# wyhlovecpp/GPT-Image-Edit

Measured on AMD Instinct MI355X. Metric: edited images/sec, 28-step FLUX-Kontext (VAE encode + 28 x MMDiT + VAE decode), higher is better.
Workload: dtype bf16; 1 GPU; cfg2_single_512x512_28step; batch_per_gpu=1, global_batch=1, height=512, width=512, S_txt=512, S_tgt=1024, S_cond=1024, seq_len=2560, num_inference_steps=28, blocks=19 double + 38 single, parallelism=dp1

## Files before the change

### gpt_image_edit_amd/csrc/attention_common.h

```cpp
#pragma once
#include <stdlib.h>

#include <type_traits>

#include "fk_common.h"

struct AttnParams {
  const bf16_t* q;
  const bf16_t* k;
  const bf16_t* v;
  bf16_t* o;
  int B, H, S;
  int64_t v_ld, v_bs;
  int64_t o_ld, o_bs;
  float scale_log2;
  float* lse;
  int n_items, min_part;
  int sk_rounds;
  float* sk_partials;
  unsigned* sk_ctl;
};

struct AttnMxOut {
  uint8_t *qa, *sa, *qb, *sb;
  int64_t ldq, lds;
  int split;
};

namespace {

constexpr int HD = 128;
constexpr int KVBLK = 64;
constexpr int K_TILE_BYTES = KVBLK * HD * 2;
constexpr int STAGE_BYTES = 2 * K_TILE_BYTES;

constexpr int PART_FLOATS = 256 * 128 + 2 * 512;

typedef __attribute__((address_space(3))) void lds_void;
typedef __attribute__((address_space(1))) const void gbl_void;
typedef short s16x4_t __attribute__((ext_vector_type(4)));

FK_DEV void buffer_lds16(__amdgpu_buffer_rsrc_t rsrc, char* lds_dst, int voffset, int soffset) {
#if defined(__HIP_DEVICE_COMPILE__)
  __builtin_amdgcn_raw_ptr_buffer_load_lds(rsrc, (lds_void*)lds_dst, 16, voffset, soffset, 0, 0);
#else
  (void)rsrc; (void)lds_dst; (void)voffset; (void)soffset;
#endif
}
FK_DEV void buffer_lds16(const BufDesc& d, char* lds_dst, int voffset, int soffset) {
  buffer_lds_opaque<16>(d, lds_addr_of(lds_dst), voffset, soffset);
}
FK_DEV s16x4_t lds_tr16(const char* p) {
  return __builtin_amdgcn_ds_read_tr16_b64_v4i16((__attribute__((address_space(3))) s16x4_t*)p);
}
template <int N>
FK_DEV void wait_vmcnt() {
  if constexpr (N == 0) asm volatile("s_waitcnt vmcnt(0)" ::: "memory");
  else if constexpr (N == 4) asm volatile("s_waitcnt vmcnt(4)" ::: "memory");
  else if constexpr (N == 8) asm volatile("s_waitcnt vmcnt(8)" ::: "memory");
  else if constexpr (N == 16) asm volatile("s_waitcnt vmcnt(16)" ::: "memory");
  else static_assert(N == 0, "add the vmcnt literal");
}

FK_DEV float merge2(float a, float wa, float b, float wb) {
#pragma clang fp contract(off)
  const float pa = a * wa;
  const float pb = b * wb;
  return pa + pb;
}

#ifndef FK_ATTN_PRIO
#define FK_ATTN_PRIO 1
#endif

}

int fk_attention_fwd4_launch(const AttnParams& p, int grid, bool streamk, hipStream_t stream);
int fk_attention_fwd4_mx_launch(const AttnParams& p, const AttnMxOut& mx, int grid, bool streamk, hipStream_t stream);
```

### gpt_image_edit_amd/csrc/attention_fwd.hip

```cpp
#include "attention_common.h"

namespace {

struct AttnParamsMasked : AttnParams {
  const uint64_t* kmask;
};

template <int NW, bool F32OUT, bool ILV, bool STREAMK, bool KMASK = false>
__global__ __launch_bounds__(NW * 64, NW >= 8 ? 2 : 1) void attention_fwd_kernel(
    const std::conditional_t<KMASK, AttnParamsMasked, AttnParams> p) {
  static_assert(!(KMASK && STREAMK), "masked launches take the plain grid");
  constexpr int STAGES = 3;
  constexpr int QBLK = NW * 32;
  static_assert(QBLK == 256, "the item list and the stream-K partial layout assume 256 query rows per workgroup");
  constexpr int LOADS = 32 / NW;
  constexpr int KL = LOADS / 2;
  constexpr int PF = STAGES - 1;
  extern __shared__ __attribute__((aligned(16))) char smem[];
  const int tid = threadIdx.x;
  const int lane = tid & 63;
  const int wave = __builtin_amdgcn_readfirstlane(tid >> 6);
  const int ql = lane & 31;
  const int hh = lane >> 5;

// ... 494 lines not shown
    const bool wide = ((p.o_ld | p.o_bs) & 7) == 0 && ((uintptr_t)p.o & 15) == 0;
#pragma unroll
    for (int df = 0; df < 4; ++df)
#pragma unroll
      for (int g = 0; g < 4; g += 2) {
        u32x2_t a, c;
        a[0] = pack_bf2(o[df][4 * g + 0] * inv, o[df][4 * g + 1] * inv);
        a[1] = pack_bf2(o[df][4 * g + 2] * inv, o[df][4 * g + 3] * inv);
        c[0] = pack_bf2(o[df][4 * g + 4] * inv, o[df][4 * g + 5] * inv);
        c[1] = pack_bf2(o[df][4 * g + 6] * inv, o[df][4 * g + 7] * inv);
        if (wide) {
#if defined(__HIP_DEVICE_COMPILE__)
          const auto r0 = __builtin_amdgcn_permlane32_swap(a[0], c[0], false, false);
          const auto r1 = __builtin_amdgcn_permlane32_swap(a[1], c[1], false, false);
          const u32x4_t w = {r0[0], r1[0], r0[1], r1[1]};
          if (q_row < p.S) *(u32x4_t*)(orow + 32 * df + 8 * g + 8 * hh) = w;
#endif
        } else if (q_row < p.S) {
          *(u32x2_t*)(orow + 32 * df + 8 * g + 4 * hh) = a;
          *(u32x2_t*)(orow + 32 * df + 8 * (g + 1) + 4 * hh) = c;
        }
      }
  }
  if constexpr (!STREAMK) break;
  else __syncthreads();
  }
}


__global__ __launch_bounds__(64) void pack_key_mask_kernel(const uint8_t* mask, int64_t batch_stride, int S, uint64_t* out) {
  const int t = blockIdx.x, b = blockIdx.y;
  const int key = t * KVBLK + (int)threadIdx.x;
  const bool valid = key < S && mask[(int64_t)b * batch_stride + key] != 0;
  const uint64_t w = __builtin_amdgcn_ballot_w64(valid);
  if (threadIdx.x == 0) out[(int64_t)b * gridDim.x + t] = w;
}

template <int NW, bool F32OUT, bool ILV, bool STREAMK, bool KMASK = false>
int launch(const std::conditional_t<KMASK, AttnParamsMasked, AttnParams>& p, int grid, hipStream_t stream) {
  constexpr int SMEM = 3 * STAGE_BYTES + 16;
  auto kern = attention_fwd_kernel<NW, F32OUT, ILV, STREAMK, KMASK>;
  FK_ENSURE_MAX_LDS(kern, SMEM, "fk_attention_fwd_bf16");
  hipLaunchKernelGGL(kern, dim3(grid), dim3(NW * 64), SMEM, stream, p);
  FK_CHECK_LAUNCH("fk_attention_fwd_bf16");
  return FK_OK;
}

static int attn_kernel_choice() {
  static int v = -1;
  if (v < 0) {
    const char* e = getenv("FK_ATTN_KERNEL");
    v = e && atoi(e) == 8 ? 8 : 4;
  }
  return v;
}

static int attn_cu_count() {
  static int cus = 0;
  if (!cus) {
    int dev = 0, v = 0;
    if (hipGetDevice(&dev) == hipSuccess &&
        hipDeviceGetAttribute(&v, hipDeviceAttributeMultiprocessorCount, dev) == hipSuccess && v > 0) cus = v;
    else return 256;
  }
  return cus;
}
constexpr int ATTN_MIN_PART = 8;
constexpr int ATTN_CTL_BYTES = 16384;

static bool use_interleaved(const AttnParams& p) {
  static int ov = -2;
  if (ov == -2) {
    const char* e = getenv("FK_ATTN_ILV");
    ov = e ? atoi(e) : -1;
  }
  if (ov >= 0) return ov != 0;
  return p.n_items >= 512;
}

int attention_entry(const void* q, const void* k, const void* v, void* o, int32_t B, int32_t H, int32_t S, int64_t v_ld,
                    int64_t v_batch_stride, int64_t o_ld, int64_t o_batch_stride, float scale, bool f32out,
                    hipStream_t stream, float* lse = nullptr, void* ws = nullptr, int64_t ws_bytes = 0, int grid = 0,
                    const AttnMxOut* mx = nullptr,
                    const uint64_t* kmask = nullptr) {
  FK_CHECK_ARG(grid >= -1 && grid != 1, "fk_attention_fwd_ws_bf16: grid %d is not 0 (stream-K grid where the plain one wastes a round), "
               "-1 (always one workgroup per 256-row block) or a workgroup count >= 2 (test hook)", grid);
  FK_CHECK_ARG(q && k && v && (o || mx), "fk_attention_fwd_bf16: null pointer");
  FK_CHECK_ARG(B > 0 && H > 0 && S > 0, "fk_attention_fwd_bf16: bad B/H/S %d %d %d", B, H, S);
  FK_CHECK_ARG(mx || (o_ld % 4 == 0 && o_batch_stride % 4 == 0 && ((uintptr_t)o % (f32out ? 16 : 8) == 0)),
               "fk_attention_fwd_bf16: output must be 8-byte aligned (o_ld %% 4 == 0)");
  FK_CHECK_ARG(v_ld % 8 == 0 && v_batch_stride % 8 == 0, "fk_attention_fwd_bf16: V strides must be multiples of 8");
  FK_CHECK_ARG(((uintptr_t)q % 16 == 0) && ((uintptr_t)k % 16 == 0) && ((uintptr_t)v % 16 == 0),
               "fk_attention_fwd_bf16: q/k/v must be 16-byte aligned");
  FK_CHECK_ARG(v_ld > 0 && (int64_t)S * HD * 2 < (1ll << 31) && ((int64_t)(S - 1) * v_ld + HD) * 2 < (1ll << 31) &&
                   (int64_t)(S + KVBLK) * v_ld * 2 < (1ll << 31),
               "fk_attention_fwd_bf16: S = %d with v_ld = %lld exceeds the 2 GiB a (batch, head)'s K / V may span", S,
               (long long)v_ld);
  const int64_t n_items = (int64_t)((S + 255) / 256) * H * B, nkt = (S + KVBLK - 1) / KVBLK;
  FK_CHECK_ARG(n_items * nkt < (1ll << 31), "fk_attention_fwd_bf16: B * H * S^2 too large for 32-bit tile counters");
  AttnParams p;
  p.q = (const bf16_t*)q; p.k = (const bf16_t*)k; p.v = (const bf16_t*)v; p.o = (bf16_t*)o;
  p.B = B; p.H = H; p.S = S; p.v_ld = v_ld; p.v_bs = v_batch_stride; p.o_ld = o_ld; p.o_bs = o_batch_stride;
  p.scale_log2 = scale * 1.4426950408889634f;
  p.lse = lse;
  p.n_items = (int)n_items;
  p.min_part = ATTN_MIN_PART;
  p.sk_rounds = 0;
  p.sk_partials = nullptr;
  p.sk_ctl = nullptr;
  if (kmask) {
    AttnParamsMasked pm;
    static_cast<AttnParams&>(pm) = p;
    pm.kmask = kmask;
    if (f32out) return launch<8, true, false, false, true>(pm, (int)n_items, stream);
    return use_interleaved(p) ? launch<8, false, true, false, true>(pm, (int)n_items, stream)
                              : launch<8, false, false, false, true>(pm, (int)n_items, stream);
  }
  if (f32out) return launch<8, true, false, false>(p, (int)n_items, stream);
  const int mode = grid == 0 ? 1 : (grid < 0 ? 0 : grid);
  const int G = mode >= 2 ? (mode < attn_cu_count() ? mode : attn_cu_count()) : attn_cu_count();
  const int64_t rounds = (n_items + G - 1) / G;
  const bool wasteful = mode >= 2 || (n_items > G && (rounds * G - n_items) * 25 >= rounds * G);
  int sk_rounds = (int)(n_items / G) - 1;
  while (sk_rounds >= 0 && (n_items - (int64_t)sk_rounds * G) * nkt < (int64_t)G * (nkt + 2 * ATTN_MIN_PART)) --sk_rounds;
  const bool cut_once = sk_rounds >= 0;
  const int64_t need = ATTN_CTL_BYTES + (int64_t)G * PART_FLOATS * 4;
  if (mode && wasteful && cut_once && ws && ws_bytes >= need && G <= ATTN_CTL_BYTES / 8) {
    p.sk_rounds = sk_rounds;
    FK_CHECK_ARG((uintptr_t)ws % 16 == 0, "fk_attention_fwd_ws_bf16: workspace must be 16-byte aligned");
    p.sk_ctl = (unsigned*)ws;
    p.sk_partials = (float*)((char*)ws + ATTN_CTL_BYTES);
    if (mx) return fk_attention_fwd4_mx_launch(p, *mx, G, true, stream);
    if (attn_kernel_choice() == 4) return fk_attention_fwd4_launch(p, G, true, stream);
    return use_interleaved(p) ? launch<8, false, true, true>(p, G, stream) : launch<8, false, false, true>(p, G, stream);
  }
  if (mx) return fk_attention_fwd4_mx_launch(p, *mx, (int)n_items, false, stream);
  if (attn_kernel_choice() == 4) return fk_attention_fwd4_launch(p, (int)n_items, false, stream);
  return use_interleaved(p) ? launch<8, false, true, false>(p, (int)n_items, stream)
                            : launch<8, false, false, false>(p, (int)n_items, stream);
}

}

extern "C" int64_t fk_attention_ws_bytes(void) { return ATTN_CTL_BYTES + (int64_t)attn_cu_count() * PART_FLOATS * 4; }

extern "C" int fk_attention_fwd_bf16(const void* q, const void* k, const void* v, void* o, int32_t B,
                                     int32_t H, int32_t S, int64_t v_ld, int64_t v_batch_stride, int64_t o_ld,
                                     int64_t o_batch_stride, float scale, fk_stream_t stream_) {
  return attention_entry(q, k, v, o, B, H, S, v_ld, v_batch_stride, o_ld, o_batch_stride, scale, false,
                         (hipStream_t)stream_);
}

extern "C" int fk_attention_fwd_lse_bf16(const void* q, const void* k, const void* v, void* o, float* lse, int32_t B,
                                         int32_t H, int32_t S, int64_t v_ld, int64_t v_batch_stride, int64_t o_ld,
                                         int64_t o_batch_stride, float scale, fk_stream_t stream_) {
  FK_CHECK_ARG(lse != nullptr, "fk_attention_fwd_lse_bf16: null lse");
  return attention_entry(q, k, v, o, B, H, S, v_ld, v_batch_stride, o_ld, o_batch_stride, scale, false,
                         (hipStream_t)stream_, lse);
}

extern "C" int fk_attention_fwd_ws_bf16(const void* q, const void* k, const void* v, void* o, float* lse, int32_t B, int32_t H,
                                        int32_t S, int64_t v_ld, int64_t v_batch_stride, int64_t o_ld, int64_t o_batch_stride,
                                        float scale, void* ws, int64_t ws_bytes, int32_t grid, fk_stream_t stream_) {
  return attention_entry(q, k, v, o, B, H, S, v_ld, v_batch_stride, o_ld, o_batch_stride, scale, false,
                         (hipStream_t)stream_, lse, ws, ws_bytes, grid);
}

extern "C" int fk_attention_fwd_ws_mxfp8(const void* q, const void* k, const void* v, float* lse, int32_t B, int32_t H, int32_t S,
                                         int64_t v_ld, int64_t v_batch_stride, float scale, const fk_attn_mx_out* out, void* ws,
                                         int64_t ws_bytes, int32_t grid, fk_stream_t stream_) {
  FK_CHECK_ARG(out != nullptr, "fk_attention_fwd_ws_mxfp8: null destination");
  FK_CHECK_ARG(H > 0 && S > 0 && out->split >= 0 && out->split <= S, "fk_attention_fwd_ws_mxfp8: bad H / S / split %d %d %lld", H, S,
               (long long)out->split);
  const int split = out->split == 0 ? S : (int)out->split;
  FK_CHECK_ARG(out->q && out->scales && (split == S || (out->q_b && out->scales_b)),
               "fk_attention_fwd_ws_mxfp8: null output pointer (rows [%d, %d) need the second stream)", split, S);
  const uintptr_t qbits = (uintptr_t)out->q | (split < S ? (uintptr_t)out->q_b : 0);
  const uintptr_t sbits = (uintptr_t)out->scales | (split < S ? (uintptr_t)out->scales_b : 0);
  FK_CHECK_ARG(out->ldq >= (int64_t)H * 128 && out->ldq % 16 == 0 && qbits % 16 == 0,
               "fk_attention_fwd_ws_mxfp8: output byte rows must be 16-byte aligned with ldq >= H * 128 (ldq %lld)", (long long)out->ldq);
  FK_CHECK_ARG(out->ldq_scale >= (int64_t)H * 4 && out->ldq_scale % 4 == 0 && sbits % 4 == 0,
               "fk_attention_fwd_ws_mxfp8: scale rows must be 4-byte aligned with ldq_scale >= H * 4 (ldq_scale %lld)",
               (long long)out->ldq_scale);
  if (attn_kernel_choice() != 4) {
    fk_set_error("fk_attention_fwd_ws_mxfp8: only the 4-wave kernel has the MXFP8-output form (FK_ATTN_KERNEL=8 is set)");
    return FK_EUNSUPPORTED;
  }
  const AttnMxOut mx = {(uint8_t*)out->q, (uint8_t*)out->scales, (uint8_t*)out->q_b, (uint8_t*)out->scales_b, out->ldq, out->ldq_scale,
                        split};
  return attention_entry(q, k, v, nullptr, B, H, S, v_ld, v_batch_stride, 0, 0, scale, false, (hipStream_t)stream_, lse, ws, ws_bytes,
                         grid, &mx);
}

extern "C" int fk_attention_fwd_f32_debug(const void* q, const void* k, const void* v, float* o, int32_t B,
                                          int32_t H, int32_t S, int64_t v_ld, int64_t v_batch_stride, int64_t o_ld,
                                          int64_t o_batch_stride, float scale, fk_stream_t stream_) {
  return attention_entry(q, k, v, o, B, H, S, v_ld, v_batch_stride, o_ld, o_batch_stride, scale, true,
                         (hipStream_t)stream_);
}

extern "C" int fk_pack_key_mask(const uint8_t* mask, int64_t batch_stride, int32_t B, int32_t S, uint64_t* out, fk_stream_t stream_) {
  FK_CHECK_ARG(mask && out && (uintptr_t)out % 8 == 0, "fk_pack_key_mask: null pointer or an output that is not 8-byte aligned");
  FK_CHECK_ARG(B > 0 && B <= 65535 && S > 0 && batch_stride >= 0, "fk_pack_key_mask: bad B / S / batch_stride %d %d %lld", B, S,
               (long long)batch_stride);
  hipLaunchKernelGGL(pack_key_mask_kernel, dim3((S + KVBLK - 1) / KVBLK, B), dim3(64), 0, (hipStream_t)stream_, mask, batch_stride, (int)S, out);
  FK_CHECK_LAUNCH("fk_pack_key_mask");
  return FK_OK;
}

extern "C" int fk_attention_fwd_masked_bf16(const void* q, const void* k, const void* v, void* o, float* lse, const uint64_t* kmask,
                                            int32_t B, int32_t H, int32_t S, int64_t v_ld, int64_t v_batch_stride, int64_t o_ld,
                                            int64_t o_batch_stride, float scale, fk_stream_t stream_) {
  FK_CHECK_ARG(kmask != nullptr && (uintptr_t)kmask % 8 == 0, "fk_attention_fwd_masked_bf16: the key mask must be an 8-byte aligned pointer");
  return attention_entry(q, k, v, o, B, H, S, v_ld, v_batch_stride, o_ld, o_batch_stride, scale, false, (hipStream_t)stream_, lse,
                         nullptr, 0, -1, nullptr, kmask);
}

extern "C" int fk_attention_fwd_masked_f32_debug(const void* q, const void* k, const void* v, float* o, const uint64_t* kmask, int32_t B,
                                                 int32_t H, int32_t S, int64_t v_ld, int64_t v_batch_stride, int64_t o_ld,
                                                 int64_t o_batch_stride, float scale, fk_stream_t stream_) {
  FK_CHECK_ARG(kmask != nullptr && (uintptr_t)kmask % 8 == 0, "fk_attention_fwd_masked_f32_debug: the key mask must be an 8-byte aligned pointer");
  return attention_entry(q, k, v, o, B, H, S, v_ld, v_batch_stride, o_ld, o_batch_stride, scale, true, (hipStream_t)stream_, nullptr,
                         nullptr, 0, -1, nullptr, kmask);
}
```

### gpt_image_edit_amd/csrc/attention_fwd4_kernel.inc

```
template <bool STREAMK>
__global__ __launch_bounds__(256, 1) void FK_A4_KERNEL(FK_A4_PARAMS) {
  constexpr int NW = 4, STAGES = A4_STAGES, QBLK = 256, LOADS = 32 / NW, KL = LOADS / 2, PF = STAGES - 1;
  extern __shared__ __attribute__((aligned(16))) char smem[];
  const int tid = threadIdx.x;
  const int lane = tid & 63;
  const int wave = __builtin_amdgcn_readfirstlane(tid >> 6);
  const int ql = lane & 31, hh = lane >> 5;
  const int nqb = (p.S + QBLK - 1) / QBLK;
  const int nkt = (p.S + KVBLK - 1) / KVBLK;
  int pos;
  {
    const int nwg = gridDim.x;
    const int q8 = nwg >> 3, r8 = nwg & 7;
    const int xcd = blockIdx.x & 7, idx = blockIdx.x >> 3;
    pos = (xcd < r8 ? xcd * (q8 + 1) : r8 * (q8 + 1) + (xcd - r8) * q8) + idx;
  }
  int u = 0, u_end = 0, round = 0;
  if constexpr (STREAMK) {
    const unsigned G = gridDim.x;
    const unsigned U = (unsigned)(p.n_items - p.sk_rounds * (int)G) * (unsigned)nkt;
    const unsigned qU = U / G, rU = U - qU * G;
    auto cut = [&](unsigned j) __attribute__((always_inline)) {
      unsigned c = qU * j + (rU * j) / G;
      const unsigned r = c % (unsigned)nkt;
      if (r != 0 && r < (unsigned)p.min_part) c -= r;
      else if (r != 0 && (unsigned)nkt - r < (unsigned)p.min_part) c += (unsigned)nkt - r;
      return (int)c;
    };
    u = cut(pos);
    u_end = cut(pos + 1);
  }
  const int prow = lane >> 4, pslot = lane & 15;
  const int tj = (lane & 15) >> 2, tq = lane & 3, tdh = (lane >> 4) & 1;
  const int v_rd = K_TILE_BYTES + (4 * hh + tj) * 256 + tdh * 32 + tq * 8;
  const int k_rd = ql * 256;
  const int k_sw = ql & 15;

  for (;;) {
  int item = pos, kt0 = 0, kt1 = nkt;
  if constexpr (STREAMK) {
    if (round < p.sk_rounds) {
      item = round * (int)gridDim.x + pos;
      ++round;
    } else {
      if (u >= u_end) break;
      const int ti = (unsigned)(u_end - 1) / (unsigned)nkt;
      item = p.sk_rounds * (int)gridDim.x + ti;
      kt1 = u_end - ti * nkt;
      kt0 = max(u - ti * nkt, 0);
      u_end -= kt1 - kt0;
    }
  }
  const int qb = item % nqb;
  const int bh = item / nqb;
  const int b = bh / p.H, h = bh - b * p.H;
  const int q_row0 = qb * QBLK + wave * 64;
  const bf16_t* Kg = p.k + (int64_t)bh * p.S * HD;
  const bf16_t* Vg = p.v + (int64_t)b * p.v_bs + h * HD;

  bf16x8_t qfA[8], qfB[8];
  {
    const bf16_t* qa = p.q + ((int64_t)bh * p.S + min(q_row0 + ql, p.S - 1)) * HD + 8 * hh;
    const bf16_t* qbp = p.q + ((int64_t)bh * p.S + min(q_row0 + 32 + ql, p.S - 1)) * HD + 8 * hh;
#pragma unroll
    for (int kk = 0; kk < 8; ++kk) {
      qfA[kk] = *(const bf16x8_t*)(qa + 16 * kk);
      qfB[kk] = *(const bf16x8_t*)(qbp + 16 * kk);
    }
  }
  const DmaDesc rs_k = make_dma_desc(Kg, (int64_t)p.S * HD * 2);
  const DmaDesc rs_v = make_dma_desc(Vg, ((int64_t)(p.S - 1) * p.v_ld + HD) * 2);
  const int k_voff0 = ((wave * 4 + prow) * HD + ((pslot ^ (wave * 4 + prow)) << 3)) * 2;
  const int v_voff0 = (int)(((wave * 4 + prow) * p.v_ld + ((((pslot >> 2) ^ prow) << 5) + ((pslot & 3) << 3))) * 2);
  const int k_tile_bytes = KVBLK * HD * 2, v_tile_bytes = (int)(KVBLK * p.v_ld * 2);
  const int v_piece_step = (int)(16 * p.v_ld * 2);
  auto issue_tile = [&](int kt, int stage) __attribute__((always_inline)) {
    char* sb = smem + stage * STAGE_BYTES;
#pragma unroll
    for (int i = 0; i < KL; ++i) {
      buffer_lds16(rs_k, sb + (i * NW + wave) * 1024, k_voff0, kt * k_tile_bytes + i * 4096);
      buffer_lds16(rs_v, sb + K_TILE_BYTES + (i * NW + wave) * 1024, v_voff0, kt * v_tile_bytes + i * v_piece_step);
    }
  };

  f32x16_t oA[4], oB[4];
  constexpr float REF_BIAS = 24.0f;
  float mA = 0.f, mB = 0.f, lA = 0.f, lB = 0.f, tA = 0.f, tB = 0.f;
  int st_cur = 0, st_pf = PF;
  auto fill = [&]() __attribute__((always_inline)) {
#pragma unroll
    for (int s = 0; s < PF; ++s)
      if (A4_DMA >= 2 || kt0 + s < kt1) issue_tile(min(kt0 + s, kt1 - 1), s);
    st_cur = 0;
    st_pf = PF;
  };
  auto acquire_tile = [&](int kt) __attribute__((always_inline)) {
    if (kt + PF - 1 < kt1) wait_vmcnt<(PF - 1) * LOADS>();
    else wait_vmcnt<0>();
    __builtin_amdgcn_s_barrier();
    if (kt + PF < kt1) issue_tile(kt + PF, st_pf);
    return smem + st_cur * STAGE_BYTES;
  };
  auto release_tile = [&]() __attribute__((always_inline)) {
    st_cur = (st_cur == STAGES - 1) ? 0 : st_cur + 1;
    st_pf = (st_pf == STAGES - 1) ? 0 : st_pf + 1;
  };
  auto k_frag = [&](const char* sb, int kb, int kk) __attribute__((always_inline)) {
    return *(const bf16x8_t*)(sb + k_rd + kb * 8192 + (((2 * kk + hh) ^ k_sw) << 4));
  };
  auto v_frag = [&](const char* sb, int st, int df) __attribute__((always_inline)) {
    const char* vp = sb + v_rd + st * 4096 + ((df ^ tj) << 6);
    const s16x4_t lo = lds_tr16(vp);
    const s16x4_t hi = lds_tr16(vp + 2048);
    bf16x8_t vf;
    vf[0] = lo[0]; vf[1] = lo[1]; vf[2] = lo[2]; vf[3] = lo[3];
    vf[4] = hi[0]; vf[5] = hi[1]; vf[6] = hi[2]; vf[7] = hi[3];
    return vf;
  };
  auto mask_block = [&](f32x16_t& s, int kt, int kb) __attribute__((always_inline)) {
    const int kbase = kt * KVBLK + 32 * kb + 4 * hh;
#pragma unroll
    for (int r = 0; r < 16; ++r)
      if (kbase + (r & 3) + 8 * (r >> 2) >= p.S) s[r] = -1.0e30f;
  };
  auto block_max = [&](const f32x16_t& s) __attribute__((always_inline)) {
    float mx = s[0];
#pragma unroll
    for (int r = 1; r < 16; ++r) mx = fmaxf(mx, s[r]);
    return fmaxf(mx, __shfl_xor(mx, 32)) * p.scale_log2;
  };
  bf16x8_t kf[8], vfr[8];
  f32x16_t sA, sB;
  u32x4_t pA[2], pB[2];

#define FK_SLOT_FENCE() __builtin_amdgcn_sched_barrier(0)
  auto s_mfma = [&](f32x16_t& acc, const bf16x8_t& a, const bf16x8_t& b, bool first) __attribute__((always_inline)) {
    if (first) asm volatile("v_mfma_f32_32x32x16_bf16 %0, %1, %2, 0" : "=&v"(acc) : "v"(a), "v"(b));
// ... 306 lines not shown
```

### gpt_image_edit_amd/csrc/blocks.hip

```cpp
#include "fk_common.h"

namespace {

constexpr int HD = 128;

struct Dims {
  int B, S_txt, S_img, S, H, D;
};

struct View {
  const void* p;
  fk_rows r;
};
View view(const void* base, const Dims& d, int64_t ld, int64_t r0, int64_t R, int64_t c0) {
  return View{(const char*)base + (r0 * ld + c0) * 2, fk_rows{ld, R, (int64_t)d.S * ld}};
}

void set_ws(fk_gemm_args& g, const fk_block_ws& ws) {
  if (g.K >= 6144 && g.N % 256 == 0 && (int64_t)g.M <= 256ll * ws.splitk_slots && ws.splitk_ws) {
    g.splitk_ws = ws.splitk_ws;
    g.splitk_slots = ws.splitk_slots;
  }
}

// ... 205 lines not shown
  {
    fk_gemm_args g = gemm(none, nullptr, w.bqkv, view(ws.qkv, d, 3 * D, 0, d.S, 0), Ms, 3 * D, D, FK_EPI_QKV);
    qkv_epi(g, ws, d, w.norm_q, w.norm_k, 0);
    ctl(g, ws); FK_TRY(mx_gemm(mxws, &g, 1, &n8, &wx.qkv, nullptr, 0, st));
  }
  const int rc_mx = (mxws.fused & 2) ? attention_mx(ws, d, cat8, nullptr, 0, st) : FK_EUNSUPPORTED;
  if (rc_mx != FK_EUNSUPPORTED) FK_TRY(rc_mx);
  else {
    FK_TRY(fk_attention_fwd_ws_bf16(ws.q, ws.k, (const char*)ws.qkv + (int64_t)2 * D * 2, ws.cat, nullptr, B, d.H, d.S, 3 * D,
                                    (int64_t)d.S * 3 * D, 5 * D, (int64_t)d.S * 5 * D, 0.08838834764831845f, ws.attn_ws,
                                    ws.attn_ws_bytes, ws.attn_grid, st));
    const View att = view(ws.cat, d, 5 * D, 0, d.S, 0);
    FK_TRY(quantize_view(mxws, att, Ms, D, cat8, st));
  }
  {
    fk_gemm_args g = gemm(none, nullptr, w.b_mlp, none, Ms, 4 * D, D, FK_EPI_GELU_TANH);
    ctl(g, ws); FK_TRY(mx_gemm(mxws, &g, 1, &n8, &wx.mlp, &cat8, D, st));
  }
  {
    fk_gemm_args g = gemm(none, nullptr, w.b_out, s_all, Ms, D, 5 * D, FK_EPI_GATE_RES);
    gate_res(g, s_all, chunk(2), mod_bs, d.S);
    set_ws(g, ws);
    ctl(g, ws); FK_TRY(mx_gemm(mxws, &g, 1, &cat8, &wx.out, nullptr, 0, st));
  }
  return FK_OK;
}

int double_block(const fk_block_ws& ws, const Dims& d, const fk_double_block_weights& w, const void* mod, int64_t mod_bs,
                 fk_stream_t st, const fk_mx_ws* mxws = nullptr,
                 const fk_double_block_weights_mx* wx = nullptr) {
  if (mxws && wx && mxws->fused) return double_block_fused(ws, d, w, mod, mod_bs, st, *mxws, *wx);
  FK_CHECK_ARG(ws.o && ws.ff && d.S_txt > 0, "fk_double_block_fwd: needs the o / ff buffers and a text stream");
  Mx mxc;
  auto mx = [&](const fk_mx_pair* pair) -> const Mx* { if (!pair) return nullptr; mxc = Mx{mxws, pair}; return &mxc; };
  const int D = d.D, B = d.B, Mi = B * d.S_img, Mt = B * d.S_txt;
  const char* mi = (const char*)mod + w.mod_off_img * 2;
  const char* mt = (const char*)mod + w.mod_off_txt * 2;
  auto chunk = [&](const char* m, int j) { return (const void*)(m + (int64_t)j * D * 2); };
  const View s_all = view(ws.s, d, D, 0, d.S, 0), n_all = view(ws.n, d, D, 0, d.S, 0);
  const View h = view(ws.s, d, D, d.S_txt, d.S_img, 0), cx = view(ws.s, d, D, 0, d.S_txt, 0);
  const View n_img = view(ws.n, d, D, d.S_txt, d.S_img, 0), n_txt = view(ws.n, d, D, 0, d.S_txt, 0);
  const int64_t M = (int64_t)B * d.S;
  FK_TRY(fk_ln_modulate2_bf16(s_all.p, s_all.r, (void*)n_all.p, n_all.r, chunk(mt, 0), chunk(mt, 1), chunk(mi, 0), chunk(mi, 1),
                              d.S_txt, mod_bs, d.S, M, D, ws.eps, st));
  {
    fk_gemm_args g[2];
    g[0] = gemm(n_img, w.wqkv_img, w.bqkv_img, view(ws.qkv, d, 3 * D, d.S_txt, d.S_img, 0), Mi, 3 * D, D, FK_EPI_QKV);
    qkv_epi(g[0], ws, d, w.norm_q, w.norm_k, d.S_txt);
    g[1] = gemm(n_txt, w.wqkv_txt, w.bqkv_txt, view(ws.qkv, d, 3 * D, 0, d.S_txt, 0), Mt, 3 * D, D, FK_EPI_QKV);
    qkv_epi(g[1], ws, d, w.norm_added_q, w.norm_added_k, 0);
    ctl(g[0], ws); FK_TRY(block_gemm(g, 2, mx(wx ? &wx->qkv_img : nullptr), st));
  }
  FK_TRY(fk_attention_fwd_ws_bf16(ws.q, ws.k, (const char*)ws.qkv + (int64_t)2 * D * 2, ws.o, nullptr, B, d.H, d.S, 3 * D,
                                  (int64_t)d.S * 3 * D, D, (int64_t)d.S * D, 0.08838834764831845f, ws.attn_ws, ws.attn_ws_bytes, ws.attn_grid, st));
  {
    fk_gemm_args g[2];
    g[0] = gemm(view(ws.o, d, D, d.S_txt, d.S_img, 0), w.w_out, w.b_out, h, Mi, D, D, FK_EPI_GATE_RES);
    gate_res(g[0], h, chunk(mi, 2), mod_bs, d.S_img);
    g[1] = gemm(view(ws.o, d, D, 0, d.S_txt, 0), w.w_add_out, w.b_add_out, cx, Mt, D, D, FK_EPI_GATE_RES);
    gate_res(g[1], cx, chunk(mt, 2), mod_bs, d.S_txt);
    set_ws(g[0], ws); set_ws(g[1], ws);
    ctl(g[0], ws); FK_TRY(block_gemm(g, 2, mx(wx ? &wx->out : nullptr), st));
  }
  FK_TRY(fk_ln_modulate2_bf16(s_all.p, s_all.r, (void*)n_all.p, n_all.r, chunk(mt, 3), chunk(mt, 4), chunk(mi, 3), chunk(mi, 4),
                              d.S_txt, mod_bs, d.S, M, D, ws.eps, st));
  {
    fk_gemm_args g[2];
    g[0] = gemm(n_img, w.w_ff1, w.b_ff1, view(ws.ff, d, 4 * D, d.S_txt, d.S_img, 0), Mi, 4 * D, D, FK_EPI_GELU_TANH);
    g[1] = gemm(n_txt, w.w_ff1_ctx, w.b_ff1_ctx, view(ws.ff, d, 4 * D, 0, d.S_txt, 0), Mt, 4 * D, D, FK_EPI_GELU_TANH);
    ctl(g[0], ws); FK_TRY(block_gemm(g, 2, mx(wx ? &wx->ff1 : nullptr), st));
  }
  {
    fk_gemm_args g[2];
    g[0] = gemm(view(ws.ff, d, 4 * D, d.S_txt, d.S_img, 0), w.w_ff2, w.b_ff2, h, Mi, D, 4 * D, FK_EPI_GATE_RES);
    gate_res(g[0], h, chunk(mi, 5), mod_bs, d.S_img);
    g[1] = gemm(view(ws.ff, d, 4 * D, 0, d.S_txt, 0), w.w_ff2_ctx, w.b_ff2_ctx, cx, Mt, D, 4 * D, FK_EPI_GATE_RES);
    gate_res(g[1], cx, chunk(mt, 5), mod_bs, d.S_txt);
    set_ws(g[0], ws); set_ws(g[1], ws);
    ctl(g[0], ws); FK_TRY(block_gemm(g, 2, mx(wx ? &wx->ff2 : nullptr), st));
  }
  return FK_OK;
}

int single_block(const fk_block_ws& ws, const Dims& d, const fk_single_block_weights& w, const void* mod, int64_t mod_bs,
                 fk_stream_t st, const fk_mx_ws* mxws = nullptr, const fk_single_block_weights_mx* wx = nullptr) {
  if (mxws && wx && mxws->fused) return single_block_fused(ws, d, w, mod, mod_bs, st, *mxws, *wx);
  Mx mxc;
  auto mx = [&](const fk_mx_pair* pair) -> const Mx* { if (!pair) return nullptr; mxc = Mx{mxws, pair}; return &mxc; };
  FK_CHECK_ARG(ws.cat != nullptr, "fk_single_block_fwd: needs the [attn | mlp] buffer");
  const int D = d.D, B = d.B;
  const int Ms = B * d.S;
  const char* m0 = (const char*)mod + w.mod_off * 2;
  auto chunk = [&](int j) { return (const void*)(m0 + (int64_t)j * D * 2); };
  const View s_all = view(ws.s, d, D, 0, d.S, 0), n_all = view(ws.n, d, D, 0, d.S, 0);
  FK_TRY(fk_ln_modulate_bf16(s_all.p, s_all.r, (void*)n_all.p, n_all.r, chunk(0), chunk(1), mod_bs, d.S, (int64_t)Ms, D, ws.eps, st));
  {
    fk_gemm_args g = gemm(n_all, w.wqkv, w.bqkv, view(ws.qkv, d, 3 * D, 0, d.S, 0), Ms, 3 * D, D, FK_EPI_QKV);
    qkv_epi(g, ws, d, w.norm_q, w.norm_k, 0);
    ctl(g, ws); FK_TRY(block_gemm(&g, 1, mx(wx ? &wx->qkv : nullptr), st));
  }
  FK_TRY(fk_attention_fwd_ws_bf16(ws.q, ws.k, (const char*)ws.qkv + (int64_t)2 * D * 2, ws.cat, nullptr, B, d.H, d.S, 3 * D,
                                  (int64_t)d.S * 3 * D, 5 * D, (int64_t)d.S * 5 * D, 0.08838834764831845f, ws.attn_ws,
                                  ws.attn_ws_bytes, ws.attn_grid, st));
  {
    fk_gemm_args g = gemm(n_all, w.w_mlp, w.b_mlp, view(ws.cat, d, 5 * D, 0, d.S, D), Ms, 4 * D, D, FK_EPI_GELU_TANH);
    ctl(g, ws); FK_TRY(block_gemm(&g, 1, mx(wx ? &wx->mlp : nullptr), st));
  }
  {
    fk_gemm_args g = gemm(view(ws.cat, d, 5 * D, 0, d.S, 0), w.w_out, w.b_out, s_all, Ms, D, 5 * D, FK_EPI_GATE_RES);
    gate_res(g, s_all, chunk(2), mod_bs, d.S);
    set_ws(g, ws);
    ctl(g, ws); FK_TRY(block_gemm(&g, 1, mx(wx ? &wx->out : nullptr), st));
  }
  return FK_OK;
}

}

extern "C" int fk_double_block_fwd(const fk_block_ws* ws, const fk_double_block_weights* w, const void* mod,
                                   int64_t mod_batch_stride, fk_stream_t stream) {
  Dims d;
  FK_TRY(check_ws(ws, d, "fk_double_block_fwd"));
  FK_CHECK_ARG(w && mod, "fk_double_block_fwd: null weights / modulation");
  return double_block(*ws, d, *w, mod, mod_batch_stride, stream);
}

extern "C" int fk_single_block_fwd(const fk_block_ws* ws, const fk_single_block_weights* w, const void* mod,
                                   int64_t mod_batch_stride, fk_stream_t stream) {
  Dims d;
  FK_TRY(check_ws(ws, d, "fk_single_block_fwd"));
  FK_CHECK_ARG(w && mod, "fk_single_block_fwd: null weights / modulation");
  return single_block(*ws, d, *w, mod, mod_batch_stride, stream);
}

extern "C" int fk_mmdit_blocks_fwd(const fk_block_ws* ws, const fk_double_block_weights* dbl, int32_t n_double,
                                   const fk_single_block_weights* sgl, int32_t n_single, const void* mod,
                                   int64_t mod_batch_stride, fk_stream_t stream) {
  Dims d;
  FK_TRY(check_ws(ws, d, "fk_mmdit_blocks_fwd"));
  FK_CHECK_ARG(mod && n_double >= 0 && n_single >= 0 && (n_double == 0 || dbl) && (n_single == 0 || sgl),
               "fk_mmdit_blocks_fwd: null weights / modulation");
  for (int i = 0; i < n_double; ++i) FK_TRY(double_block(*ws, d, dbl[i], mod, mod_batch_stride, stream));
  for (int i = 0; i < n_single; ++i) FK_TRY(single_block(*ws, d, sgl[i], mod, mod_batch_stride, stream));
  return FK_OK;
}

namespace {
int check_mx(const fk_mx_ws* mx, const char* who) {
  FK_CHECK_ARG(mx && mx->q && mx->s && (uintptr_t)mx->q % 16 == 0 && (uintptr_t)mx->s % 4 == 0,
               "%s: null or misaligned quantized-activation workspace", who);
  FK_CHECK_ARG((mx->fused & 3) != 2,
               "%s: fk_mx_ws.fused = %d: bit 1 (the attention emits MXFP8) is valid only together with bit 0 (the fused schedule)", who,
               (int)mx->fused);
  return FK_OK;
}
}

extern "C" int fk_double_block_fwd_mx(const fk_block_ws* ws, const fk_mx_ws* mx, const fk_double_block_weights* w,
                                      const fk_double_block_weights_mx* wx, const void* mod, int64_t mod_batch_stride,
                                      fk_stream_t stream) {
  Dims d;
  FK_TRY(check_ws(ws, d, "fk_double_block_fwd_mx"));
  FK_TRY(check_mx(mx, "fk_double_block_fwd_mx"));
  FK_CHECK_ARG(w && wx && mod, "fk_double_block_fwd_mx: null weights / modulation");
  return double_block(*ws, d, *w, mod, mod_batch_stride, stream, mx, wx);
}

extern "C" int fk_single_block_fwd_mx(const fk_block_ws* ws, const fk_mx_ws* mx, const fk_single_block_weights* w,
                                      const fk_single_block_weights_mx* wx, const void* mod, int64_t mod_batch_stride,
                                      fk_stream_t stream) {
  Dims d;
  FK_TRY(check_ws(ws, d, "fk_single_block_fwd_mx"));
  FK_TRY(check_mx(mx, "fk_single_block_fwd_mx"));
  FK_CHECK_ARG(w && wx && mod, "fk_single_block_fwd_mx: null weights / modulation");
  return single_block(*ws, d, *w, mod, mod_batch_stride, stream, mx, wx);
}

extern "C" int fk_mmdit_blocks_fwd_mx(const fk_block_ws* ws, const fk_mx_ws* mx, const fk_double_block_weights* dbl,
                                      const fk_double_block_weights_mx* dblx, int32_t n_double, const fk_single_block_weights* sgl,
                                      const fk_single_block_weights_mx* sglx, int32_t n_single, const void* mod,
                                      int64_t mod_batch_stride, fk_stream_t stream) {
  Dims d;
  FK_TRY(check_ws(ws, d, "fk_mmdit_blocks_fwd_mx"));
  FK_TRY(check_mx(mx, "fk_mmdit_blocks_fwd_mx"));
  FK_CHECK_ARG(mod && n_double >= 0 && n_single >= 0 && (n_double == 0 || (dbl && dblx)) && (n_single == 0 || (sgl && sglx)),
               "fk_mmdit_blocks_fwd_mx: null weights / modulation");
  if (mx->fused) {
    if (n_double > 0) FK_TRY(check_fused_ws(*mx, d, 4 * d.D, "fk_mmdit_blocks_fwd_mx"));
    if (n_single > 0) FK_TRY(check_fused_ws(*mx, d, 5 * d.D, "fk_mmdit_blocks_fwd_mx"));
  }
  for (int i = 0; i < n_double; ++i) FK_TRY(double_block(*ws, d, dbl[i], mod, mod_batch_stride, stream, mx, &dblx[i]));
  for (int i = 0; i < n_single; ++i) FK_TRY(single_block(*ws, d, sgl[i], mod, mod_batch_stride, stream, mx, &sglx[i]));
  return FK_OK;
}
```

### gpt_image_edit_amd/libfk.py

```python
import ctypes
import os

_HERE = os.path.dirname(os.path.abspath(__file__))
LIB_PATH = os.environ.get("FK_LIB_PATH") or os.path.join(_HERE, "libfk_gfx950.so")

c_i32, c_i64, c_f32, c_vp = ctypes.c_int32, ctypes.c_int64, ctypes.c_float, ctypes.c_void_p
c_f64 = ctypes.c_double

FK_PRODIGY_SLOTS = ("d", "d_max", "d_numerator", "d_denom", "d_hat", "dlr", "k", "skipped", "sum_dot", "sum_abs")

FK_SPLITK_SLOT_BYTES = 256 * 256 * 4 + 8
FK_EPI_NONE, FK_EPI_GELU_TANH, FK_EPI_SILU, FK_EPI_GATE_RES, FK_EPI_RES, FK_EPI_SCALE, FK_EPI_QKV = range(7)


class Rows(ctypes.Structure):
    _fields_ = [("ld", c_i64), ("rows_per_batch", c_i64), ("batch_stride", c_i64)]


class GemmArgs(ctypes.Structure):
    _fields_ = [
        ("A", c_vp), ("a", Rows),
        ("W", c_vp), ("ldw", c_i64),
        ("bias", c_vp),
        ("C", c_vp), ("c", Rows),
# ... 47 lines not shown
        ("dmodT", c_vp), ("gemm_variant", c_i32), ("gemm_plan", c_i32), ("gemm_group_m", c_i32), ("gemm_mfma", c_i32), ("attn_grid", c_i32),
        ("attn_passes", c_i32), ("gemm_variant_used", ctypes.POINTER(c_i32))]


class BlockSaved(ctypes.Structure):
    _fields_ = [(n, c_vp) for n in ("x0", "n1", "qkv", "q", "k", "y1", "h1", "o", "lse", "x1", "n2", "y2")]


SINGLE_GRAD_FIELDS = ("dwqkv", "dbqkv", "dw_mlp", "db_mlp", "dw_out", "db_out", "dnorm", "dw_mod", "db_mod")
DOUBLE_GRAD_FIELDS = ("dwqkv_img", "dbqkv_img", "dwqkv_txt", "dbqkv_txt", "dw_out", "db_out", "dw_add_out", "db_add_out", "dw_ff1", "db_ff1",
                      "dw_ff1_ctx", "db_ff1_ctx", "dw_ff2", "db_ff2", "dw_ff2_ctx", "db_ff2_ctx", "dnorm", "dw_mod_img", "db_mod_img",
                      "dw_mod_txt", "db_mod_txt")


class SingleBlockGrads(ctypes.Structure):
    _fields_ = [(n, c_vp) for n in SINGLE_GRAD_FIELDS]


class DoubleBlockGrads(ctypes.Structure):
    _fields_ = [(n, c_vp) for n in DOUBLE_GRAD_FIELDS]


DOUBLE_BLOCK_FIELDS = ("wqkv_img", "bqkv_img", "wqkv_txt", "bqkv_txt", "norm_q", "norm_k", "norm_added_q", "norm_added_k",
                       "w_out", "b_out", "w_add_out", "b_add_out", "w_ff1", "b_ff1", "w_ff1_ctx", "b_ff1_ctx",
                       "w_ff2", "b_ff2", "w_ff2_ctx", "b_ff2_ctx")
SINGLE_BLOCK_FIELDS = ("wqkv", "bqkv", "norm_q", "norm_k", "w_mlp", "b_mlp", "w_out", "b_out")


class DoubleBlockWeights(ctypes.Structure):
    _fields_ = [(n, c_vp) for n in DOUBLE_BLOCK_FIELDS] + [("mod_off_img", c_i64), ("mod_off_txt", c_i64)]


class SingleBlockWeights(ctypes.Structure):
    _fields_ = [(n, c_vp) for n in SINGLE_BLOCK_FIELDS] + [("mod_off", c_i64)]


class MxPair(ctypes.Structure):
    _fields_ = [("q", c_vp), ("s", c_vp)]


DOUBLE_BLOCK_MX_FIELDS = ("qkv_img", "qkv_txt", "out", "add_out", "ff1", "ff1_ctx", "ff2", "ff2_ctx")
SINGLE_BLOCK_MX_FIELDS = ("qkv", "mlp", "out")


class DoubleBlockWeightsMx(ctypes.Structure):
    _fields_ = [(n, MxPair) for n in DOUBLE_BLOCK_MX_FIELDS]


class SingleBlockWeightsMx(ctypes.Structure):
    _fields_ = [(n, MxPair) for n in SINGLE_BLOCK_MX_FIELDS]


class AttnMxOut(ctypes.Structure):
    _fields_ = [("q", c_vp), ("scales", c_vp), ("q_b", c_vp), ("scales_b", c_vp), ("split", c_i64), ("ldq", c_i64), ("ldq_scale", c_i64)]


class MxWs(ctypes.Structure):
    _fields_ = [("q", c_vp), ("s", c_vp), ("q_bytes", c_i64), ("s_bytes", c_i64), ("fused", c_i32),
                ("quantize_launches", ctypes.POINTER(c_i32)), ("splitk", c_i32)]


class LoraTerm(ctypes.Structure):
    _fields_ = [("up", c_vp), ("ld_up", c_i64), ("down", c_vp), ("ld_down", c_i64), ("rank", c_i32), ("scale", c_f32)]


FK_LORA_MAX_TERMS, FK_LORA_MAX_RANK = 4, 128

SIGNATURES = {
    "fk_gemm_bf16": (c_i32, [ctypes.POINTER(GemmArgs), c_vp]),
    "fk_gemm_bf16_grouped": (c_i32, [ctypes.POINTER(GemmArgs), c_i32, c_vp]),
    "fk_quantize_mxfp8": (c_i32, [c_vp, Rows, c_i64, c_i32, c_vp, c_i64, c_vp, c_i64, c_vp]),
    "fk_gemm_mxfp8": (c_i32, [ctypes.POINTER(GemmMxfp8Args), c_vp]),
    "fk_gemm_mxfp8_grouped": (c_i32, [ctypes.POINTER(GemmMxfp8Args), c_i32, c_vp]),
    "fk_gemm_mxfp8_q": (c_i32, [ctypes.POINTER(GemmMxfp8QArgs), c_vp]),
    "fk_gemm_mxfp8_q_grouped": (c_i32, [ctypes.POINTER(GemmMxfp8QArgs), c_i32, c_vp]),
    "fk_ln_modulate_mxfp8": (c_i32, [c_vp, Rows, c_vp, c_i64, c_vp, c_i64, c_vp, c_vp, c_i64, c_i64, c_i64, c_i32, c_f32, c_vp]),
    "fk_ln_modulate2_mxfp8": (c_i32, [c_vp, Rows, c_vp, c_vp, c_vp, c_vp, c_i64, c_i64, c_vp, c_vp, c_vp, c_vp, c_i64, c_i64, c_i64,
                                      c_i64, c_i32, c_f32, c_vp]),
    "fk_ln_modulate_bf16": (c_i32, [c_vp, Rows, c_vp, Rows, c_vp, c_vp, c_i64, c_i64, c_i64, c_i32, c_f32, c_vp]),
    "fk_ln_modulate2_bf16": (c_i32, [c_vp, Rows, c_vp, Rows, c_vp, c_vp, c_vp, c_vp, c_i64, c_i64, c_i64, c_i64, c_i32, c_f32, c_vp]),
    "fk_qkv_post_bf16": (c_i32, [c_vp] * 9 + [c_i32] * 4 + [c_f32, c_vp]),
    "fk_attention_fwd_bf16": (c_i32, [c_vp] * 4 + [c_i32] * 3 + [c_i64] * 4 + [c_f32, c_vp]),
    "fk_attention_fwd_ws_bf16": (c_i32, [c_vp] * 5 + [c_i32] * 3 + [c_i64] * 4 + [c_f32, c_vp, c_i64, c_i32, c_vp]),
    "fk_attention_fwd_ws_mxfp8": (c_i32, [c_vp] * 4 + [c_i32] * 3 + [c_i64] * 2 + [c_f32, ctypes.POINTER(AttnMxOut), c_vp, c_i64, c_i32, c_vp]),
    "fk_attention_ws_bytes": (c_i64, []),
    "fk_attention_fwd_f32_debug": (c_i32, [c_vp] * 4 + [c_i32] * 3 + [c_i64] * 4 + [c_f32, c_vp]),
    "fk_pack_key_mask": (c_i32, [c_vp, c_i64, c_i32, c_i32, c_vp, c_vp]),
    "fk_attention_fwd_masked_bf16": (c_i32, [c_vp] * 6 + [c_i32] * 3 + [c_i64] * 4 + [c_f32, c_vp]),
    "fk_attention_fwd_masked_f32_debug": (c_i32, [c_vp] * 5 + [c_i32] * 3 + [c_i64] * 4 + [c_f32, c_vp]),
    "fk_attention_bwd_masked_bf16": (c_i32, [ctypes.POINTER(AttnView)] * 4 + [c_vp, c_vp] + [ctypes.POINTER(AttnView)] * 3 + [c_vp] + [c_i32] * 3 + [c_f32, c_i32, c_vp]),
    "fk_attention_fwd_lse_bf16": (c_i32, [c_vp] * 5 + [c_i32] * 3 + [c_i64] * 4 + [c_f32, c_vp]),
    "fk_attention_bwd_bf16": (c_i32, [ctypes.POINTER(AttnView)] * 4 + [c_vp, c_vp] + [ctypes.POINTER(AttnView)] * 3 + [c_i32] * 3 + [c_f32, c_vp]),
    "fk_attention_bwd_ws_bf16": (c_i32, [ctypes.POINTER(AttnView)] * 4 + [c_vp, c_vp] + [ctypes.POINTER(AttnView)] * 3 + [c_i32] * 3 + [c_f32, c_vp, c_i64, c_i32, c_i32, c_vp]),
    "fk_bwd_ws_floats": (c_i64, []),
    "fk_bwd_ew_max_blocks": (c_i64, []),
    "fk_ln_modulate_bwd_bf16": (c_i32, [c_vp, Rows, c_vp, Rows, c_vp, c_i64, c_i64, c_vp, Rows, c_vp, Rows, c_vp, c_vp, c_i64, c_vp, c_i32, c_i32, c_f32, c_vp]),
    "fk_gate_res_bwd_bf16": (c_i32, [c_vp, Rows, c_vp, Rows, c_vp, c_i64, c_i64, c_vp, Rows, c_vp, c_i64, c_vp, c_i32, c_i32, c_vp]),
    "fk_gelu_bwd_bf16": (c_i32, [c_vp, c_vp, c_vp, c_i64, c_vp]),
    "fk_silu_bwd_bf16": (c_i32, [c_vp, c_vp, c_vp, c_i64, c_vp]),
    "fk_qkv_post_bwd_bf16": (c_i32, [c_vp] * 12 + [c_i32] * 4 + [c_f32, c_vp]),
    "fk_gate_res_fwd_bf16": (c_i32, [c_vp, Rows, c_vp, Rows, c_vp, c_i64, c_i64, c_vp, Rows, c_i64, c_i32, c_vp]),
    "fk_gelu_tanh_bf16": (c_i32, [c_vp, Rows, c_vp, Rows, c_i64, c_i32, c_vp]),
    "fk_f32_to_bf16_transposed": (c_i32, [c_vp, c_i64, c_vp, c_i32, c_i32, c_i32, c_vp]),
    "fk_colsum_bf16": (c_i32, [c_vp, Rows, c_i64, c_i32, c_vp, c_vp, c_vp]),
    "fk_rowdot_bf16": (c_i32, [c_vp, c_i64, c_i64, c_vp, c_i64, c_i64, c_vp, c_i32, c_i32, c_i32, c_vp]),
    "fk_silu_bf16": (c_i32, [c_vp, c_vp, c_i64, c_vp]),
    "fk_timestep_proj": (c_i32, [c_vp, c_i32, c_vp, c_vp, c_i32, c_vp]),
    "fk_add3_bf16": (c_i32, [c_vp] * 4 + [c_i64, c_vp]),
    "fk_true_cfg_bf16": (c_i32, [c_vp, c_vp, c_vp, c_f32, c_i64, c_vp]),
    "fk_reduce_ws_doubles": (c_i64, []),
    "fk_flow_noisy_tokens_bf16": (c_i32, [c_vp, c_vp, c_vp, c_vp, c_i64] + [c_i32] * 4 + [c_vp]),
    "fk_flow_loss_bf16": (c_i32, [c_vp, c_i64, c_vp, c_vp, c_vp, c_vp, c_i64, c_vp, c_vp] + [c_i32] * 4 + [c_vp]),
    "fk_flow_loss_weighted_bf16": (c_i32, [c_vp, c_i64, c_vp, c_vp, c_vp, c_vp, c_vp, c_vp, c_vp, c_i64, c_vp, c_vp] + [c_i32] * 4 + [c_vp]),
    "fk_sumsq": (c_i32, [c_vp, c_i32, c_i64, c_i32, c_vp, c_vp, c_vp]),
    "fk_adamw_step": (c_i32, [c_vp, c_vp, c_vp, c_i32, c_vp, c_vp, c_vp] + [c_f32] * 6 + [c_i32, c_i64, c_vp]),
    "fk_adamw_step_scaled": (c_i32, [c_vp, c_vp, c_vp, c_i32, c_vp, c_vp, c_vp] + [c_f32] * 7 + [c_i32, c_i64, c_vp]),
    "fk_prodigy_ws_doubles": (c_i64, []),
    "fk_prodigy_begin": (c_i32, [c_vp] + [c_f64] * 4 + [c_i32, c_vp]),
    "fk_prodigy_moments": (c_i32, [c_vp, c_vp, c_vp, c_i32, c_vp, c_vp, c_vp, c_vp, c_vp] + [c_f32] * 6 + [c_f64, c_i32, c_i32,
                                                                                                         c_i64, c_vp, c_vp]),
    "fk_prodigy_update_d": (c_i32, [c_vp, c_f64, c_f64, c_f64, c_vp]),
    "fk_prodigy_apply": (c_i32, [c_vp, c_vp, c_vp, c_vp, c_vp, c_f32, c_f32, c_i32, c_i64, c_vp]),
    "fk_euler_step_bf16": (c_i32, [c_vp, c_i64, c_vp, c_i64, c_i32, c_i32, c_i32, c_f32, c_vp]),
    "fk_euler_inpaint_step_bf16": (c_i32, [c_vp, c_i64, c_vp, c_i64, c_vp, c_i64, c_vp, c_i64, c_vp, c_i64, c_i32, c_i32, c_i32,
                                           c_f32, c_f32, c_vp]),
    "fk_scale_noise_bf16": (c_i32, [c_vp, c_i64, c_vp, c_i64, c_vp, c_i64, c_i32, c_i32, c_i32, c_f32, c_vp]),
    "fk_ab2_step_bf16": (c_i32, [c_vp, c_i64, c_vp, c_i64, c_vp, c_i64, c_vp, c_i64, c_vp, c_i64, c_vp, c_i64, c_i32, c_i32, c_i32,
                                 c_f32, c_f32, c_i32, c_f32, c_vp]),
    "fk_solver_step_f32": (c_i32, [c_vp, c_i64, c_vp, c_i64, c_vp, c_i64, c_vp, c_i64, c_vp, c_i64, c_vp, c_i64, c_vp, c_i64,
                                   c_i32, c_i32, c_i32, c_f32, c_f32, c_i32, c_i32, c_f32, c_vp]),
    "fk_absdiff_ws_floats": (c_i64, []),
    "fk_absdiff_sums_bf16": (c_i32, [c_vp, Rows, c_vp, Rows, c_i64, c_i32, c_i32, c_vp, c_vp, c_i64, c_vp]),
    "fk_residual_absdiff_sums_bf16": (c_i32, [c_vp, Rows, c_vp, Rows, c_vp, Rows, c_vp, Rows, c_i64, c_i32, c_i32, c_vp, c_vp, c_i64,
                                              c_vp]),
    "fk_residual_save_bf16": (c_i32, [c_vp, Rows, c_vp, Rows, c_vp, Rows, c_i64, c_i32, c_i32, c_vp]),
    "fk_residual_apply_bf16": (c_i32, [c_vp, Rows, c_vp, Rows, c_vp, Rows, c_i64, c_i32, c_i32, c_vp]),
    "fk_lora_merge_bf16": (c_i32, [c_vp, c_i64, c_vp, c_i64, c_i32, c_i32, ctypes.POINTER(LoraTerm), c_i32, c_vp]),
    "fk_lora_grad_ws_floats": (c_i64, [c_i32, c_i32, c_i32]),
    "fk_lora_grad_bf16": (c_i32, [c_vp, c_i64, c_vp, c_i64, c_vp, c_i64, c_i32, c_i32, c_i32, c_f32, c_vp, c_vp, c_vp, c_i64, c_vp]),
    "fk_lora_grad_acc_bf16": (c_i32, [c_vp, c_i64, c_vp, c_i64, c_vp, c_i64, c_i32, c_i32, c_i32, c_f32, c_vp, c_vp, c_i32, c_vp, c_i64,
                                      c_vp]),
    "fk_lora_side_grad_ws_floats": (c_i64, [c_i64] * 5),
    "fk_lora_side_grad_bf16": (c_i32, [c_vp, c_i64, c_i64, c_vp, c_i64, c_i64, c_i64, c_i64, c_i64, c_i64, c_vp, c_i64, c_vp, c_i64,
                                       c_i64, c_f32, c_vp, c_vp, c_i32, c_vp, c_i64, c_vp]),
    "fk_transpose_bf16": (c_i32, [c_vp, c_i64, c_i64, c_vp, c_i64, c_i64, c_i32, c_i32, c_i32, c_vp]),
    "fk_attention_hd512_bf16": (c_i32, [c_vp, c_vp, c_vp, c_i64, c_i64, c_vp, c_i64, c_i64, c_i32, c_i32, c_f32, c_vp]),
    "fk_softmax_rows": (c_i32, [c_vp, c_i64, c_vp, c_i64, c_i64, c_i32, c_vp]),
    "fk_softmax_rows_parts": (c_i32, [c_vp, c_i64, c_vp, c_i64, c_i64, c_i64, c_i32, c_vp]),
    "fk_split_f32_rows": (c_i32, [c_vp, c_i64, c_vp, c_i64, c_i64, c_i64, c_i32, c_i32, c_i32, c_vp]),
    "fk_groupnorm_f32_nhwc": (c_i32, [c_vp, c_vp, c_vp, c_vp, c_vp, c_vp, c_i32, c_i64, c_i32, c_i32, c_f32, c_i32, c_i32, c_vp]),
    "fk_conv2d_nhwc_f32out": (c_i32, [c_vp, c_vp]),
    "fk_conv3x3_halo_f32out": (c_i32, [c_vp, c_vp]),
    "fk_nchw_f32_to_nhwc_parts": (c_i32, [c_vp, c_vp, c_i32, c_i32, c_i32, c_i32, c_i32, c_i32, c_vp]),
    "fk_nhwc_f32_to_nchw": (c_i32, [c_vp, c_vp, c_i32, c_i32, c_i32, c_i32, c_i32, c_f32, c_f32, c_vp]),
    "fk_conv2d_nhwc_bf16": (c_i32, [ctypes.POINTER(ConvArgs), c_vp]),
    "fk_conv3x3_halo_bf16": (c_i32, [ctypes.POINTER(ConvArgs), c_vp, c_vp, c_vp, c_i32, c_i32, c_vp]),
    "fk_conv3x3_halo_f32_debug": (c_i32, [ctypes.POINTER(ConvArgs), c_vp, c_vp, c_vp, c_i32, c_i32, c_vp]),
    "fk_groupnorm_ws_floats": (c_i64, [c_i32, c_i64, c_i32]),
    "fk_groupnorm_stats_nhwc_bf16": (c_i32, [c_vp, c_vp, c_vp, c_i32, c_i64, c_i32, c_i32, c_f32, c_vp]),
    "fk_groupnorm_apply_nhwc_bf16": (c_i32, [c_vp] * 5 + [c_i32, c_i64, c_i32, c_i32, c_i32, c_vp]),
    "fk_nchw_to_nhwc_bf16": (c_i32, [c_vp, c_i32, c_vp] + [c_i32] * 5 + [c_f32, c_f32, c_vp]),
    "fk_nhwc_to_nchw": (c_i32, [c_vp, c_vp] + [c_i32] * 6 + [c_f32, c_f32, c_vp]),
    "fk_pixels_u8_to_nhwc_bf16": (c_i32, [c_vp, c_vp] + [c_i32] * 7 + [c_vp]),
    "fk_image_to_u8_nhwc": (c_i32, [c_vp, c_i32, c_vp] + [c_i32] * 4 + [c_vp]),
    "fk_mask_bbox_ws_ints": (c_i64, []),
    "fk_mask_bbox_u8": (c_i32, [c_vp] + [c_i32] * 4 + [c_vp, c_vp, c_i64, c_vp]),
    "fk_mask_blur_u8": (c_i32, [c_vp] * 4 + [c_i32] * 4 + [c_vp]),
    "fk_pixels_u8_box_to_nhwc_bf16": (c_i32, [c_vp, c_vp] + [c_i32] * 11 + [c_vp]),
    "fk_image_overlay_u8": (c_i32, [c_vp] + [c_i32] * 3 + [c_vp, c_i32, c_vp, c_i32, c_vp] + [c_i32] * 7 + [c_vp]),
    "fk_double_block_fwd": (c_i32, [ctypes.POINTER(BlockWs), ctypes.POINTER(DoubleBlockWeights), c_vp, c_i64, c_vp]),
    "fk_single_block_fwd": (c_i32, [ctypes.POINTER(BlockWs), ctypes.POINTER(SingleBlockWeights), c_vp, c_i64, c_vp]),
    "fk_single_block_bwd": (c_i32, [ctypes.POINTER(BwdWs), ctypes.POINTER(BlockSaved), ctypes.POINTER(SingleBlockWeights),
                                    ctypes.POINTER(SingleBlockGrads), c_vp]),
    "fk_double_block_bwd": (c_i32, [ctypes.POINTER(BwdWs), ctypes.POINTER(BlockSaved), ctypes.POINTER(DoubleBlockWeights),
                                    ctypes.POINTER(DoubleBlockGrads), c_vp]),
    "fk_double_block_fwd_mx": (c_i32, [ctypes.POINTER(BlockWs), ctypes.POINTER(MxWs), ctypes.POINTER(DoubleBlockWeights),
                                       ctypes.POINTER(DoubleBlockWeightsMx), c_vp, c_i64, c_vp]),
    "fk_single_block_fwd_mx": (c_i32, [ctypes.POINTER(BlockWs), ctypes.POINTER(MxWs), ctypes.POINTER(SingleBlockWeights),
                                       ctypes.POINTER(SingleBlockWeightsMx), c_vp, c_i64, c_vp]),
    "fk_mmdit_blocks_fwd_mx": (c_i32, [ctypes.POINTER(BlockWs), ctypes.POINTER(MxWs), ctypes.POINTER(DoubleBlockWeights),
                                       ctypes.POINTER(DoubleBlockWeightsMx), c_i32, ctypes.POINTER(SingleBlockWeights),
                                       ctypes.POINTER(SingleBlockWeightsMx), c_i32, c_vp, c_i64, c_vp]),
    "fk_mmdit_blocks_fwd": (c_i32, [ctypes.POINTER(BlockWs), ctypes.POINTER(DoubleBlockWeights), c_i32,
                                    ctypes.POINTER(SingleBlockWeights), c_i32, c_vp, c_i64, c_vp]),
    "fk_last_error": (ctypes.c_char_p, []),
    "fk_version": (ctypes.c_char_p, []),
}

_lib = None


def load():
    global _lib
    if _lib is not None:
        return _lib
    if not os.path.exists(LIB_PATH):
        raise RuntimeError(
            f"{LIB_PATH} not found: the HIP extension is not built. Run `python -c 'import "
            f"__graft_entry__ as g; g.build()'` (or `make -C gpt_image_edit_amd/csrc`). There is no CPU "
            f"fallback for the FLUX-Kontext hot path.")
    lib = ctypes.CDLL(LIB_PATH)
    for name, (res, args) in SIGNATURES.items():
        fn = getattr(lib, name)
        fn.restype = res
        fn.argtypes = args
    _lib = lib
    return lib


def check(code, what):
    if code != 0:
        msg = load().fk_last_error().decode(errors="replace")
        raise RuntimeError(f"{what} failed (code {code}): {msg}")
```

### gpt_image_edit_amd/ops.py

```python
import ctypes
import threading
from types import SimpleNamespace
import os

import torch

from . import helpers, libfk, param_tree
from .libfk import (FK_EPI_GATE_RES, FK_EPI_GELU_TANH, FK_EPI_NONE, FK_EPI_QKV, FK_EPI_RES, FK_EPI_SCALE,
                    FK_EPI_SILU, GemmArgs, GemmMxfp8Args, GemmMxfp8QArgs, Rows)

BF16 = torch.bfloat16


def _stream():
    return ctypes.c_void_p(torch.cuda.current_stream().cuda_stream)


def _ptr(t):
    return ctypes.c_void_p(t.data_ptr()) if t is not None else ctypes.c_void_p(0)


def _need_cuda(*ts):
    for t in ts:
        if t is not None and not t.is_cuda:
# ... 31 lines not shown
        _SPLITK_WS[key] = ws
    return ws, SPLITK_SLOTS


_VARIANT_USED = threading.local()


def _variant_slot():
    slot = getattr(_VARIANT_USED, "slot", None)
    if slot is None:
        slot = _VARIANT_USED.slot = ctypes.c_int32(0)
    return slot


def gemm_last_variant():
    return int(_variant_slot().value)


def _check_splitk_ws(splitk_ws):
    ws, slots = splitk_ws
    _need_cuda(ws)
    if (ws.dtype != torch.uint8 or not ws.is_contiguous() or int(slots) < 1 or ws.numel() < int(slots) * libfk.FK_SPLITK_SLOT_BYTES
            or ws.data_ptr() % 16 != 0):
        raise ValueError("splitk_ws: (contiguous 16-byte aligned uint8 tensor of >= slots * FK_SPLITK_SLOT_BYTES bytes, slots >= 1)")
    return ws, int(slots)


def _gemm_args(a, w, bias, out, epilogue, res, gate, out_fp32, alpha, qkv=None, layout=0, splitk_ws=None):
    _need_cuda(a, w, bias, out, res, gate)
    if a.dtype != BF16 or w.dtype != BF16:
        raise TypeError("fk_gemm_bf16 takes bf16 operands")
    if layout == 0:
        M, ra = rows_of(a)
        N, K = w.shape
        if a.shape[-1] != K:
            raise ValueError(f"K mismatch: a {tuple(a.shape)} vs w {tuple(w.shape)}")
        out_shape = (*a.shape[:-1], N)
    elif layout == 1:
        M, ra = rows_of(a)
        K, N = w.shape
        if a.shape[-1] != K or w.stride(1) != 1:
            raise ValueError(f"layout 1: a {tuple(a.shape)} @ w {tuple(w.shape)} (w rows contiguous)")
        out_shape = (*a.shape[:-1], N)
    elif layout == 2:
        a = a[0] if a.dim() == 3 and a.shape[0] == 1 else a
        w = w[0] if w.dim() == 3 and w.shape[0] == 1 else w
        K, ra = rows_of(a)
        M, N = a.shape[-1], w.shape[-1]
        Kw, rw = rows_of(w)
        if Kw != K or w.stride(-1) != 1 or (rw.rows_per_batch > 0 and rw.batch_stride != rw.rows_per_batch * rw.ld):
            raise ValueError(f"layout 2: a {tuple(a.shape)} ^T @ w {tuple(w.shape)} (uniformly strided w rows)")
        out_shape = (M, N)
    else:
        raise ValueError(f"layout {layout}")
    if out is None:
        out = torch.empty(out_shape, device=a.device, dtype=torch.float32 if out_fp32 else BF16)
    Mo, rc = rows_of(out)
    if Mo != M or out.shape[-1] != N:
        raise ValueError(f"output shape {tuple(out.shape)} does not match M={M}, N={N}")
    args = GemmArgs()
    args.layout = layout
    args.A, args.a = a.data_ptr(), ra
    args.W, args.ldw = w.data_ptr(), (w.stride(0) if layout != 2 else rw.ld)
    args.bias = bias.data_ptr() if bias is not None else None
    args.C, args.c = out.data_ptr(), rc
    if res is not None:
        Mr, rr = rows_of(res)
        if Mr != M:
            raise ValueError("residual rows mismatch")
        args.res, args.r = res.data_ptr(), rr
    if gate is not None:
        if a.dim() != 3 or gate.dim() != 2 or gate.shape[0] != a.shape[0] or gate.stride(1) != 1:
            raise ValueError("gate must be a [B, N] view matching a 3-D activation")
        args.gate = gate.data_ptr()
        args.gate_batch_stride = gate.stride(0)
        args.gate_rows_per_batch = a.shape[1]
    args.M, args.N, args.K = M, N, K
    _apply_gemm_launch(args)
    args.variant_used = ctypes.pointer(_variant_slot())
    args.epilogue, args.out_fp32, args.alpha = epilogue, int(out_fp32), float(alpha)
    if int(out_fp32) == 1:
        args.f32_flags = ((1 if bias is not None and bias.dtype == torch.float32 else 0) |
                          (2 if res is not None and res.dtype == torch.float32 and epilogue == FK_EPI_NONE else 0))
    if splitk_ws is not None:
        ws, slots = _check_splitk_ws(splitk_ws)
        args.splitk_ws, args.splitk_slots = ws.data_ptr(), slots
    elif K >= 6144 and N % 256 == 0 and M <= 256 * SPLITK_SLOTS and int(out_fp32) != 1 and layout == 0:
        ws, slots = splitk_workspace(a.device)
        args.splitk_ws, args.splitk_slots = ws.data_ptr(), slots
    if epilogue == FK_EPI_QKV:
        _set_qkv(args, qkv)
    return args, out


def _set_qkv(args, qkv):
    cs = qkv["cs"] if "cs" in qkv else pack_rope(qkv["cos"], qkv["sin"])
    _need_cuda(qkv["q_out"], qkv["k_out"], qkv["wq"], qkv["wk"], cs)
    if cs.dtype != torch.float32 or not cs.is_contiguous() or tuple(cs.shape) != (qkv["q_out"].shape[2], 64, 2):
        raise ValueError("cs must be a contiguous fp32 [S_total, 64, 2] table (see pack_rope)")
    args.q_out, args.k_out = qkv["q_out"].data_ptr(), qkv["k_out"].data_ptr()
    args.wq, args.wk = qkv["wq"].data_ptr(), qkv["wk"].data_ptr()
    args.rope_cs = cs.data_ptr()
    args.qkv_s_offset, args.qkv_s_total, args.qkv_heads = qkv["s_offset"], qkv["q_out"].shape[2], qkv["q_out"].shape[1]


def gemm(a, w, bias=None, out=None, epilogue=FK_EPI_NONE, res=None, gate=None, out_fp32=False, alpha=1.0, qkv=None, layout=0,
         splitk_ws=None):
    args, out = _gemm_args(a, w, bias, out, epilogue, res, gate, out_fp32, alpha, qkv, layout, splitk_ws)
    libfk.check(libfk.load().fk_gemm_bf16(ctypes.byref(args), _stream()), "fk_gemm_bf16")
    return out


FK_GEMM_PLAN_EXPLICIT = 8
FK_GEMM_PLAN_SPLITK = {"default": 0, "whole": 16, "symmetric": 32, "unannounced": 64}


def _env_int(name, default):
    v = os.environ.get(name)
    return default if v is None or v == "" else int(v)


LAUNCH = SimpleNamespace(
    gemm_variant=_env_int("FK_GEMM_BN", 0),
    gemm_plan=(FK_GEMM_PLAN_EXPLICIT | (_env_int("FK_GEMM_PLAN", 3) & 7)) if os.environ.get("FK_GEMM_PLAN") else 0,
    gemm_splitk=0,
    gemm_group_m=_env_int("FK_GEMM_GROUP_M", 0),
    gemm_mfma=_env_int("FK_GEMM_MFMA", 0),
    attn_grid={0: -1, 1: 0}.get(_env_int("FK_ATTN_SPLIT", 1), _env_int("FK_ATTN_SPLIT", 1)),
    attn_bwd_passes=0 if _env_int("FK_ATTN_BWD", 1) else 3)
_LAUNCH_CFG_EPOCH = [0]


def launch_config_epoch():
    return _LAUNCH_CFG_EPOCH[0]


def _set_launch(**kw):
    for k, v in kw.items():
        setattr(LAUNCH, k, v)
    _LAUNCH_CFG_EPOCH[0] += 1


def gemm_set_variant(variant):
    if int(variant) not in (0, 128, 256, 384, 512, 640, 1024):
        raise ValueError(f"gemm_set_variant: {variant} is not one of 0, 128, 256, 384, 512, 640, 1024")
    _set_launch(gemm_variant=int(variant))


def gemm_set_plan(allow):
    if not 0 <= int(allow) <= 7:
        raise ValueError(f"gemm_set_plan: {allow} is not in 0..7")
    _set_launch(gemm_plan=FK_GEMM_PLAN_EXPLICIT | int(allow))


def gemm_set_splitk_exchange(mode):
    _set_launch(gemm_splitk=FK_GEMM_PLAN_SPLITK[mode])


def launch_plan():
    if not LAUNCH.gemm_splitk:
        return LAUNCH.gemm_plan
    return (LAUNCH.gemm_plan or (FK_GEMM_PLAN_EXPLICIT | 3)) | LAUNCH.gemm_splitk


def gemm_set_group_m(depth):
    if not 0 <= int(depth) <= 4096:
        raise ValueError(f"gemm_set_group_m: {depth} is not 0 (default) or 1..4096 row tiles")
# ... 196 lines not shown
    return outs


def ln_modulate(x, shift, scale, out=None, eps=1e-6):
    _need_cuda(x, shift, scale, out)
    if x.dim() != 3:
        raise ValueError("x must be [B, R, D]")
    B, R, D = x.shape
    if out is None:
        out = torch.empty((B, R, D), device=x.device, dtype=BF16)
    M, rx = rows_of(x)
    _, ro = rows_of(out)
    if shift.stride(0) != scale.stride(0) or shift.stride(1) != 1 or scale.stride(1) != 1:
        raise ValueError("shift/scale must be [B, D] views with a common batch stride")
    lib = libfk.load()
    libfk.check(lib.fk_ln_modulate_bf16(_ptr(x), rx, _ptr(out), ro, _ptr(shift), _ptr(scale),
                                        shift.stride(0), R, M, D, eps, _stream()), "fk_ln_modulate_bf16")
    return out


def ln_modulate2(x, shift_a, scale_a, shift_b, scale_b, split, out=None, eps=1e-6):
    _need_cuda(x, shift_a, scale_a, shift_b, scale_b, out)
    B, R, D = x.shape
    if out is None:
        out = torch.empty((B, R, D), device=x.device, dtype=BF16)
    M, rx = rows_of(x)
    _, ro = rows_of(out)
    st = shift_a.stride(0)
    if any(t.stride(0) != st or t.stride(1) != 1 for t in (scale_a, shift_b, scale_b)):
        raise ValueError("modulation views must share one batch stride")
    libfk.check(libfk.load().fk_ln_modulate2_bf16(_ptr(x), rx, _ptr(out), ro, _ptr(shift_a), _ptr(scale_a),
                                                  _ptr(shift_b), _ptr(scale_b), split, st, R, M, D, eps, _stream()),
                "fk_ln_modulate2_bf16")
    return out


def qkv_post(qkv, q_out, k_out, wq_img, wk_img, wq_txt, wk_txt, cos, sin, s_txt, eps=1e-6):
    _need_cuda(qkv, q_out, k_out, cos, sin)
    B, S, D3 = qkv.shape
    H = D3 // 384
    if not qkv.is_contiguous():
        raise ValueError("qkv must be contiguous")
    lib = libfk.load()
    libfk.check(lib.fk_qkv_post_bf16(_ptr(qkv), _ptr(q_out), _ptr(k_out), _ptr(wq_img), _ptr(wk_img), _ptr(wq_txt),
                                     _ptr(wk_txt), _ptr(cos), _ptr(sin), B, S, s_txt, H, eps, _stream()),
                "fk_qkv_post_bf16")


_ATTN_WS = {}


def attention_workspace(device):
    key = (device.index if device.index is not None else torch.cuda.current_device(), torch.cuda.current_stream(device).cuda_stream)
    ws = _ATTN_WS.get(key)
    if ws is None:
        ws = torch.zeros(libfk.load().fk_attention_ws_bytes(), device=device, dtype=torch.uint8)
        _ATTN_WS[key] = ws
    return ws


def attention_set_split(mode):
    mode = int(mode)
    if mode < 0:
        raise ValueError(f"attention_set_split: {mode} is not 0, 1 or a workgroup count >= 2")
    _set_launch(attn_grid={0: -1, 1: 0}.get(mode, mode))


def pack_key_mask(mask):
    _need_cuda(mask)
    if mask.dim() != 2:
        raise ValueError("pack_key_mask takes a [B, S] mask")
    m = (mask != 0).to(torch.uint8).contiguous()
    B, S = m.shape
    out = torch.empty((B, (S + 63) // 64), device=m.device, dtype=torch.int64)
    libfk.check(libfk.load().fk_pack_key_mask(_ptr(m), m.stride(0), B, S, _ptr(out), _stream()), "fk_pack_key_mask")
    return out


def _check_key_mask(key_mask, B, S):
    if key_mask.dtype != torch.int64 or key_mask.shape != (B, (S + 63) // 64) or not key_mask.is_contiguous():
        raise ValueError(f"key_mask must be the contiguous int64 [{B}, {(S + 63) // 64}] tensor pack_key_mask gives")


def attention(q, k, v, out, scale=None, lse=None, key_mask=None):
    _need_cuda(q, k, v, out, lse, key_mask)
    B, H, S, hd = q.shape
    if hd != 128:
        raise ValueError("head_dim must be 128")
    if v.dim() != 3 or v.shape[-1] != H * 128 or v.stride(2) != 1:
        raise ValueError("v must be a [B, S, H*128] view with a contiguous last dimension")
    if lse is not None and (lse.dtype != torch.float32 or lse.shape != (B, H, S) or not lse.is_contiguous()):
        raise ValueError("lse must be a contiguous fp32 [B,H,S] tensor")
    if scale is None:
        scale = hd ** -0.5
    if key_mask is not None:
        _check_key_mask(key_mask, B, S)
        libfk.check(libfk.load().fk_attention_fwd_masked_bf16(_ptr(q), _ptr(k), _ptr(v), _ptr(out), _ptr(lse), _ptr(key_mask), B, H, S,
                                                             v.stride(1), v.stride(0), out.stride(1), out.stride(0), scale,
                                                             _stream()), "fk_attention_fwd_masked_bf16")
        return out
    ws = attention_workspace(q.device)
    libfk.check(libfk.load().fk_attention_fwd_ws_bf16(_ptr(q), _ptr(k), _ptr(v), _ptr(out), _ptr(lse), B, H, S, v.stride(1),
                                                     v.stride(0), out.stride(1), out.stride(0), scale, _ptr(ws), ws.numel(),
                                                     LAUNCH.attn_grid, _stream()), "fk_attention_fwd_bf16")
    return out


def attention_mxfp8(q, k, v, out, out_b=None, split=0, scale=None, lse=None):
    _need_cuda(q, k, v, lse, *out, *(out_b or ()))
    B, H, S, hd = q.shape
    if hd != 128:
        raise ValueError("head_dim must be 128")
    if v.dim() != 3 or v.shape[-1] != H * 128 or v.stride(2) != 1:
        raise ValueError("v must be a [B, S, H*128] view with a contiguous last dimension")
    if lse is not None and (lse.dtype != torch.float32 or lse.shape != (B, H, S) or not lse.is_contiguous()):
        raise ValueError("lse must be a contiguous fp32 [B,H,S] tensor")
    pairs = [out] + ([out_b] if out_b is not None else [])
    for qt, st in pairs:
        if qt.dtype != torch.uint8 or st.dtype != torch.uint8 or qt.dim() != 2 or st.dim() != 2 or qt.stride(1) != 1 or st.stride(1) != 1:
            raise ValueError("attention_mxfp8: an output is a (uint8 [rows, cols], uint8 [rows, cols / 32]) pair, rows contiguous")
    if len({pr[0].stride(0) for pr in pairs}) != 1 or len({pr[1].stride(0) for pr in pairs}) != 1:
        raise ValueError("attention_mxfp8: both streams' outputs must share their row strides")
    dst = libfk.AttnMxOut(_ptr(out[0]), _ptr(out[1]), _ptr(out_b[0]) if out_b is not None else None,
                          _ptr(out_b[1]) if out_b is not None else None, int(split), out[0].stride(0), out[1].stride(0))
    ws = attention_workspace(q.device)
    libfk.check(libfk.load().fk_attention_fwd_ws_mxfp8(_ptr(q), _ptr(k), _ptr(v), _ptr(lse), B, H, S, v.stride(1), v.stride(0),
                                                      hd ** -0.5 if scale is None else scale, ctypes.byref(dst), _ptr(ws),
                                                      ws.numel(), LAUNCH.attn_grid, _stream()), "fk_attention_fwd_ws_mxfp8")
    return out if out_b is None else (out, out_b)


def attention_f32_debug(q, k, v, scale=None, key_mask=None):
    _need_cuda(q, k, v, key_mask)
    B, H, S, hd = q.shape
    if hd != 128 or v.dim() != 3 or v.shape[-1] != H * 128 or v.stride(2) != 1:
        raise ValueError("q, k: [B,H,S,128]; v: [B,S,H*128] view with a contiguous last dimension")
    out = torch.empty((B, S, H * 128), device=q.device, dtype=torch.float32)
    if key_mask is not None:
        _check_key_mask(key_mask, B, S)
        libfk.check(libfk.load().fk_attention_fwd_masked_f32_debug(_ptr(q), _ptr(k), _ptr(v), _ptr(out), _ptr(key_mask), B, H, S,
                                                                  v.stride(1), v.stride(0), out.stride(1), out.stride(0),
                                                                  hd ** -0.5 if scale is None else scale, _stream()),
                    "fk_attention_fwd_masked_f32_debug")
        return out
    libfk.check(libfk.load().fk_attention_fwd_f32_debug(_ptr(q), _ptr(k), _ptr(v), _ptr(out), B, H, S, v.stride(1),
                                                       v.stride(0), out.stride(1), out.stride(0),
                                                       hd ** -0.5 if scale is None else scale, _stream()),
                "fk_attention_fwd_f32_debug")
    return out


def silu(x, out=None):
    _need_cuda(x)
    if out is None:
        out = torch.empty_like(x)
    libfk.check(libfk.load().fk_silu_bf16(_ptr(x), _ptr(out), x.numel(), _stream()), "fk_silu_bf16")
    return out


def add3(a, b, c, out=None):
    _need_cuda(a, b, c)
    if out is None:
        out = torch.empty_like(a)
    libfk.check(libfk.load().fk_add3_bf16(_ptr(a), _ptr(b), _ptr(c), _ptr(out), a.numel(), _stream()),
                "fk_add3_bf16")
    return out


def true_cfg(pos, neg, scale, out=None):
    _need_cuda(pos, neg, out)
    if pos.shape != neg.shape or pos.dtype != BF16 or neg.dtype != BF16 or not (pos.is_contiguous() and neg.is_contiguous()):
        raise ValueError("true_cfg takes two contiguous bf16 tensors of one shape")
    if out is None:
        out = torch.empty_like(pos)
    libfk.check(libfk.load().fk_true_cfg_bf16(_ptr(pos), _ptr(neg), _ptr(out), float(scale), pos.numel(), _stream()),
                "fk_true_cfg_bf16")
    return out


def timestep_proj(v, freqs, out=None):
    _need_cuda(v, freqs)
    B = v.shape[0]
    if v.dtype not in (BF16, torch.float32):
        raise TypeError("timestep must be bf16 or fp32")
# ... 926 lines not shown
```

### gpt_image_edit_amd/pipeline.py

```python
import os
from types import SimpleNamespace

import numpy as np
import torch

from . import helpers, image_processor, ops
from .scheduler import FlowMatchEulerDiscreteScheduler

BF16 = torch.bfloat16


class FluxPipelineOutput(SimpleNamespace):
    pass


class FluxKontextPipeline:
    def __init__(self, transformer, vae, scheduler=None, text_encoder=None, tokenizer=None,
                 text_encoder_2=None, tokenizer_2=None, use_graph=None):
        self.use_graph = (os.environ.get("FK_GRAPH", "0") == "1") if use_graph is None else bool(use_graph)
        self._loop_graph = None
        self.transformer = transformer
        self.vae = vae
        self.scheduler = scheduler or FlowMatchEulerDiscreteScheduler()
        self.text_encoder, self.tokenizer = text_encoder, tokenizer
# ... 398 lines not shown

        num_channels_latents = self.transformer.config.in_channels // 4
        latents, image_latents, latent_ids, image_ids = self.prepare_latents(
            image, batch_size, num_channels_latents, height, width, BF16, device, generator, latents)
        S_tgt = latents.shape[1]
        if image_ids is not None:
            latent_ids = torch.cat([latent_ids, image_ids], dim=0)
            tokens = torch.cat([latents, image_latents], dim=1).contiguous()
        else:
            tokens = latents.contiguous().clone()
        x0 = noise = None
        if mask is not None or strength < 1.0:
            if init_image is None and cond_hw == (height, width):
                x0 = image_latents
            else:
                x0 = self._encode_init_image(image_in if init_image is None else init_image, batch_size,
                                             num_channels_latents, height, width, device, edit)
            noise = latents.contiguous()

        sig = np.linspace(1.0, 1 / num_inference_steps, num_inference_steps) if sigmas is None else sigmas
        cfg = self.scheduler.config
        mu = helpers.calculate_shift(S_tgt, cfg.get("base_image_seq_len", 256), cfg.get("max_image_seq_len", 4096),
                                     cfg.get("base_shift", 0.5), cfg.get("max_shift", 1.15))
        self.scheduler.set_timesteps(sigmas=sig, mu=mu, device="cpu")
        t_start = helpers.strength_t_start(len(self.scheduler.timesteps), strength)
        timesteps = self.scheduler.timesteps[t_start:]
        self._num_timesteps = len(timesteps)
        t_model = (timesteps.to(BF16) / 1000)[:, None].expand(-1, model_batch).contiguous().to(device)
        guidance = None
        if self.transformer.config.guidance_embeds:
            guidance = torch.full([model_batch], guidance_scale, device=device, dtype=torch.float32)
        self.scheduler.set_begin_index(t_start)
        if t_start > 0:
            ops.scale_noise(x0, noise, float(self.scheduler._sigmas_host[t_start]), out=tokens[:, :S_tgt])
        steps = range(t_start, t_start + len(timesteps))
        model_tokens = torch.empty((model_batch, *tokens.shape[1:]), device=device, dtype=BF16) if do_true_cfg else tokens
        solver_order = getattr(self.scheduler, "solver_order", 1)
        if solver_order not in (1, 2):
            raise NotImplementedError(f"the denoise loop has a first- and a second-order step, not solver_order={solver_order}")
        ab2 = [self.scheduler.coefficients(i, i > t_start) for i in steps] if solver_order == 2 else None
        hist = torch.empty((batch_size, S_tgt, tokens.shape[2]), device=device, dtype=BF16) if ab2 is not None else None
        state = torch.empty((batch_size, S_tgt, tokens.shape[2]), device=device, dtype=torch.float32) \
            if latent_state == "fp32" else None

        L = SimpleNamespace(tokens=tokens, model_tokens=model_tokens, t_model=t_model, guidance=guidance, pooled=model_pooled,
                            embeds=model_embeds, text_ids=text_ids, latent_ids=latent_ids, S_tgt=S_tgt, batch_size=batch_size,
                            do_true_cfg=do_true_cfg, true_cfg_scale=true_cfg_scale, jak=joint_attention_kwargs or {},
                            geom=(height, width, None if image is None else tuple(image.shape[-2:])),
                            dsigma=[self.scheduler.dsigma(i) for i in steps], inpaint=inpaint,
                            sigma_next=[self.scheduler.sigma_next(i) for i in steps] if inpaint else [],
                            x0=x0 if mask is not None else None, noise=noise if mask is not None else None, mask=mask,
                            step_cache=step_cache, cache_state=None, ab2=ab2, hist=hist, latent_state=latent_state, state=state)
        graphable = self.use_graph and callback_on_step_end is None and not joint_attention_kwargs and not self._interrupt
        if graphable and step_cache is not None and step_cache.adaptive:
            if not self._said_adaptive_is_eager:
                print("step cache: the adaptive mode reads its measure back once per step, so this call runs the eager loop; "
                      "replay its decisions through the graph with StepCache(schedule=step_cache.computed_steps)")
                self._said_adaptive_is_eager = True
            graphable = False
        if graphable:
            tokens = self._denoise_graph(L)
        else:
            self._denoise(L, callback_on_step_end, timesteps)

        latents = tokens[:, :S_tgt]
        if output_type == "latent":
            image_out = latents.contiguous()
        else:
            z = self._unpack_latents(latents, height, width, self.vae_scale_factor).contiguous()
            vcfg = self.vae.config
            img = self.vae.decode(z, return_dict=False, pre_div=vcfg.scaling_factor, pre_add=vcfg.shift_factor)[0]
            if edit is not None and edit.overlay:
                image_out = ops.image_overlay(img.contiguous(), edit.pic, edit.alpha, edit.box).cpu().numpy()
                if output_type == "pil":
                    from PIL import Image
                    image_out = [Image.fromarray(a) for a in image_out]
            else:
                image_out = self.postprocess(img, output_type)
        if not return_dict:
            return (image_out,)
        return FluxPipelineOutput(images=image_out, latents=latents, crop_box=edit.box if edit is not None and edit.crop else None)

    def _denoise(self, L, callback_on_step_end=None, timesteps=None):
        if hasattr(self.transformer, "prepare_conditioning"):
            self.transformer.prepare_conditioning(L.t_model, L.guidance, L.pooled)
        tokens, B = L.tokens, L.batch_size
        sc, st = L.step_cache, None
        if sc is not None:
            st = self._step_cache_state(L)
            sc.begin(len(L.dsigma))
        seed = True
        for i in range(len(L.dsigma)):
            if self._interrupt:
                continue
            if L.do_true_cfg:
                L.model_tokens[:B].copy_(tokens)
                L.model_tokens[B:].copy_(tokens)
            fwd = dict(hidden_states=L.model_tokens, timestep=L.t_model[i], guidance=L.guidance,
                       pooled_projections=L.pooled, encoder_hidden_states=L.embeds,
                       txt_ids=L.text_ids, img_ids=L.latent_ids, joint_attention_kwargs=L.jak)
            if sc is None:
                noise_pred = self.transformer(**fwd, return_dict=False)[0]
            else:
                self.transformer.step_cache_begin(st, **fwd)
                compute = sc.step(i, st.sums.tolist() if sc.adaptive and i > 0 else None)
                noise_pred = self.transformer.step_cache_end(st, compute)
            if L.do_true_cfg:
                noise_pred = ops.true_cfg(noise_pred[:B], noise_pred[B:], L.true_cfg_scale)
            self._solver_step(L, i, noise_pred, seed)
            seed = False
            if callback_on_step_end is not None:
                out = callback_on_step_end(self, i, timesteps[i], {"latents": tokens[:, :L.S_tgt]})
                if out and "latents" in out:
                    tokens[:, :L.S_tgt].copy_(out["latents"])
                    seed = True
        if sc is not None:
            sc.block_passes = st.block_passes

    def _solver_step(self, L, i, noise_pred, seed):
        sigma_next = L.sigma_next[i] if L.inpaint else 0.0
        c_v, c_h, use_hist = L.ab2[i] if L.ab2 is not None else (L.dsigma[i], 0.0, 0)
        if L.state is not None:
            ops.solver_step_f32(L.state, L.tokens, noise_pred, L.S_tgt, c_v, c_h, use_hist, 0 if seed else 1, L.hist, sigma_next,
                                L.x0, L.noise, L.mask)
        elif L.ab2 is not None:
            ops.ab2_step(L.tokens, noise_pred, L.hist, L.S_tgt, c_v, c_h, use_hist, sigma_next, L.x0, L.noise, L.mask)
        elif L.inpaint:
            ops.euler_inpaint_step(L.tokens, noise_pred, L.S_tgt, c_v, sigma_next, L.x0, L.noise, L.mask)
        else:
            ops.euler_step(L.tokens, noise_pred, L.S_tgt, c_v)

    def _step_cache_state(self, L):
        tr = self.transformer
        if not hasattr(tr, "step_cache_begin"):
            raise ValueError("`step_cache` needs a transformer with the two-phase forward (HipFluxTransformer2DModel)")
        st = L.cache_state if L.cache_state is not None else self._cache_state
        sc = L.step_cache
        if st is None or st.measure != sc.adaptive or st.mode != sc.measure:
            st = tr.step_cache_state(measure=sc.adaptive, mode=sc.measure)
        if L.cache_state is None:
            self._cache_state = st
        st.steps, st.block_passes, st.have_residual, st.f = 0, 0, False, None
        return st

    _GRAPH_INPUTS = ("tokens", "t_model", "guidance", "pooled", "embeds", "text_ids", "latent_ids", "x0", "noise", "mask")

    def _graph_key(self, L):
        if hasattr(self.transformer, "packed"):
            self.transformer.packed()
        key = (tuple(L.tokens.shape), tuple(L.embeds.shape), tuple(L.latent_ids.shape), L.geom, L.do_true_cfg,
               float(L.true_cfg_scale), tuple(L.dsigma), L.guidance is None, L.S_tgt,
               getattr(self.transformer, "_pack_serial", 0), ops.launch_config_epoch(),
               L.inpaint, None if L.mask is None else tuple(L.mask.shape), tuple(L.sigma_next),
               None if L.step_cache is None else (L.step_cache.schedule, L.step_cache.measure),
               L.latent_state,
               1 if L.ab2 is None else 2, None if L.ab2 is None else tuple(L.ab2))
        return key

    def _denoise_graph(self, L):
        key = self._graph_key(L)
        cur = torch.cuda.current_stream()
        if self._loop_graph is None or self._loop_graph[0] != key:
            self._loop_graph = None
            G = SimpleNamespace(**vars(L))
            for n in self._GRAPH_INPUTS:
                t = getattr(L, n)
                setattr(G, n, None if t is None else t.clone())
            G.model_tokens = torch.empty_like(L.model_tokens) if L.do_true_cfg else G.tokens
            if L.hist is not None:
                G.hist = torch.empty_like(L.hist)
            if L.state is not None:
                G.state = torch.empty_like(L.state)
            if L.step_cache is not None:
                G.cache_state = self.transformer.step_cache_state(measure=False, mode=L.step_cache.measure)
            side = torch.cuda.Stream(device=L.tokens.device)
            side.wait_stream(cur)
            with torch.cuda.stream(side):
                self._denoise(G)
            cur.wait_stream(side)
            graph = torch.cuda.CUDAGraph()
            with torch.cuda.graph(graph):
                self._denoise(G)
            self._loop_graph = (key, G, graph)
        _, G, graph = self._loop_graph
# ... 15 lines not shown
```

### gpt_image_edit_amd/transformer.py

```python
import math
import os
from types import SimpleNamespace

import torch
from torch import nn

from . import flux_spec, ops
from .lora import LoraMixin
from .param_tree import ParamTreeMixin, build_param_tree

BF16 = torch.bfloat16
FUSE_QKV = os.environ.get("FK_FUSE_QKV", "1") != "0"
MLP_FIRST = os.environ.get("FK_MLP_FIRST", "0") == "1"
BLOCK_API = int(os.environ.get("FK_BLOCK_API", "2"))
MX_FUSED_QUANT = os.environ.get("FK_MX_FUSED_QUANT", "0") == "1"
MX_SPLITK = os.environ.get("FK_MX_SPLITK", "0") == "1"


def set_mx_splitk(on):
    global MX_SPLITK
    MX_SPLITK = bool(on)
    ops._set_launch()


MX_FUSED_ATTN = os.environ.get("FK_MX_FUSED_ATTN", "0") == "1"


def set_mx_fused_attn(on):
    global MX_FUSED_ATTN
    MX_FUSED_ATTN = bool(on)
    ops._set_launch()


def _mx_fused_bits():
    return (1 | (2 if MX_FUSED_ATTN else 0)) if MX_FUSED_QUANT else 0


OVERLAP_MLP = {"0": False, "1": True, "auto": "auto"}.get(os.environ.get("FK_OVERLAP_MLP", "0"), False)


def rope_tables(ids, axes_dim=(16, 56, 56), theta=10000.0):
    pos = ids.detach().to(torch.float32)
    cos_parts, sin_parts = [], []
    for i, d in enumerate(axes_dim):
        inv = 1.0 / (theta ** (torch.arange(0, d, 2, dtype=torch.float64, device=pos.device) / d))
        ang = pos[:, i].to(torch.float64)[:, None] * inv[None, :]
        cos_parts.append(torch.repeat_interleave(torch.cos(ang), 2, dim=1).float())
        sin_parts.append(torch.repeat_interleave(torch.sin(ang), 2, dim=1).float())
    return torch.cat(cos_parts, dim=1).contiguous(), torch.cat(sin_parts, dim=1).contiguous()


class HipFluxTransformer2DModel(LoraMixin, ParamTreeMixin, nn.Module):

    def __init__(self, config=None, device="cuda", dtype=BF16, init="empty", seed=0, weight_format="bf16"):
        super().__init__()
        if dtype != BF16:
            raise ValueError("the HIP path computes in bf16 (fp32 accumulate); dtype must be torch.bfloat16")
        cfg = dict(flux_spec.FLUX_KONTEXT_CONFIG)
        cfg.update(config or {})
        self.config = SimpleNamespace(**cfg)
        self.num_heads = cfg["num_attention_heads"]
        if cfg["attention_head_dim"] != 128:
            raise ValueError("attention_head_dim must be 128 (kernel tiling)")
        self.inner_dim = self.num_heads * 128
        shapes = flux_spec.flux_param_shapes(cfg)
        if init == "synthetic":
            state = flux_spec.synthetic_state(shapes, seed=seed, device=device, dtype=dtype,
                                              gen_device="cuda" if str(device).startswith("cuda") else None)
        else:
            state = {k: torch.empty(s, device=device, dtype=dtype) for k, s in shapes.items()}
        self._names = list(shapes.keys())
        self.__dict__["_pmap"] = build_param_tree(self, state, requires_grad=False)
        self._packed = None
        self._train_packs = False
        self._ws = {}
        self._rope_cache = {}
        self._freqs = None
        self._cond = None
        self._lora_init()
        self.weight_format = "bf16"
        self.set_weight_format(weight_format)

    WEIGHT_FORMATS = ("bf16", "mxfp8")

    def set_weight_format(self, weight_format):
        if weight_format not in self.WEIGHT_FORMATS:
            raise ValueError(f"weight_format must be one of {self.WEIGHT_FORMATS}, got {weight_format!r}")
        if weight_format != self.weight_format:
            self.weight_format = weight_format
            self._packed = None

    def load_state_dict(self, state_dict, strict=True, **kwargs):
        self._packed = None
        return super().load_state_dict(state_dict, strict=strict, **kwargs)

    @property
    def dtype(self):
        return BF16

    @property
    def device(self):
        return self.p("x_embedder.weight").device

    def _apply(self, fn, *a, **k):
        self._packed = None
        self._ws = {}
        self._rope_cache = {}
        self._freqs = None
        self._cond = None
        for name, t in self._lora_base.items():
            self._lora_base[name] = fn(t)
        for entries in self._lora_adapters.values():
            for e in entries.values():
                e.up, e.down = fn(e.up), fn(e.down)
        return super()._apply(fn, *a, **k)

    def packed(self):
        pk = self._packed
        if (pk is None or pk.format != self._pack_format() or pk.versions != self.param_versions(pk.sources)
                or pk.alias_ptrs != self._ptrs(pk.aliased)):
            pk = self.pack_weights()
        return pk

    def _ptrs(self, names):
        pm = self._pmap
        return tuple(pm[n].data_ptr() for n in names)

    def _fuse(self, pk, names):
        ts = [self.p(n).data for n in names]
        side_by_side = all(t.is_contiguous() and t.untyped_storage().data_ptr() == ts[0].untyped_storage().data_ptr() for t in ts) and all(
            b.data_ptr() == a.data_ptr() + a.numel() * a.element_size() for a, b in zip(ts, ts[1:]))
        if side_by_side and self._train_packs:
            shape = (sum(t.shape[0] for t in ts),) + tuple(ts[0].shape[1:])
            pk.aliased += names
            return ts[0].new_empty(0).set_(ts[0].untyped_storage(), ts[0].storage_offset(), shape)
        pk.sources += names
        t = torch.cat(ts).contiguous()
        pk.copies.append((t, names))
        return t

    def repack(self, changed):
        pk = self._packed
        if pk is None:
            return
        if pk.mod_w is not None and any(n in changed for n in pk.mod_sources):
            self._packed = None
            return
        for t, names in pk.copies:
            if any(n in changed for n in names):
                torch.cat([self.p(n).data for n in names], out=t)
        pk.versions = self.param_versions(pk.sources)

    def _pack_format(self):
        return "bf16" if self._train_packs else self.weight_format

    MX_DOUBLE = (("out", "attn.to_out.0.weight"), ("add_out", "attn.to_add_out.weight"), ("ff1", "ff.net.0.proj.weight"),
                 ("ff1_ctx", "ff_context.net.0.proj.weight"), ("ff2", "ff.net.2.weight"), ("ff2_ctx", "ff_context.net.2.weight"))
    MX_SINGLE = (("mlp", "proj_mlp.weight"), ("out", "proj_out.weight"))

    def _pack_mx(self, pk):
        pk.mx_double, pk.mx_single = [], []
        for i, blk in enumerate(pk.double):
            p = f"transformer_blocks.{i}."
            m = SimpleNamespace(qkv_img=ops.quantize_mxfp8(blk.wqkv_img), qkv_txt=ops.quantize_mxfp8(blk.wqkv_txt))
            for f, n in self.MX_DOUBLE:
                setattr(m, f, ops.quantize_mxfp8(self.p(p + n).data))
# ... 47 lines not shown
            assert o == off
        else:
            pk.mod_w = torch.cat([self.p(n + ".weight") for n in mod_names]).contiguous()
            pk.mod_b = torch.cat([self.p(n + ".bias") for n in mod_names]).contiguous()
            pk.sources += pk.mod_sources
        if pk.format == "mxfp8":
            self._pack_mx(pk)
        pk.versions, pk.alias_ptrs = self.param_versions(pk.sources), self._ptrs(pk.aliased)
        self.__dict__["_pack_serial"] = pk.serial = self.__dict__.get("_pack_serial", 0) + 1
        self._packed = pk
        return pk

    def _workspace(self, B, S_txt, S_img):
        key = (B, S_txt, S_img)
        ws = self._ws.get(key)
        if ws is not None:
            return ws
        dev, D, H = self.device, self.inner_dim, self.num_heads
        S = S_txt + S_img
        S_pad = (S + 63) // 64 * 64
        e = lambda *shape: torch.empty(shape, device=dev, dtype=BF16)
        ws = SimpleNamespace(
            S=S, S_pad=S_pad,
            s=e(B, S, D), n=e(B, S, D), qkv=e(B, S, 3 * D), q=e(B, H, S, 128), k=e(B, H, S, 128),
            o=e(B, S, D), ff=e(B, S, 4 * D), cat=e(B, S, 5 * D),
            mod=e(B, self._packed.mod_total), temb=e(B, D), act=e(B, D), tproj=e(B, 256), e1=e(B, D),
            t_emb=e(B, D), g_emb=e(B, D), p_emb=e(B, D), mxq=None, mxs=None,
        )
        self._ws = {key: ws}
        return ws

    def _overlap_pays(self, B, S, cus=256):
        nwg = B * self.num_heads * ((S + 255) // 256)
        rounds = (nwg + cus - 1) // cus
        return nwg > cus and (rounds * cus - nwg) / (rounds * cus) >= 0.08

    def _side_stream(self):
        st = self.__dict__.get("_side")
        if st is None:
            st = torch.cuda.Stream(device=self.device)
            self.__dict__["_side"] = st
            self.__dict__["_side_events"] = (torch.cuda.Event(), torch.cuda.Event())
        return st

    def _rope(self, txt_ids, img_ids, packed=False):
        key = (id(txt_ids), id(img_ids), txt_ids._version, img_ids._version)
        hit = self._rope_cache.get(key)
        if hit is None:
            t2 = txt_ids[0] if txt_ids.dim() == 3 else txt_ids
            i2 = img_ids[0] if img_ids.dim() == 3 else img_ids
            ids = torch.cat([t2.float().to(self.device), i2.float().to(self.device)], dim=0)
            cos, sin = rope_tables(ids, self.config.axes_dims_rope)
            hit = (cos, sin, txt_ids, img_ids, ops.pack_rope(cos, sin, check=False))
            self._rope_cache = {key: hit}
        return hit[4] if packed else (hit[0], hit[1])

    def _conditioning(self, timestep, guidance, pooled, tproj, e1, t_emb, g_emb, p_emb, temb, act, mod):
        c, P, pk = self.config, self.p, self._packed
        if self._freqs is None:
            self._freqs = torch.exp(-math.log(10000.0) * torch.arange(128, dtype=torch.float32) / 128).to(self.device)
        te = "time_text_embed."
        ops.timestep_proj(timestep if timestep.dtype in (BF16, torch.float32) else timestep.float(), self._freqs, out=tproj)
        ops.gemm(tproj, P(te + "timestep_embedder.linear_1.weight"), P(te + "timestep_embedder.linear_1.bias"), out=e1, epilogue=ops.FK_EPI_SILU)
        ops.gemm(e1, P(te + "timestep_embedder.linear_2.weight"), P(te + "timestep_embedder.linear_2.bias"), out=t_emb)
        if c.guidance_embeds:
            if guidance is None:
                raise ValueError("guidance is required when config.guidance_embeds is True")
            ops.timestep_proj(guidance if guidance.dtype in (BF16, torch.float32) else guidance.float(), self._freqs, out=tproj)
            ops.gemm(tproj, P(te + "guidance_embedder.linear_1.weight"), P(te + "guidance_embedder.linear_1.bias"), out=e1, epilogue=ops.FK_EPI_SILU)
            ops.gemm(e1, P(te + "guidance_embedder.linear_2.weight"), P(te + "guidance_embedder.linear_2.bias"), out=g_emb)
        else:
            g_emb.zero_()
        ops.gemm(pooled, P(te + "text_embedder.linear_1.weight"), P(te + "text_embedder.linear_1.bias"), out=e1, epilogue=ops.FK_EPI_SILU)
        ops.gemm(e1, P(te + "text_embedder.linear_2.weight"), P(te + "text_embedder.linear_2.bias"), out=p_emb)
        ops.add3(t_emb, g_emb, p_emb, out=temb)
        ops.silu(temb, out=act)
        if pk.mod_w is not None:
            ops.gemm(act, pk.mod_w, pk.mod_b, out=mod)
        else:
            for n, o, rows in pk.mod_parts:
                ops.gemm(act, P(n + ".weight"), P(n + ".bias"), out=mod[:, o:o + rows])

    @torch.no_grad()
    def prepare_conditioning(self, timesteps, guidance, pooled_projections):
        pk = self.packed()
        N, B = timesteps.shape
        D, dev = self.inner_dim, self.device
        ts = timesteps.contiguous()
        M = N * B
        e = lambda *shape: torch.empty(shape, device=dev, dtype=BF16)
        g_all = guidance.repeat(N).contiguous() if guidance is not None else None
        pooled = pooled_projections.to(BF16)
        p_all = pooled.repeat(N, 1).contiguous()
        mod = e(M, pk.mod_total)
        self._conditioning(ts.view(M), g_all, p_all, e(M, 256), e(M, D), e(M, D), e(M, D), e(M, D), e(M, D), e(M, D), mod)
        sources = [n for n in self._names if n.startswith("time_text_embed.")] + list(pk.mod_sources)
        self._cond = SimpleNamespace(ts=ts, N=N, B=B, step_bytes=B * ts.element_size(), guidance=guidance,
                                     pooled=pooled_projections, mod=mod.view(N, B, pk.mod_total), sources=sources,
                                     versions=self.param_versions(sources))

    def _cached_modulation(self, timestep, guidance, pooled_in):
        cd = self._cond
        if cd is None or timestep is None or timestep.dtype != cd.ts.dtype or timestep.numel() != cd.B:
            return None
        off = timestep.data_ptr() - cd.ts.data_ptr()
        if off < 0 or off % cd.step_bytes or off // cd.step_bytes >= cd.N or guidance is not cd.guidance:
            return None
        if pooled_in is not cd.pooled and pooled_in.data_ptr() != cd.pooled.data_ptr():
            return None
        if cd.versions != self.param_versions(cd.sources):
            self._cond = None
            return None
        return cd.mod[off // cd.step_bytes]

    def forward(self, hidden_states, encoder_hidden_states=None, pooled_projections=None, timestep=None,
                img_ids=None, txt_ids=None, guidance=None, joint_attention_kwargs=None, return_dict=True,
                **unused):
        if not hidden_states.is_cuda:
            raise RuntimeError("HipFluxTransformer2DModel needs GPU tensors: there is no CPU fallback")
        key_mask = None
        if joint_attention_kwargs and joint_attention_kwargs.get("attention_mask") is not None:
            key_mask = self._joint_key_mask(joint_attention_kwargs["attention_mask"], hidden_states, encoder_hidden_states)
        if torch.is_grad_enabled():
            names = self.grad_parameter_names()
            if names or (encoder_hidden_states is not None and encoder_hidden_states.requires_grad):
                sample = self._forward_train(names, hidden_states, encoder_hidden_states, pooled_projections, timestep,
                                             img_ids, txt_ids, guidance, key_mask)
                return SimpleNamespace(sample=sample) if return_dict else (sample,)
        return self._forward_infer(hidden_states, encoder_hidden_states, pooled_projections, timestep, img_ids, txt_ids,
                                   guidance, return_dict, key_mask)

    def _joint_key_mask(self, mask, hidden_states, encoder_hidden_states):
        B, S_img = hidden_states.shape[0], hidden_states.shape[1]
        S_txt = 0 if encoder_hidden_states is None else encoder_hidden_states.shape[1]
        if not torch.is_tensor(mask) or mask.dim() not in (2, 3) or mask.shape[0] != B or mask.shape[-1] != S_img:
            raise ValueError(f"attention_mask must be a [B, S_img] = [{B}, {S_img}] or [B, C, S_img] tensor, got "
                             f"{tuple(mask.shape) if torch.is_tensor(mask) else type(mask).__name__}")
        if S_txt < 1:
            raise ValueError("attention_mask needs a text stream (S_txt >= 1): the text keys are what keeps every sample's key set non-empty")
        if self.weight_format == "mxfp8":
            raise ValueError('attention_mask is not available with weight_format="mxfp8": the masked attention runs on the bf16 route')
        m = mask.to(hidden_states.device) != 0
        if m.dim() == 3:
            m = m.any(dim=1)
        joint = torch.cat([torch.ones((B, S_txt), device=m.device, dtype=torch.bool), m], dim=1)
        return ops.pack_key_mask(joint)

    def grad_parameter_names(self):
        return [n for n, prm in self._pmap.items() if prm.requires_grad]

    def _forward_train(self, names, hidden_states, encoder_hidden_states, pooled_projections, timestep, img_ids, txt_ids,
                       guidance, key_mask=None):
        from .backward import FluxBackward, FluxTrainFunction
        key = tuple(names)
        bw = self.__dict__.get("_autograd_bw")
        if bw is None or bw.trainable_key != key:
            bw = FluxBackward(self, trainable=names,
                              store_activations=False if self.gradient_checkpointing else "auto")
            bw.trainable_key = key
            self.__dict__["_autograd_bw"] = bw
        bw.store_activations = False if self.gradient_checkpointing else "auto"
        params = [self._pmap[n] for n in names]
        return FluxTrainFunction.apply(bw, names, hidden_states, encoder_hidden_states, pooled_projections, timestep,
                                       img_ids, txt_ids, guidance, key_mask, *params)

    @torch.no_grad()
    def _forward_infer(self, hidden_states, encoder_hidden_states, pooled_projections, timestep, img_ids, txt_ids,
                       guidance, return_dict, key_mask=None):
        f = self._infer_frame(hidden_states, encoder_hidden_states, pooled_projections, img_ids, txt_ids)
        P = self.p
        ops.gemm(f.hs, P("x_embedder.weight"), P("x_embedder.bias"), out=f.h)
        ops.gemm(f.enc, P("context_embedder.weight"), P("context_embedder.bias"), out=f.cx)
        mod = self._infer_modulation(f, timestep, guidance, pooled_projections)
        self._infer_blocks(f, mod, key_mask)
        sample = self._infer_head(f, mod)
        if not return_dict:
            return (sample,)
        return SimpleNamespace(sample=sample)

    def _infer_frame(self, hidden_states, encoder_hidden_states, pooled_projections, img_ids, txt_ids):
        pk = self.packed()
        B, S_img, _ = hidden_states.shape
        S_txt = encoder_hidden_states.shape[1]
        ws = self._workspace(B, S_txt, S_img)
        cos, sin = self._rope(txt_ids, img_ids)
        cs = self._rope(txt_ids, img_ids, packed=True)
        if cos.shape[0] != ws.S:
            raise ValueError(f"txt_ids + img_ids give {cos.shape[0]} positions for a sequence of {ws.S}")
        s, n = ws.s, ws.n
        return SimpleNamespace(pk=pk, ws=ws, B=B, S_img=S_img, S_txt=S_txt, cos=cos, sin=sin, cs=cs,
                               hs=hidden_states.to(BF16).contiguous(), enc=encoder_hidden_states.to(BF16).contiguous(),
                               pooled=pooled_projections.to(BF16).contiguous(),
                               h=s[:, S_txt:], cx=s[:, :S_txt],
                               n_img=n[:, S_txt:])

    def _infer_modulation(self, f, timestep, guidance, pooled_projections):
        mod = self._cached_modulation(timestep, guidance, pooled_projections)
        if mod is None:
            ws = f.ws
            self._conditioning(timestep, guidance, f.pooled, ws.tproj, ws.e1, ws.t_emb, ws.g_emb, ws.p_emb, ws.temb,
                               ws.act, ws.mod)
            mod = ws.mod
        return mod

    @staticmethod
    def _block_ranges(pk, blocks):
        nd, ns = len(pk.double), len(pk.single)
        lo, hi = (0, nd + ns) if blocks is None else blocks
        if not 0 <= lo <= hi <= nd + ns:
            raise ValueError(f"block range {blocks} outside the model's {nd} + {ns} blocks")
        return range(min(lo, nd), min(hi, nd)), range(max(lo - nd, 0), max(hi - nd, 0))

    def _infer_blocks(self, f, mod, key_mask=None, blocks=None):
        D = self.inner_dim
        pk, ws, B, S_txt, S_img, cos, sin, cs = f.pk, f.ws, f.B, f.S_txt, f.S_img, f.cos, f.sin, f.cs
        s = ws.s
        block_api = BLOCK_API if (FUSE_QKV and not MLP_FIRST and not (OVERLAP_MLP and (OVERLAP_MLP != "auto" or self._overlap_pays(B, ws.S)))
                                  and S_txt > 0) else 0
        if key_mask is not None:
            self._blocks_by_kernel_calls(ws, pk, mod, cos, sin, cs, B, S_txt, key_mask, blocks=blocks)
        elif pk.format == "mxfp8":
            if ws.mxq is None:
                cols = 6 * D
                ws.mxq = torch.empty(B * ws.S * cols, device=s.device, dtype=torch.uint8)
                ws.mxs = torch.empty(B * ws.S * cols // 32, device=s.device, dtype=torch.uint8)
            if S_txt == 0:
                raise ValueError("the mxfp8 weight format needs a text stream (S_txt > 0)")
            if BLOCK_API:
                self._blocks_by_c_entry(ws, pk, mod, cs, B, S_txt, S_img, BLOCK_API, blocks=blocks)
            elif MX_FUSED_QUANT:
                self._blocks_by_kernel_calls_mx_fused(ws, pk, mod, cs, B, S_txt, blocks=blocks)
            else:
                self._blocks_by_kernel_calls_mx(ws, pk, mod, cs, S_txt, blocks=blocks)
        elif block_api:
            self._blocks_by_c_entry(ws, pk, mod, cs, B, S_txt, S_img, block_api, blocks=blocks)
        else:
            self._blocks_by_kernel_calls(ws, pk, mod, cos, sin, cs, B, S_txt, blocks=blocks)

    def _infer_head(self, f, mod):
        D, off = self.inner_dim, f.pk.mod_out
        ops.ln_modulate(f.h, mod[:, off + D: off + 2 * D], mod[:, off: off + D], out=f.n_img)
        return ops.gemm(f.n_img, self.p("proj_out.weight"), self.p("proj_out.bias"))

    def step_cache_state(self, measure, mode="input"):
        if mode not in ("input", "first_block"):
            raise ValueError(f"unknown step-cache mode {mode!r}")
        if mode == "first_block" and len(self.packed().double) + len(self.packed().single) < 2:
            raise ValueError("the first-block step cache needs a model of at least two blocks: behind block 0 there is nothing to skip")
        return SimpleNamespace(measure=bool(measure), mode=mode, key=None, f=None, mod=None, key_mask=None, block_passes=0, steps=0,
                               have_residual=False, h0=None, r=None, cur=None, prev=None, sums=None, absdiff_ws=None)

    @torch.no_grad()
    def step_cache_begin(self, state, hidden_states, encoder_hidden_states=None, pooled_projections=None, timestep=None,
                         img_ids=None, txt_ids=None, guidance=None, joint_attention_kwargs=None):
        if not hidden_states.is_cuda:
            raise RuntimeError("HipFluxTransformer2DModel needs GPU tensors: there is no CPU fallback")
        state.key_mask = None
        if joint_attention_kwargs and joint_attention_kwargs.get("attention_mask") is not None:
            state.key_mask = self._joint_key_mask(joint_attention_kwargs["attention_mask"], hidden_states, encoder_hidden_states)
        f = self._infer_frame(hidden_states, encoder_hidden_states, pooled_projections, img_ids, txt_ids)
        if state.mode == "first_block":
            return self._first_block_begin(state, f, timestep, guidance, pooled_projections)
        D, dev = self.inner_dim, f.ws.s.device
        key = (f.B, f.S_img, D, dev, state.measure)
        if state.key != key:
            e = lambda: torch.empty((f.B, f.S_img, D), device=dev, dtype=BF16)
            state.key, state.h0, state.r, state.have_residual, state.steps = key, e(), e(), False, 0
            if state.measure:
                state.cur, state.prev = e(), e()
                state.sums = torch.zeros(2, device=dev, dtype=torch.float32)
                state.absdiff_ws = ops.absdiff_ws(dev)
        ops.gemm(f.hs, self.p("x_embedder.weight"), self.p("x_embedder.bias"), out=state.h0)
        state.f, state.mod = f, self._infer_modulation(f, timestep, guidance, pooled_projections)
        if state.measure:
            pk, mod = f.pk, state.mod
            off = pk.double[0].mod_img if pk.double else pk.single[0].mod
            ops.ln_modulate(state.h0, mod[:, off: off + D], mod[:, off + D: off + 2 * D], out=state.cur)
            if state.steps > 0:
                ops.absdiff_sums(state.cur, state.prev, out=state.sums, ws=state.absdiff_ws)
            state.cur, state.prev = state.prev, state.cur
        state.steps += 1

    def _first_block_begin(self, state, f, timestep, guidance, pooled_projections):
        D, dev = self.inner_dim, f.ws.s.device
        key = (f.B, f.S_img, D, dev, state.measure, state.mode)
        if state.key != key:
            e = lambda: torch.empty((f.B, f.S_img, D), device=dev, dtype=BF16)
            state.key, state.h0, state.r, state.have_residual, state.steps = key, e(), e(), False, 0
            if state.measure:
                state.cur, state.prev = e(), e()
                state.sums = torch.zeros(2, device=dev, dtype=torch.float32)
                state.absdiff_ws = ops.absdiff_ws(dev)
        ops.gemm(f.hs, self.p("x_embedder.weight"), self.p("x_embedder.bias"), out=f.h)
        ops.gemm(f.enc, self.p("context_embedder.weight"), self.p("context_embedder.bias"), out=f.cx)
        state.f, state.mod = f, self._infer_modulation(f, timestep, guidance, pooled_projections)
        if state.measure:
            state.h0.copy_(f.h)
        self._infer_blocks(f, state.mod, state.key_mask, blocks=(0, 1))
        if state.measure:
            if state.steps > 0:
                ops.residual_absdiff_sums(f.h, state.h0, state.prev, r_out=state.cur, out=state.sums, ws=state.absdiff_ws)
            else:
                ops.residual_save(f.h, state.h0, state.cur)
        state.steps += 1

    def _first_block_end(self, state, f, mod, compute):
        if compute:
            state.h0.copy_(f.h)
            pk = f.pk
            self._infer_blocks(f, mod, state.key_mask, blocks=(1, len(pk.double) + len(pk.single)))
            ops.residual_save(f.h, state.h0, state.r)
            if state.measure:
                state.cur, state.prev = state.prev, state.cur
            state.have_residual = True
            state.block_passes += 1
        else:
            if not state.have_residual:
                raise RuntimeError("step cache: a skipped step before any computed one has no residual to add")
            ops.residual_apply(f.h, state.r, out=f.h)
        return self._infer_head(f, mod)

    @torch.no_grad()
    def step_cache_end(self, state, compute):
        f, mod = state.f, state.mod
        if f is None:
            raise RuntimeError("step_cache_end without step_cache_begin")
        state.f = None
        if state.mode == "first_block":
            return self._first_block_end(state, f, mod, compute)
        if compute:
            f.h.copy_(state.h0)
            ops.gemm(f.enc, self.p("context_embedder.weight"), self.p("context_embedder.bias"), out=f.cx)
            self._infer_blocks(f, mod, state.key_mask)
            ops.residual_save(f.h, state.h0, state.r)
            state.have_residual = True
            state.block_passes += 1
        else:
            if not state.have_residual:
                raise RuntimeError("step cache: a skipped step before any computed one has no residual to add")
            ops.residual_apply(state.h0, state.r, out=f.h)
        return self._infer_head(f, mod)

    def _blocks_by_kernel_calls(self, ws, pk, mod, cos, sin, cs, B, S_txt, key_mask=None, blocks=None):
        P, D = self.p, self.inner_dim
        s, n = ws.s, ws.n
        h, cx = s[:, S_txt:], s[:, :S_txt]
        n_img, n_txt = n[:, S_txt:], n[:, :S_txt]

        def chunk(off, j):
            return mod[:, off + j * D: off + (j + 1) * D]

        dr, sr = self._block_ranges(pk, blocks)
        for i in dr:
            blk = pk.double[i]
            p = f"transformer_blocks.{i}."
            mi, mt = blk.mod_img, blk.mod_txt
            ops.ln_modulate2(s, chunk(mt, 0), chunk(mt, 1), chunk(mi, 0), chunk(mi, 1), S_txt, out=n)
            if FUSE_QKV:
                ops.gemm_grouped([dict(a=n_img, w=blk.wqkv_img, bias=blk.bqkv_img, out=ws.qkv[:, S_txt:],
                                       qkv=dict(q_out=ws.q, k_out=ws.k, wq=P(p + "attn.norm_q.weight"),
                                                wk=P(p + "attn.norm_k.weight"), cs=cs, s_offset=S_txt)),
                                  dict(a=n_txt, w=blk.wqkv_txt, bias=blk.bqkv_txt, out=ws.qkv[:, :S_txt],
                                       qkv=dict(q_out=ws.q, k_out=ws.k, wq=P(p + "attn.norm_added_q.weight"),
                                                wk=P(p + "attn.norm_added_k.weight"), cs=cs, s_offset=0))],
                                 epilogue=ops.FK_EPI_QKV)
            else:
                ops.gemm_grouped([dict(a=n_img, w=blk.wqkv_img, bias=blk.bqkv_img, out=ws.qkv[:, S_txt:]),
                                  dict(a=n_txt, w=blk.wqkv_txt, bias=blk.bqkv_txt, out=ws.qkv[:, :S_txt])])
                ops.qkv_post(ws.qkv, ws.q, ws.k, P(p + "attn.norm_q.weight"), P(p + "attn.norm_k.weight"),
                             P(p + "attn.norm_added_q.weight"), P(p + "attn.norm_added_k.weight"), cos, sin, S_txt)
            ops.attention(ws.q, ws.k, ws.qkv[:, :, 2 * D:], ws.o, key_mask=key_mask)
            ops.gemm_grouped([dict(a=ws.o[:, S_txt:], w=P(p + "attn.to_out.0.weight"), bias=P(p + "attn.to_out.0.bias"),
                                   out=h, res=h, gate=chunk(mi, 2)),
                              dict(a=ws.o[:, :S_txt], w=P(p + "attn.to_add_out.weight"), bias=P(p + "attn.to_add_out.bias"),
                                   out=cx, res=cx, gate=chunk(mt, 2))], epilogue=ops.FK_EPI_GATE_RES)
            ops.ln_modulate2(s, chunk(mt, 3), chunk(mt, 4), chunk(mi, 3), chunk(mi, 4), S_txt, out=n)
            ops.gemm_grouped([dict(a=n_img, w=P(p + "ff.net.0.proj.weight"), bias=P(p + "ff.net.0.proj.bias"), out=ws.ff[:, S_txt:]),
                              dict(a=n_txt, w=P(p + "ff_context.net.0.proj.weight"), bias=P(p + "ff_context.net.0.proj.bias"),
                                   out=ws.ff[:, :S_txt])], epilogue=ops.FK_EPI_GELU_TANH)
            ops.gemm_grouped([dict(a=ws.ff[:, S_txt:], w=P(p + "ff.net.2.weight"), bias=P(p + "ff.net.2.bias"),
                                   out=h, res=h, gate=chunk(mi, 5)),
                              dict(a=ws.ff[:, :S_txt], w=P(p + "ff_context.net.2.weight"), bias=P(p + "ff_context.net.2.bias"),
                                   out=cx, res=cx, gate=chunk(mt, 5))], epilogue=ops.FK_EPI_GATE_RES)

        use_side = key_mask is None and (self._overlap_pays(B, ws.S) if OVERLAP_MLP == "auto" else OVERLAP_MLP)
        side = self._side_stream() if use_side else None
        if side is not None:
            main = torch.cuda.current_stream()
            ev_n, ev_mlp = self._side_events
        for i in sr:
            blk = pk.single[i]
            p = f"single_transformer_blocks.{i}."
            m0 = blk.mod
            ops.ln_modulate(s, chunk(m0, 0), chunk(m0, 1), out=n)
            if side is not None:
                ev_n.record(main)
                side.wait_event(ev_n)
                with torch.cuda.stream(side):
                    ops.gemm(n, P(p + "proj_mlp.weight"), P(p + "proj_mlp.bias"), out=ws.cat[:, :, D:],
                             epilogue=ops.FK_EPI_GELU_TANH)
                    ev_mlp.record(side)
            if side is None and MLP_FIRST:
                ops.gemm(n, P(p + "proj_mlp.weight"), P(p + "proj_mlp.bias"), out=ws.cat[:, :, D:],
                         epilogue=ops.FK_EPI_GELU_TANH)
            if FUSE_QKV:
                ops.gemm(n, blk.wqkv, blk.bqkv, out=ws.qkv, epilogue=ops.FK_EPI_QKV,
                         qkv=dict(q_out=ws.q, k_out=ws.k, wq=P(p + "attn.norm_q.weight"),
                                  wk=P(p + "attn.norm_k.weight"), cs=cs, s_offset=0))
            else:
                ops.gemm(n, blk.wqkv, blk.bqkv, out=ws.qkv)
                ops.qkv_post(ws.qkv, ws.q, ws.k, P(p + "attn.norm_q.weight"), P(p + "attn.norm_k.weight"), None, None,
                             cos, sin, 0)
            ops.attention(ws.q, ws.k, ws.qkv[:, :, 2 * D:], ws.cat[:, :, :D], key_mask=key_mask)
            if side is not None:
                main.wait_event(ev_mlp)
            elif not MLP_FIRST:
                ops.gemm(n, P(p + "proj_mlp.weight"), P(p + "proj_mlp.bias"), out=ws.cat[:, :, D:],
                         epilogue=ops.FK_EPI_GELU_TANH)
            ops.gemm(ws.cat, P(p + "proj_out.weight"), P(p + "proj_out.bias"), out=s,
                     epilogue=ops.FK_EPI_GATE_RES, res=s, gate=chunk(m0, 2))


    def _blocks_by_kernel_calls_mx(self, ws, pk, mod, cs, S_txt, blocks=None):
        P, D = self.p, self.inner_dim
        s, n = ws.s, ws.n
        h, cx = s[:, S_txt:], s[:, :S_txt]
        n_img, n_txt = n[:, S_txt:], n[:, :S_txt]

        def chunk(off, j):
            return mod[:, off + j * D: off + (j + 1) * D]

        def mm(problems, epilogue):
            for pr in problems:
                pr["a"] = ops.quantize_mxfp8(pr["a"])
            ops.gemm_mxfp8_grouped(problems, epilogue=epilogue, splitk=MX_SPLITK and problems[0]["w"][0].shape[1] >= 6144)

        dr, sr = self._block_ranges(pk, blocks)
        for i in dr:
            blk, w = pk.double[i], pk.mx_double[i]
            p = f"transformer_blocks.{i}."
            mi, mt = blk.mod_img, blk.mod_txt
            ops.ln_modulate2(s, chunk(mt, 0), chunk(mt, 1), chunk(mi, 0), chunk(mi, 1), S_txt, out=n)
            mm([dict(a=n_img, w=w.qkv_img, bias=blk.bqkv_img, out=ws.qkv[:, S_txt:],
                     qkv=dict(q_out=ws.q, k_out=ws.k, wq=P(p + "attn.norm_q.weight"), wk=P(p + "attn.norm_k.weight"), cs=cs,
                              s_offset=S_txt)),
                dict(a=n_txt, w=w.qkv_txt, bias=blk.bqkv_txt, out=ws.qkv[:, :S_txt],
                     qkv=dict(q_out=ws.q, k_out=ws.k, wq=P(p + "attn.norm_added_q.weight"), wk=P(p + "attn.norm_added_k.weight"),
                              cs=cs, s_offset=0))], ops.FK_EPI_QKV)
            ops.attention(ws.q, ws.k, ws.qkv[:, :, 2 * D:], ws.o)
            mm([dict(a=ws.o[:, S_txt:], w=w.out, bias=P(p + "attn.to_out.0.bias"), out=h, res=h, gate=chunk(mi, 2)),
                dict(a=ws.o[:, :S_txt], w=w.add_out, bias=P(p + "attn.to_add_out.bias"), out=cx, res=cx, gate=chunk(mt, 2))],
               ops.FK_EPI_GATE_RES)
            ops.ln_modulate2(s, chunk(mt, 3), chunk(mt, 4), chunk(mi, 3), chunk(mi, 4), S_txt, out=n)
            mm([dict(a=n_img, w=w.ff1, bias=P(p + "ff.net.0.proj.bias"), out=ws.ff[:, S_txt:]),
                dict(a=n_txt, w=w.ff1_ctx, bias=P(p + "ff_context.net.0.proj.bias"), out=ws.ff[:, :S_txt])], ops.FK_EPI_GELU_TANH)
            mm([dict(a=ws.ff[:, S_txt:], w=w.ff2, bias=P(p + "ff.net.2.bias"), out=h, res=h, gate=chunk(mi, 5)),
                dict(a=ws.ff[:, :S_txt], w=w.ff2_ctx, bias=P(p + "ff_context.net.2.bias"), out=cx, res=cx, gate=chunk(mt, 5))],
               ops.FK_EPI_GATE_RES)
        for i in sr:
            blk, w = pk.single[i], pk.mx_single[i]
            p = f"single_transformer_blocks.{i}."
            m0 = blk.mod
            ops.ln_modulate(s, chunk(m0, 0), chunk(m0, 1), out=n)
            mm([dict(a=n, w=w.qkv, bias=blk.bqkv, out=ws.qkv,
                     qkv=dict(q_out=ws.q, k_out=ws.k, wq=P(p + "attn.norm_q.weight"), wk=P(p + "attn.norm_k.weight"), cs=cs,
                              s_offset=0))], ops.FK_EPI_QKV)
            ops.attention(ws.q, ws.k, ws.qkv[:, :, 2 * D:], ws.cat[:, :, :D])
            mm([dict(a=n, w=w.mlp, bias=P(p + "proj_mlp.bias"), out=ws.cat[:, :, D:])], ops.FK_EPI_GELU_TANH)
            mm([dict(a=ws.cat, w=w.out, bias=P(p + "proj_out.bias"), out=s, res=s, gate=chunk(m0, 2))], ops.FK_EPI_GATE_RES)

    def _blocks_by_kernel_calls_mx_fused(self, ws, pk, mod, cs, B, S_txt, blocks=None):
        P, D = self.p, self.inner_dim
        s = ws.s
        S = ws.S
        h, cx = s[:, S_txt:], s[:, :S_txt]
        M, Mi, Mt = B * S, B * (S - S_txt), B * S_txt

        def chunk(off, j):
            return mod[:, off + j * D: off + (j + 1) * D]

        def region(byte_off, rows, ld):
            return (ws.mxq[byte_off: byte_off + rows * ld].view(rows, ld),
                    ws.mxs[byte_off // 32: (byte_off + rows * ld) // 32].view(rows, ld // 32))

        def streams(byte_off, ld):
            return region(byte_off, Mi, ld), region(byte_off + Mi * ld, Mt, ld)

        n8_img, n8_txt = streams(0, D)
        o8_img, o8_txt = streams(M * D, D)
        ff8_img, ff8_txt = streams(M * D, 4 * D)
        dr, sr = self._block_ranges(pk, blocks)
        for i in dr:
            blk, w = pk.double[i], pk.mx_double[i]
            p = f"transformer_blocks.{i}."
            mi, mt = blk.mod_img, blk.mod_txt
            ops.ln_modulate2_mxfp8(s, chunk(mt, 0), chunk(mt, 1), chunk(mi, 0), chunk(mi, 1), S_txt, out=n8_txt, out_b=n8_img)
            ops.gemm_mxfp8_grouped(
                [dict(a=n8_img, w=w.qkv_img, bias=blk.bqkv_img, out=ws.qkv[:, S_txt:],
                      qkv=dict(q_out=ws.q, k_out=ws.k, wq=P(p + "attn.norm_q.weight"), wk=P(p + "attn.norm_k.weight"), cs=cs,
                               s_offset=S_txt)),
                 dict(a=n8_txt, w=w.qkv_txt, bias=blk.bqkv_txt, out=ws.qkv[:, :S_txt],
                      qkv=dict(q_out=ws.q, k_out=ws.k, wq=P(p + "attn.norm_added_q.weight"), wk=P(p + "attn.norm_added_k.weight"),
                               cs=cs, s_offset=0))], epilogue=ops.FK_EPI_QKV)
# ... 3 lines not shown
                ops.attention(ws.q, ws.k, ws.qkv[:, :, 2 * D:], ws.o)
                ops.quantize_mxfp8(ws.o[:, S_txt:], *o8_img)
                ops.quantize_mxfp8(ws.o[:, :S_txt], *o8_txt)
            ops.gemm_mxfp8_grouped(
                [dict(a=o8_img, w=w.out, bias=P(p + "attn.to_out.0.bias"), out=h, res=h, gate=chunk(mi, 2)),
                 dict(a=o8_txt, w=w.add_out, bias=P(p + "attn.to_add_out.bias"), out=cx, res=cx, gate=chunk(mt, 2))],
                epilogue=ops.FK_EPI_GATE_RES)
            ops.ln_modulate2_mxfp8(s, chunk(mt, 3), chunk(mt, 4), chunk(mi, 3), chunk(mi, 4), S_txt, out=n8_txt, out_b=n8_img)
            ops.gemm_mxfp8_grouped(
                [dict(a=n8_img, w=w.ff1, bias=P(p + "ff.net.0.proj.bias"), out_mx=ff8_img),
                 dict(a=n8_txt, w=w.ff1_ctx, bias=P(p + "ff_context.net.0.proj.bias"), out_mx=ff8_txt)], epilogue=ops.FK_EPI_GELU_TANH)
            ops.gemm_mxfp8_grouped(
                [dict(a=ff8_img, w=w.ff2, bias=P(p + "ff.net.2.bias"), out=h, res=h, gate=chunk(mi, 5)),
                 dict(a=ff8_txt, w=w.ff2_ctx, bias=P(p + "ff_context.net.2.bias"), out=cx, res=cx, gate=chunk(mt, 5))],
                epilogue=ops.FK_EPI_GATE_RES, splitk=MX_SPLITK)
        n8 = region(0, M, D)
        cat8 = region(M * D, M, 5 * D)
        cat8_attn = (cat8[0][:, :D], cat8[1][:, :D // 32])
        for i in sr:
            blk, w = pk.single[i], pk.mx_single[i]
            p = f"single_transformer_blocks.{i}."
            m0 = blk.mod
            ops.ln_modulate_mxfp8(s, chunk(m0, 0), chunk(m0, 1), out=n8)
            ops.gemm_mxfp8(n8, w.qkv, bias=blk.bqkv, out=ws.qkv, epilogue=ops.FK_EPI_QKV,
                           qkv=dict(q_out=ws.q, k_out=ws.k, wq=P(p + "attn.norm_q.weight"), wk=P(p + "attn.norm_k.weight"), cs=cs,
                                    s_offset=0))
            if MX_FUSED_ATTN:
                ops.attention_mxfp8(ws.q, ws.k, ws.qkv[:, :, 2 * D:], cat8_attn)
            else:
                ops.attention(ws.q, ws.k, ws.qkv[:, :, 2 * D:], ws.cat[:, :, :D])
                ops.quantize_mxfp8(ws.cat[:, :, :D], *cat8_attn)
            ops.gemm_mxfp8(n8, w.mlp, bias=P(p + "proj_mlp.bias"), epilogue=ops.FK_EPI_GELU_TANH, out_mx=(cat8[0], cat8[1], D))
            ops.gemm_mxfp8(cat8, w.out, bias=P(p + "proj_out.bias"), out=s, res=s, gate=chunk(m0, 2), epilogue=ops.FK_EPI_GATE_RES,
                           splitk=MX_SPLITK)

    def _block_mx_structs(self, pk):
        from . import libfk
        st = self.__dict__.get("_block_structs_mx")
        if st is None or st.serial != pk.serial:
            nd, ns = len(pk.mx_double), len(pk.mx_single)
            dbl, sgl = (libfk.DoubleBlockWeightsMx * max(nd, 1))(), (libfk.SingleBlockWeightsMx * max(ns, 1))()
            for arr, blocks, fields in ((dbl, pk.mx_double, libfk.DOUBLE_BLOCK_MX_FIELDS), (sgl, pk.mx_single, libfk.SINGLE_BLOCK_MX_FIELDS)):
                for i, m in enumerate(blocks):
                    for f in fields:
                        q, sc = getattr(m, f)
                        setattr(arr[i], f, libfk.MxPair(q.data_ptr(), sc.data_ptr()))
            st = SimpleNamespace(serial=pk.serial, dbl=dbl, sgl=sgl)
            self.__dict__["_block_structs_mx"] = st
        return st

    def _block_weight_structs(self, pk):
        from . import libfk
        P = self.p
        names_d = ("attn.norm_q.weight", "attn.norm_k.weight", "attn.norm_added_q.weight", "attn.norm_added_k.weight",
                   "attn.to_out.0.weight", "attn.to_out.0.bias", "attn.to_add_out.weight", "attn.to_add_out.bias",
                   "ff.net.0.proj.weight", "ff.net.0.proj.bias", "ff_context.net.0.proj.weight", "ff_context.net.0.proj.bias",
                   "ff.net.2.weight", "ff.net.2.bias", "ff_context.net.2.weight", "ff_context.net.2.bias")
        names_s = ("attn.norm_q.weight", "attn.norm_k.weight", "proj_mlp.weight", "proj_mlp.bias", "proj_out.weight", "proj_out.bias")
        ptrs = []
        for i, blk in enumerate(pk.double):
            p = f"transformer_blocks.{i}."
            ptrs.append((blk.wqkv_img.data_ptr(), blk.bqkv_img.data_ptr(), blk.wqkv_txt.data_ptr(), blk.bqkv_txt.data_ptr())
                        + tuple(P(p + k).data_ptr() for k in names_d))
        for i, blk in enumerate(pk.single):
            p = f"single_transformer_blocks.{i}."
            ptrs.append((blk.wqkv.data_ptr(), blk.bqkv.data_ptr()) + tuple(P(p + k).data_ptr() for k in names_s))
        ptrs = tuple(ptrs)
        st = self.__dict__.get("_block_structs")
        if st is None or st.ptrs != ptrs:
            nd, ns = len(pk.double), len(pk.single)
            dbl, sgl = (libfk.DoubleBlockWeights * max(nd, 1))(), (libfk.SingleBlockWeights * max(ns, 1))()
            for i, blk in enumerate(pk.double):
                for f, v in zip(libfk.DOUBLE_BLOCK_FIELDS, ptrs[i]):
                    setattr(dbl[i], f, v)
                dbl[i].mod_off_img, dbl[i].mod_off_txt = blk.mod_img, blk.mod_txt
            for i, blk in enumerate(pk.single):
                for f, v in zip(libfk.SINGLE_BLOCK_FIELDS, ptrs[nd + i]):
                    setattr(sgl[i], f, v)
                sgl[i].mod_off = blk.mod
            st = SimpleNamespace(ptrs=ptrs, dbl=dbl, sgl=sgl, nd=nd, ns=ns)
            self.__dict__["_block_structs"] = st
        return st

    def _blocks_by_c_entry(self, ws, pk, mod, cs, B, S_txt, S_img, api, blocks=None):
        import ctypes
        from . import libfk
        lib = libfk.load()
        st = self._block_weight_structs(pk)
        sk, slots = ops.splitk_workspace(ws.s.device)
        aw = ops.attention_workspace(ws.s.device)
        key = tuple(getattr(ws, f).data_ptr() for f in ("s", "n", "qkv", "q", "k", "o", "ff", "cat")) + (
            cs.data_ptr(), sk.data_ptr(), aw.data_ptr(), B, S_txt, S_img, pk.format,
            ws.mxq.data_ptr() if pk.format == "mxfp8" else 0, _mx_fused_bits(), MX_SPLITK)
        bw = self.__dict__.get("_block_ws")
        if bw is None or bw[0] != key:
            c = libfk.BlockWs()
            for f in ("s", "n", "qkv", "q", "k", "o", "ff", "cat"):
                setattr(c, f, getattr(ws, f).data_ptr())
            c.rope_cs, c.splitk_ws, c.attn_ws, c.attn_ws_bytes, c.splitk_slots = cs.data_ptr(), sk.data_ptr(), aw.data_ptr(), aw.numel(), slots
            c.B, c.S_txt, c.S_img, c.H, c.eps = B, S_txt, S_img, self.num_heads, 1e-6
            mxw = None
            if pk.format == "mxfp8":
                mxw = libfk.MxWs(ws.mxq.data_ptr(), ws.mxs.data_ptr(), ws.mxq.numel(), ws.mxs.numel(), _mx_fused_bits(),
                                 ctypes.pointer(ops._QUANTIZE_SLOT),
                                 int(MX_SPLITK))
            bw = (key, c, (cs, sk, aw, ws.mxq, ws.mxs), mxw)
            self.__dict__["_block_ws"] = bw
        c = bw[1]
        L = ops.LAUNCH
        c.gemm_variant, c.gemm_plan, c.gemm_group_m, c.gemm_mfma, c.attn_grid = L.gemm_variant, ops.launch_plan(), L.gemm_group_m, L.gemm_mfma, L.attn_grid
        c.gemm_variant_used = ctypes.pointer(ops._variant_slot())
        stream = ctypes.c_void_p(torch.cuda.current_stream().cuda_stream)
        mp, mbs = ctypes.c_void_p(mod.data_ptr()), mod.stride(0)
        dr, sr = self._block_ranges(pk, blocks)

        def at(arr, r):
            return arr if r.start == 0 or not len(r) else ctypes.pointer(arr[r.start])

        if pk.format == "mxfp8":
            sx, mxw = self._block_mx_structs(pk), bw[3]
            if api >= 2:
                libfk.check(lib.fk_mmdit_blocks_fwd_mx(ctypes.byref(c), ctypes.byref(mxw), at(st.dbl, dr), at(sx.dbl, dr), len(dr),
                                                       at(st.sgl, sr), at(sx.sgl, sr), len(sr), mp, mbs, stream),
                            "fk_mmdit_blocks_fwd_mx")
                return
            for i in dr:
                libfk.check(lib.fk_double_block_fwd_mx(ctypes.byref(c), ctypes.byref(mxw), ctypes.byref(st.dbl[i]),
                                                       ctypes.byref(sx.dbl[i]), mp, mbs, stream), "fk_double_block_fwd_mx")
            for i in sr:
                libfk.check(lib.fk_single_block_fwd_mx(ctypes.byref(c), ctypes.byref(mxw), ctypes.byref(st.sgl[i]),
                                                       ctypes.byref(sx.sgl[i]), mp, mbs, stream), "fk_single_block_fwd_mx")
            return
        if api >= 2:
            libfk.check(lib.fk_mmdit_blocks_fwd(ctypes.byref(c), at(st.dbl, dr), len(dr), at(st.sgl, sr), len(sr), mp, mbs, stream),
                        "fk_mmdit_blocks_fwd")
            return
        for i in dr:
            libfk.check(lib.fk_double_block_fwd(ctypes.byref(c), ctypes.byref(st.dbl[i]), mp, mbs, stream), "fk_double_block_fwd")
        for i in sr:
            libfk.check(lib.fk_single_block_fwd(ctypes.byref(c), ctypes.byref(st.sgl[i]), mp, mbs, stream), "fk_single_block_fwd")

    gradient_checkpointing = False

    def enable_gradient_checkpointing(self):
        self.gradient_checkpointing = True

    def disable_gradient_checkpointing(self):
        self.gradient_checkpointing = False

    def save_pretrained(self, save_directory, max_shard_size=5 << 30, **unused):
        import json
        import os as _os
        from . import checkpoint
        _os.makedirs(save_directory, exist_ok=True)
        checkpoint.save_sharded(self.state_dict(), save_directory, max_shard_bytes=int(max_shard_size))
        cfg = {"_class_name": "FluxTransformer2DModel", "_diffusers_version": "0.32.2"}
        cfg.update({k: (list(v) if isinstance(v, tuple) else v) for k, v in vars(self.config).items()})
        with open(_os.path.join(save_directory, "config.json"), "w") as f:
            json.dump(cfg, f, indent=1)
        return save_directory

    @classmethod
    def from_pretrained(cls, directory, device="cuda", subfolder=None, torch_dtype=BF16, weight_format="bf16", **unused):
        import os as _os
        from . import checkpoint
        d = _os.path.join(directory, subfolder) if subfolder else directory
        cfg = checkpoint._config_of(d, flux_spec.FLUX_KONTEXT_CONFIG)
        model = cls(config=cfg, device=device, dtype=torch_dtype, init="empty")
        state = checkpoint.read_state_dict(d, dtype=BF16)
        checkpoint.check_against(flux_spec.flux_param_shapes(cfg), state, f"FLUX transformer at {d}")
        model.load_state_dict(state, strict=True)
        model.set_weight_format(weight_format)
        return model
```

### include/fk.h

```cpp
#ifndef FK_H_
#define FK_H_

#include <stdint.h>

#ifdef __cplusplus
extern "C" {
#endif

typedef void* fk_stream_t;

enum {
  FK_OK = 0,
  FK_EINVAL = -1,
  FK_EUNSUPPORTED = -2,
  FK_ELAUNCH = -3,
};

enum {
  FK_EPI_NONE = 0,
  FK_EPI_GELU_TANH = 1,
  FK_EPI_SILU = 2,
  FK_EPI_GATE_RES = 3,
  FK_EPI_RES = 4,
  FK_EPI_SCALE = 5,
// ... 13 lines not shown
  void* C; fk_rows c;
  const void* res; fk_rows r;
  const void* gate;
  int64_t gate_batch_stride;
  int64_t gate_rows_per_batch;
  int32_t M, N, K;
  int32_t epilogue;
  int32_t out_fp32;
  float alpha;
  void* q_out; void* k_out;
  const void* wq; const void* wk;
  const float* rope_cs;
  void* splitk_ws;
  int32_t qkv_s_offset, qkv_s_total, qkv_heads;
  int32_t splitk_slots;
  int32_t layout;
  int32_t f32_flags;
  int32_t variant, plan, group_m, mfma;
  int32_t* variant_used;
} fk_gemm_args;
#define FK_GEMM_PLAN_EXPLICIT 8
#define FK_GEMM_PLAN_BATCH_INVARIANT (FK_GEMM_PLAN_EXPLICIT | 1)
#define FK_GEMM_PLAN_SPLITK_WHOLE 16
#define FK_GEMM_PLAN_SPLITK_SYMMETRIC 32
#define FK_GEMM_PLAN_SPLITK_UNANNOUNCED 64
#define FK_SPLITK_SLOT_BYTES (256 * 256 * 4 + 8)

int fk_gemm_bf16(const fk_gemm_args* args, fk_stream_t stream);

#define FK_MAX_GROUP 4
int fk_gemm_bf16_grouped(const fk_gemm_args* args, int32_t n, fk_stream_t stream);

int fk_quantize_mxfp8(const void* x, fk_rows xr, int64_t M, int32_t K, void* q, int64_t ldq, void* scales,
                      int64_t ld_scale, fk_stream_t stream);

typedef struct fk_gemm_mxfp8_args {
  fk_gemm_args g;
  const void* A8; int64_t lda8;
  const void* A_scale; int64_t lda_scale;
  const void* W8; int64_t ldw8;
  const void* W_scale; int64_t ldw_scale;
} fk_gemm_mxfp8_args;

int fk_gemm_mxfp8(const fk_gemm_mxfp8_args* args, fk_stream_t stream);
int fk_gemm_mxfp8_grouped(const fk_gemm_mxfp8_args* args, int32_t n, fk_stream_t stream);

typedef struct fk_gemm_mxfp8_q_args {
  fk_gemm_mxfp8_args a;
  void* Q; int64_t ldq;
  void* Q_scale; int64_t ldq_scale;
  int64_t col_offset;
} fk_gemm_mxfp8_q_args;
int fk_gemm_mxfp8_q(const fk_gemm_mxfp8_q_args* args, fk_stream_t stream);
int fk_gemm_mxfp8_q_grouped(const fk_gemm_mxfp8_q_args* args, int32_t n, fk_stream_t stream);

int fk_ln_modulate_bf16(const void* x, fk_rows xr, void* out, fk_rows outr, const void* shift,
                        const void* scale, int64_t mod_batch_stride, int64_t mod_rows_per_batch,
                        int64_t M, int32_t D, float eps, fk_stream_t stream);

int fk_ln_modulate2_bf16(const void* x, fk_rows xr, void* out, fk_rows outr, const void* shift,
                         const void* scale, const void* shift_b, const void* scale_b, int64_t split,
                         int64_t mod_batch_stride, int64_t mod_rows_per_batch, int64_t M, int32_t D, float eps,
                         fk_stream_t stream);

int fk_ln_modulate_mxfp8(const void* x, fk_rows xr, void* q, int64_t ldq, void* scales, int64_t ld_scale, const void* shift,
                         const void* scale, int64_t mod_batch_stride, int64_t mod_rows_per_batch, int64_t M, int32_t D,
                         float eps, fk_stream_t stream);
int fk_ln_modulate2_mxfp8(const void* x, fk_rows xr, void* q, void* scales, void* q_b, void* scales_b, int64_t ldq,
                          int64_t ld_scale, const void* shift, const void* scale, const void* shift_b, const void* scale_b,
                          int64_t split, int64_t mod_batch_stride, int64_t mod_rows_per_batch, int64_t M, int32_t D, float eps,
                          fk_stream_t stream);

int fk_qkv_post_bf16(const void* qkv, void* q_out, void* k_out, const void* wq_img, const void* wk_img,
                     const void* wq_txt, const void* wk_txt, const float* cos, const float* sin, int32_t B,
                     int32_t S, int32_t S_txt, int32_t H, float eps, fk_stream_t stream);

int fk_attention_fwd_bf16(const void* q, const void* k, const void* v, void* o, int32_t B, int32_t H,
                          int32_t S, int64_t v_ld, int64_t v_batch_stride, int64_t o_ld,
                          int64_t o_batch_stride, float scale, fk_stream_t stream);
int fk_attention_fwd_ws_bf16(const void* q, const void* k, const void* v, void* o, float* lse, int32_t B, int32_t H,
                             int32_t S, int64_t v_ld, int64_t v_batch_stride, int64_t o_ld, int64_t o_batch_stride,
                             float scale, void* ws, int64_t ws_bytes, int32_t grid, fk_stream_t stream);
int64_t fk_attention_ws_bytes(void);

typedef struct fk_attn_mx_out {
  void* q; void* scales;
  void* q_b; void* scales_b;
  int64_t split;
  int64_t ldq, ldq_scale;
} fk_attn_mx_out;
int fk_attention_fwd_ws_mxfp8(const void* q, const void* k, const void* v, float* lse, int32_t B, int32_t H, int32_t S,
                              int64_t v_ld, int64_t v_batch_stride, float scale, const fk_attn_mx_out* out, void* ws,
                              int64_t ws_bytes, int32_t grid, fk_stream_t stream);

int fk_attention_fwd_f32_debug(const void* q, const void* k, const void* v, float* o, int32_t B, int32_t H,
                               int32_t S, int64_t v_ld, int64_t v_batch_stride, int64_t o_ld,
                               int64_t o_batch_stride, float scale, fk_stream_t stream);

int fk_pack_key_mask(const uint8_t* mask, int64_t batch_stride, int32_t B, int32_t S, uint64_t* out, fk_stream_t stream);
int fk_attention_fwd_masked_bf16(const void* q, const void* k, const void* v, void* o, float* lse, const uint64_t* kmask, int32_t B,
                                 int32_t H, int32_t S, int64_t v_ld, int64_t v_batch_stride, int64_t o_ld, int64_t o_batch_stride,
                                 float scale, fk_stream_t stream);
int fk_attention_fwd_masked_f32_debug(const void* q, const void* k, const void* v, float* o, const uint64_t* kmask, int32_t B,
                                      int32_t H, int32_t S, int64_t v_ld, int64_t v_batch_stride, int64_t o_ld,
                                      int64_t o_batch_stride, float scale, fk_stream_t stream);

typedef struct fk_block_ws {
  void *s, *n, *qkv, *q, *k, *o, *ff, *cat;
  const float* rope_cs;
  void* splitk_ws;
  void* attn_ws;
  int64_t attn_ws_bytes;
  int32_t splitk_slots;
  int32_t B, S_txt, S_img, H;
  float eps;
  int32_t gemm_variant, gemm_plan, gemm_group_m, gemm_mfma, attn_grid;
  int32_t* gemm_variant_used;
} fk_block_ws;
typedef struct fk_double_block_weights {
  const void *wqkv_img, *bqkv_img, *wqkv_txt, *bqkv_txt;
  const void *norm_q, *norm_k, *norm_added_q, *norm_added_k;
  const void *w_out, *b_out, *w_add_out, *b_add_out;
  const void *w_ff1, *b_ff1, *w_ff1_ctx, *b_ff1_ctx;
  const void *w_ff2, *b_ff2, *w_ff2_ctx, *b_ff2_ctx;
  int64_t mod_off_img, mod_off_txt;
} fk_double_block_weights;
typedef struct fk_single_block_weights {
  const void *wqkv, *bqkv, *norm_q, *norm_k;
  const void *w_mlp, *b_mlp, *w_out, *b_out;
  int64_t mod_off;
} fk_single_block_weights;
int fk_double_block_fwd(const fk_block_ws* ws, const fk_double_block_weights* w, const void* mod, int64_t mod_batch_stride,
                        fk_stream_t stream);
int fk_single_block_fwd(const fk_block_ws* ws, const fk_single_block_weights* w, const void* mod, int64_t mod_batch_stride,
                        fk_stream_t stream);
int fk_mmdit_blocks_fwd(const fk_block_ws* ws, const fk_double_block_weights* dbl, int32_t n_double,
                        const fk_single_block_weights* sgl, int32_t n_single, const void* mod, int64_t mod_batch_stride,
                        fk_stream_t stream);

typedef struct fk_mx_pair {
  const void* q;
  const void* s;
} fk_mx_pair;
typedef struct fk_double_block_weights_mx {
  fk_mx_pair qkv_img, qkv_txt, out, add_out, ff1, ff1_ctx, ff2, ff2_ctx;
} fk_double_block_weights_mx;
typedef struct fk_single_block_weights_mx {
  fk_mx_pair qkv, mlp, out;
} fk_single_block_weights_mx;
typedef struct fk_mx_ws {
  void* q;
  void* s;
  int64_t q_bytes, s_bytes;
  int32_t fused;
  int32_t* quantize_launches;
  int32_t splitk;
} fk_mx_ws;
int fk_double_block_fwd_mx(const fk_block_ws* ws, const fk_mx_ws* mx, const fk_double_block_weights* w,
                           const fk_double_block_weights_mx* wx, const void* mod, int64_t mod_batch_stride, fk_stream_t stream);
int fk_single_block_fwd_mx(const fk_block_ws* ws, const fk_mx_ws* mx, const fk_single_block_weights* w,
                           const fk_single_block_weights_mx* wx, const void* mod, int64_t mod_batch_stride, fk_stream_t stream);
int fk_mmdit_blocks_fwd_mx(const fk_block_ws* ws, const fk_mx_ws* mx, const fk_double_block_weights* dbl,
                           const fk_double_block_weights_mx* dblx, int32_t n_double, const fk_single_block_weights* sgl,
                           const fk_single_block_weights_mx* sglx, int32_t n_single, const void* mod, int64_t mod_batch_stride,
                           fk_stream_t stream);

int fk_attention_fwd_lse_bf16(const void* q, const void* k, const void* v, void* o, float* lse, int32_t B, int32_t H,
                              int32_t S, int64_t v_ld, int64_t v_batch_stride, int64_t o_ld, int64_t o_batch_stride,
                              float scale, fk_stream_t stream);
typedef struct fk_attn_view {
  const void* p;
  int64_t ld, head_stride, batch_stride;
} fk_attn_view;
int fk_attention_bwd_bf16(const fk_attn_view* q, const fk_attn_view* k, const fk_attn_view* v, const fk_attn_view* dout,
                          const float* lse, const float* dsum, const fk_attn_view* dq, const fk_attn_view* dk,
                          const fk_attn_view* dv, int32_t B, int32_t H, int32_t S, float scale, fk_stream_t stream);
int fk_attention_bwd_ws_bf16(const fk_attn_view* q, const fk_attn_view* k, const fk_attn_view* v, const fk_attn_view* dout,
                             const float* lse, const float* dsum, const fk_attn_view* dq, const fk_attn_view* dk,
                             const fk_attn_view* dv, int32_t B, int32_t H, int32_t S, float scale, void* ws, int64_t ws_bytes,
                             int32_t grid, int32_t passes, fk_stream_t stream);

int fk_attention_bwd_masked_bf16(const fk_attn_view* q, const fk_attn_view* k, const fk_attn_view* v, const fk_attn_view* dout,
                                 const float* lse, const float* dsum, const fk_attn_view* dq, const fk_attn_view* dk,
                                 const fk_attn_view* dv, const uint64_t* kmask, int32_t B, int32_t H, int32_t S, float scale,
                                 int32_t passes, fk_stream_t stream);

int64_t fk_bwd_ws_floats(void);
int64_t fk_bwd_ew_max_blocks(void);
int fk_ln_modulate_bwd_bf16(const void* x, fk_rows xr, const void* dn, fk_rows dnr, const void* scale,
                            int64_t mod_batch_stride, int64_t rows_per_batch, const void* dx_in, fk_rows dxi, void* dx_out,
                            fk_rows dxo, float* dshift, float* dscale, int64_t dmod_batch_stride, float* ws, int32_t B,
                            int32_t D, float eps, fk_stream_t stream);
int fk_gate_res_bwd_bf16(const void* dout, fk_rows dor, const void* y, fk_rows yr, const void* gate,
                         int64_t gate_batch_stride, int64_t rows_per_batch, void* dy, fk_rows dyr, float* dgate,
                         int64_t dgate_batch_stride, float* ws, int32_t B, int32_t N, fk_stream_t stream);
int fk_gelu_bwd_bf16(const void* h, const void* df, void* out, int64_t n, fk_stream_t stream);
int fk_silu_bwd_bf16(const void* h, const void* df, void* out, int64_t n, fk_stream_t stream);
int fk_qkv_post_bwd_bf16(const void* dq, const void* dk, const void* qkv, void* dqkv, const void* wq_img, const void* wk_img,
                         const void* wq_txt, const void* wk_txt, const float* cos, const float* sin, float* dw, float* ws,
                         int32_t B, int32_t S, int32_t S_txt, int32_t H, float eps, fk_stream_t stream);
int fk_gate_res_fwd_bf16(const void* res, fk_rows rr, const void* y, fk_rows yr, const void* gate, int64_t gate_batch_stride,
                         int64_t rows_per_batch, void* out, fk_rows orr, int64_t M, int32_t N, fk_stream_t stream);
int fk_gelu_tanh_bf16(const void* x, fk_rows xr, void* y, fk_rows yr, int64_t M, int32_t N, fk_stream_t stream);
int fk_f32_to_bf16_transposed(const float* src, int64_t src_ld, void* dst, int32_t dst_ld, int32_t R, int32_t C,
                              fk_stream_t stream);
int fk_colsum_bf16(const void* x, fk_rows xr, int64_t M, int32_t N, float* out, float* ws, fk_stream_t stream);
int fk_rowdot_bf16(const void* a, int64_t a_ld, int64_t a_batch_stride, const void* c, int64_t c_ld,
                   int64_t c_batch_stride, float* out, int32_t B, int32_t S, int32_t H, fk_stream_t stream);

typedef struct fk_bwd_ws {
  int32_t B, S_txt, S_img, H;
  float eps;
  int32_t splitk_slots;
  void* g;
  void *dy, *dff, *dn, *d_o, *dqkv;
  void *dq, *dk;
  float* dsum;
  float* dmod;
  void *ff, *cat;
  const float *cos, *sin;
  float* red_ws;
  void* attn_ws; int64_t attn_ws_bytes;
  void* splitk_ws;
  const void* mod; int64_t mod_batch_stride;
  const void *actT, *onesT;
  void* dmodT;
  int32_t gemm_variant, gemm_plan, gemm_group_m, gemm_mfma, attn_grid, attn_passes;
  int32_t* gemm_variant_used;
} fk_bwd_ws;
typedef struct fk_block_saved {
  const void *x0;
  const void *n1, *qkv, *q, *k;
  const void *y1, *h1, *o;
  const float* lse;
  const void *x1, *n2, *y2;
} fk_block_saved;
typedef struct fk_single_block_grads {
  void* dwqkv; float* dbqkv;
  void* dw_mlp; float* db_mlp;
  void* dw_out; float* db_out;
  float* dnorm;
  void *dw_mod, *db_mod;
} fk_single_block_grads;
typedef struct fk_double_block_grads {
  void* dwqkv_img; float* dbqkv_img; void* dwqkv_txt; float* dbqkv_txt;
  void* dw_out; float* db_out; void* dw_add_out; float* db_add_out;
  void* dw_ff1; float* db_ff1; void* dw_ff1_ctx; float* db_ff1_ctx;
  void* dw_ff2; float* db_ff2; void* dw_ff2_ctx; float* db_ff2_ctx;
// ... 190 lines not shown
```

Before: 1.122 images/s.

## Compute only target-token rows in the last single block and output head

Adds an output-row window so the final single transformer block runs attention queries, the MLP GEMM and the output projection only over the rows whose outputs are consumed (the target image tokens), and the final LayerNorm and proj_out head process only those tokens. The attention kernel gains a query-block offset and count so it launches only the windowed 256-row blocks. The pipeline also passes text embeddings into prepare_conditioning, which probably precomputes text-side work once for the whole denoising loop. Split-K is turned off for the smaller windowed out-projection when the grid would already fill the device. The cost removed is the wasted compute on text and conditioning-image rows of the last block, whose results are discarded, in exchange for extra code paths.

```diff
diff --git a/gpt_image_edit_amd/csrc/attention_common.h b/gpt_image_edit_amd/csrc/attention_common.h
--- a/gpt_image_edit_amd/csrc/attention_common.h
+++ b/gpt_image_edit_amd/csrc/attention_common.h
@@ -19,6 +19,7 @@
   int sk_rounds;
   float* sk_partials;
   unsigned* sk_ctl;
+  int qb_first, qb_count;
 };
 
 struct AttnMxOut {
diff --git a/gpt_image_edit_amd/csrc/attention_fwd.hip b/gpt_image_edit_amd/csrc/attention_fwd.hip
--- a/gpt_image_edit_amd/csrc/attention_fwd.hip
+++ b/gpt_image_edit_amd/csrc/attention_fwd.hip
@@ -600,7 +600,8 @@
                     int64_t v_batch_stride, int64_t o_ld, int64_t o_batch_stride, float scale, bool f32out,
                     hipStream_t stream, float* lse = nullptr, void* ws = nullptr, int64_t ws_bytes = 0, int grid = 0,
                     const AttnMxOut* mx = nullptr,
-                    const uint64_t* kmask = nullptr) {
+                    const uint64_t* kmask = nullptr,
+                    int win_row0 = 0, int win_rows = 0) {
   FK_CHECK_ARG(grid >= -1 && grid != 1, "fk_attention_fwd_ws_bf16: grid %d is not 0 (stream-K grid where the plain one wastes a round), "
                "-1 (always one workgroup per 256-row block) or a workgroup count >= 2 (test hook)", grid);
   FK_CHECK_ARG(q && k && v && (o || mx), "fk_attention_fwd_bf16: null pointer");
@@ -626,6 +627,8 @@
   p.sk_rounds = 0;
   p.sk_partials = nullptr;
   p.sk_ctl = nullptr;
+  p.qb_first = 0;
+  p.qb_count = (S + 255) / 256;
   if (kmask) {
     AttnParamsMasked pm;
     static_cast<AttnParams&>(pm) = p;
@@ -653,7 +656,14 @@
     return use_interleaved(p) ? launch<8, false, true, true>(p, G, stream) : launch<8, false, false, true>(p, G, stream);
   }
   if (mx) return fk_attention_fwd4_mx_launch(p, *mx, (int)n_items, false, stream);
-  if (attn_kernel_choice() == 4) return fk_attention_fwd4_launch(p, (int)n_items, false, stream);
+  if (attn_kernel_choice() == 4) {
+    if (win_rows > 0) {
+      p.qb_first = win_row0 / 256;
+      p.qb_count = (win_row0 + win_rows + 255) / 256 - p.qb_first;
+      p.n_items = B * H * p.qb_count;
+    }
+    return fk_attention_fwd4_launch(p, p.n_items, false, stream);
+  }
   return use_interleaved(p) ? launch<8, false, true, false>(p, (int)n_items, stream)
                             : launch<8, false, false, false>(p, (int)n_items, stream);
 }
@@ -682,6 +692,16 @@
                                         float scale, void* ws, int64_t ws_bytes, int32_t grid, fk_stream_t stream_) {
   return attention_entry(q, k, v, o, B, H, S, v_ld, v_batch_stride, o_ld, o_batch_stride, scale, false,
                          (hipStream_t)stream_, lse, ws, ws_bytes, grid);
+}
+
+extern "C" int fk_attention_fwd_ws_rows_bf16(const void* q, const void* k, const void* v, void* o, float* lse, int32_t B, int32_t H,
+                                             int32_t S, int64_t v_ld, int64_t v_batch_stride, int64_t o_ld, int64_t o_batch_stride,
+                                             float scale, int32_t row0, int32_t rows, void* ws, int64_t ws_bytes, int32_t grid,
+                                             fk_stream_t stream_) {
+  FK_CHECK_ARG(row0 >= 0 && rows > 0 && (int64_t)row0 + rows <= S, "fk_attention_fwd_ws_rows_bf16: rows [%d, %d + %d) outside [0, %d)", row0,
+               row0, rows, S);
+  return attention_entry(q, k, v, o, B, H, S, v_ld, v_batch_stride, o_ld, o_batch_stride, scale, false,
+                         (hipStream_t)stream_, lse, ws, ws_bytes, grid, nullptr, nullptr, row0, rows);
 }
 
 extern "C" int fk_attention_fwd_ws_mxfp8(const void* q, const void* k, const void* v, float* lse, int32_t B, int32_t H, int32_t S,
diff --git a/gpt_image_edit_amd/csrc/attention_fwd4_kernel.inc b/gpt_image_edit_amd/csrc/attention_fwd4_kernel.inc
--- a/gpt_image_edit_amd/csrc/attention_fwd4_kernel.inc
+++ b/gpt_image_edit_amd/csrc/attention_fwd4_kernel.inc
@@ -6,7 +6,6 @@
   const int lane = tid & 63;
   const int wave = __builtin_amdgcn_readfirstlane(tid >> 6);
   const int ql = lane & 31, hh = lane >> 5;
-  const int nqb = (p.S + QBLK - 1) / QBLK;
   const int nkt = (p.S + KVBLK - 1) / KVBLK;
   int pos;
   {
@@ -51,8 +50,8 @@
       u_end -= kt1 - kt0;
     }
   }
-  const int qb = item % nqb;
-  const int bh = item / nqb;
+  const int qb = p.qb_first + item % p.qb_count;
+  const int bh = item / p.qb_count;
   const int b = bh / p.H, h = bh - b * p.H;
   const int q_row0 = qb * QBLK + wave * 64;
   const bf16_t* Kg = p.k + (int64_t)bh * p.S * HD;
diff --git a/gpt_image_edit_amd/csrc/blocks.hip b/gpt_image_edit_amd/csrc/blocks.hip
--- a/gpt_image_edit_amd/csrc/blocks.hip
+++ b/gpt_image_edit_amd/csrc/blocks.hip
@@ -311,39 +311,89 @@
   return FK_OK;
 }
 
+bool full_block_may_split(const Dims& d) {
+  static int cus = 0;
+  if (!cus) {
+    int dev = 0, v = 0;
+    cus = hipGetDevice(&dev) == hipSuccess && hipDeviceGetAttribute(&v, hipDeviceAttributeMultiprocessorCount, dev) == hipSuccess && v > 0 ? v : 256;
+  }
+  return 2 * (((int64_t)d.B * d.S + 255) / 256) * (d.D / 256) <= cus;
+}
+
 int single_block(const fk_block_ws& ws, const Dims& d, const fk_single_block_weights& w, const void* mod, int64_t mod_bs,
-                 fk_stream_t st, const fk_mx_ws* mxws = nullptr, const fk_single_block_weights_mx* wx = nullptr) {
+                 fk_stream_t st, const fk_mx_ws* mxws = nullptr, const fk_single_block_weights_mx* wx = nullptr, int win_r0 = 0,
+                 int win_rows = 0) {
   if (mxws && wx && mxws->fused) return single_block_fused(ws, d, w, mod, mod_bs, st, *mxws, *wx);
   Mx mxc;
   auto mx = [&](const fk_mx_pair* pair) -> const Mx* { if (!pair) return nullptr; mxc = Mx{mxws, pair}; return &mxc; };
   FK_CHECK_ARG(ws.cat != nullptr, "fk_single_block_fwd: needs the [attn | mlp] buffer");
   const int D = d.D, B = d.B;
   const int Ms = B * d.S;
+  const bool win = win_rows > 0;
+  const int r0 = win ? win_r0 : 0, R = win ? win_rows : d.S, Mw = B * R;
   const char* m0 = (const char*)mod + w.mod_off * 2;
   auto chunk = [&](int j) { return (const void*)(m0 + (int64_t)j * D * 2); };
   const View s_all = view(ws.s, d, D, 0, d.S, 0), n_all = view(ws.n, d, D, 0, d.S, 0);
+  const View s_w = view(ws.s, d, D, r0, R, 0), n_w = view(ws.n, d, D, r0, R, 0);
   FK_TRY(fk_ln_modulate_bf16(s_all.p, s_all.r, (void*)n_all.p, n_all.r, chunk(0), chunk(1), mod_bs, d.S, (int64_t)Ms, D, ws.eps, st));
   {
     fk_gemm_args g = gemm(n_all, w.wqkv, w.bqkv, view(ws.qkv, d, 3 * D, 0, d.S, 0), Ms, 3 * D, D, FK_EPI_QKV);
     qkv_epi(g, ws, d, w.norm_q, w.norm_k, 0);
     ctl(g, ws); FK_TRY(block_gemm(&g, 1, mx(wx ? &wx->qkv : nullptr), st));
   }
-  FK_TRY(fk_attention_fwd_ws_bf16(ws.q, ws.k, (const char*)ws.qkv + (int64_t)2 * D * 2, ws.cat, nullptr, B, d.H, d.S, 3 * D,
-                                  (int64_t)d.S * 3 * D, 5 * D, (int64_t)d.S * 5 * D, 0.08838834764831845f, ws.attn_ws,
-                                  ws.attn_ws_bytes, ws.attn_grid, st));
-  {
-    fk_gemm_args g = gemm(n_all, w.w_mlp, w.b_mlp, view(ws.cat, d, 5 * D, 0, d.S, D), Ms, 4 * D, D, FK_EPI_GELU_TANH);
+  if (win)
+    FK_TRY(fk_attention_fwd_ws_rows_bf16(ws.q, ws.k, (const char*)ws.qkv + (int64_t)2 * D * 2, ws.cat, nullptr, B, d.H, d.S, 3 * D,
+                                         (int64_t)d.S * 3 * D, 5 * D, (int64_t)d.S * 5 * D, 0.08838834764831845f, r0, R, ws.attn_ws,
+                                         ws.attn_ws_bytes, ws.attn_grid, st));
+  else
+    FK_TRY(fk_attention_fwd_ws_bf16(ws.q, ws.k, (const char*)ws.qkv + (int64_t)2 * D * 2, ws.cat, nullptr, B, d.H, d.S, 3 * D,
+                                    (int64_t)d.S * 3 * D, 5 * D, (int64_t)d.S * 5 * D, 0.08838834764831845f, ws.attn_ws,
+                                    ws.attn_ws_bytes, ws.attn_grid, st));
+  {
+    fk_gemm_args g = gemm(n_w, w.w_mlp, w.b_mlp, view(ws.cat, d, 5 * D, r0, R, D), Mw, 4 * D, D, FK_EPI_GELU_TANH);
     ctl(g, ws); FK_TRY(block_gemm(&g, 1, mx(wx ? &wx->mlp : nullptr), st));
   }
   {
-    fk_gemm_args g = gemm(view(ws.cat, d, 5 * D, 0, d.S, 0), w.w_out, w.b_out, s_all, Ms, D, 5 * D, FK_EPI_GATE_RES);
-    gate_res(g, s_all, chunk(2), mod_bs, d.S);
-    set_ws(g, ws);
+    fk_gemm_args g = gemm(view(ws.cat, d, 5 * D, r0, R, 0), w.w_out, w.b_out, s_w, Mw, D, 5 * D, FK_EPI_GATE_RES);
+    gate_res(g, s_w, chunk(2), mod_bs, R);
+    if (!win || full_block_may_split(d)) set_ws(g, ws);
     ctl(g, ws); FK_TRY(block_gemm(&g, 1, mx(wx ? &wx->out : nullptr), st));
   }
   return FK_OK;
 }
 
+int check_window(const fk_block_ws* ws, const fk_mx_ws* mx, int32_t row0, int32_t rows, const char* who) {
+  if (mx) {
+    fk_set_error("%s: the MXFP8 forms have no output-row window (pass mx = NULL, or call the unwindowed MXFP8 entry point)", who);
+    return FK_EUNSUPPORTED;
+  }
+  FK_CHECK_ARG(row0 >= 0 && rows > 0 && (int64_t)row0 + rows <= (int64_t)ws->S_txt + ws->S_img,
+               "%s: rows [%d, %d + %d) outside the joint sequence of %d", who, row0, row0, rows, ws->S_txt + ws->S_img);
+  return FK_OK;
+}
+
+}
+
+extern "C" int fk_single_block_fwd_rows(const fk_block_ws* ws, const fk_mx_ws* mx, const fk_single_block_weights* w, const void* mod,
+                                        int64_t mod_batch_stride, int32_t row0, int32_t rows, fk_stream_t stream) {
+  Dims d;
+  FK_TRY(check_ws(ws, d, "fk_single_block_fwd_rows"));
+  FK_TRY(check_window(ws, mx, row0, rows, "fk_single_block_fwd_rows"));
+  FK_CHECK_ARG(w && mod, "fk_single_block_fwd_rows: null weights / modulation");
+  return single_block(*ws, d, *w, mod, mod_batch_stride, stream, nullptr, nullptr, row0, rows);
+}
+
+extern "C" int fk_mmdit_blocks_fwd_rows(const fk_block_ws* ws, const fk_mx_ws* mx, const fk_double_block_weights* dbl, int32_t n_double,
+                                        const fk_single_block_weights* sgl, int32_t n_single, const void* mod,
+                                        int64_t mod_batch_stride, int32_t row0, int32_t rows, fk_stream_t stream) {
+  Dims d;
+  FK_TRY(check_ws(ws, d, "fk_mmdit_blocks_fwd_rows"));
+  FK_TRY(check_window(ws, mx, row0, rows, "fk_mmdit_blocks_fwd_rows"));
+  FK_CHECK_ARG(mod && n_double >= 0 && n_single >= 1 && (n_double == 0 || dbl) && sgl,
+               "fk_mmdit_blocks_fwd_rows: null weights / modulation, or no single block to apply the window to");
+  for (int i = 0; i < n_double; ++i) FK_TRY(double_block(*ws, d, dbl[i], mod, mod_batch_stride, stream));
+  for (int i = 0; i < n_single - 1; ++i) FK_TRY(single_block(*ws, d, sgl[i], mod, mod_batch_stride, stream));
+  return single_block(*ws, d, sgl[n_single - 1], mod, mod_batch_stride, stream, nullptr, nullptr, row0, rows);
 }
 
 extern "C" int fk_double_block_fwd(const fk_block_ws* ws, const fk_double_block_weights* w, const void* mod,
diff --git a/gpt_image_edit_amd/libfk.py b/gpt_image_edit_amd/libfk.py
--- a/gpt_image_edit_amd/libfk.py
+++ b/gpt_image_edit_amd/libfk.py
@@ -153,6 +153,7 @@
     "fk_qkv_post_bf16": (c_i32, [c_vp] * 9 + [c_i32] * 4 + [c_f32, c_vp]),
     "fk_attention_fwd_bf16": (c_i32, [c_vp] * 4 + [c_i32] * 3 + [c_i64] * 4 + [c_f32, c_vp]),
     "fk_attention_fwd_ws_bf16": (c_i32, [c_vp] * 5 + [c_i32] * 3 + [c_i64] * 4 + [c_f32, c_vp, c_i64, c_i32, c_vp]),
+    "fk_attention_fwd_ws_rows_bf16": (c_i32, [c_vp] * 5 + [c_i32] * 3 + [c_i64] * 4 + [c_f32, c_i32, c_i32, c_vp, c_i64, c_i32, c_vp]),
     "fk_attention_fwd_ws_mxfp8": (c_i32, [c_vp] * 4 + [c_i32] * 3 + [c_i64] * 2 + [c_f32, ctypes.POINTER(AttnMxOut), c_vp, c_i64, c_i32, c_vp]),
     "fk_attention_ws_bytes": (c_i64, []),
     "fk_attention_fwd_f32_debug": (c_i32, [c_vp] * 4 + [c_i32] * 3 + [c_i64] * 4 + [c_f32, c_vp]),
@@ -254,6 +255,10 @@
                                        ctypes.POINTER(SingleBlockWeightsMx), c_i32, c_vp, c_i64, c_vp]),
     "fk_mmdit_blocks_fwd": (c_i32, [ctypes.POINTER(BlockWs), ctypes.POINTER(DoubleBlockWeights), c_i32,
                                     ctypes.POINTER(SingleBlockWeights), c_i32, c_vp, c_i64, c_vp]),
+    "fk_single_block_fwd_rows": (c_i32, [ctypes.POINTER(BlockWs), ctypes.POINTER(MxWs), ctypes.POINTER(SingleBlockWeights), c_vp, c_i64,
+                                         c_i32, c_i32, c_vp]),
+    "fk_mmdit_blocks_fwd_rows": (c_i32, [ctypes.POINTER(BlockWs), ctypes.POINTER(MxWs), ctypes.POINTER(DoubleBlockWeights), c_i32,
+                                         ctypes.POINTER(SingleBlockWeights), c_i32, c_vp, c_i64, c_i32, c_i32, c_vp]),
     "fk_last_error": (ctypes.c_char_p, []),
     "fk_version": (ctypes.c_char_p, []),
 }
diff --git a/gpt_image_edit_amd/ops.py b/gpt_image_edit_amd/ops.py
--- a/gpt_image_edit_amd/ops.py
+++ b/gpt_image_edit_amd/ops.py
@@ -137,7 +137,9 @@
     if int(out_fp32) == 1:
         args.f32_flags = ((1 if bias is not None and bias.dtype == torch.float32 else 0) |
                           (2 if res is not None and res.dtype == torch.float32 and epilogue == FK_EPI_NONE else 0))
-    if splitk_ws is not None:
+    if splitk_ws is False:
+        pass
+    elif splitk_ws is not None:
         ws, slots = _check_splitk_ws(splitk_ws)
         args.splitk_ws, args.splitk_slots = ws.data_ptr(), slots
     elif K >= 6144 and N % 256 == 0 and M <= 256 * SPLITK_SLOTS and int(out_fp32) != 1 and layout == 0:
@@ -500,7 +502,7 @@
         raise ValueError(f"key_mask must be the contiguous int64 [{B}, {(S + 63) // 64}] tensor pack_key_mask gives")
 
 
-def attention(q, k, v, out, scale=None, lse=None, key_mask=None):
+def attention(q, k, v, out, scale=None, lse=None, key_mask=None, q_rows=None):
     _need_cuda(q, k, v, out, lse, key_mask)
     B, H, S, hd = q.shape
     if hd != 128:
@@ -518,6 +520,12 @@
                                                              _stream()), "fk_attention_fwd_masked_bf16")
         return out
     ws = attention_workspace(q.device)
+    if q_rows is not None:
+        row0, rows = (int(x) for x in q_rows)
+        libfk.check(libfk.load().fk_attention_fwd_ws_rows_bf16(_ptr(q), _ptr(k), _ptr(v), _ptr(out), _ptr(lse), B, H, S, v.stride(1),
+                                                              v.stride(0), out.stride(1), out.stride(0), scale, row0, rows, _ptr(ws),
+                                                              ws.numel(), LAUNCH.attn_grid, _stream()), "fk_attention_fwd_ws_rows_bf16")
+        return out
     libfk.check(libfk.load().fk_attention_fwd_ws_bf16(_ptr(q), _ptr(k), _ptr(v), _ptr(out), _ptr(lse), B, H, S, v.stride(1),
                                                      v.stride(0), out.stride(1), out.stride(0), scale, _ptr(ws), ws.numel(),
                                                      LAUNCH.attn_grid, _stream()), "fk_attention_fwd_bf16")
diff --git a/gpt_image_edit_amd/pipeline.py b/gpt_image_edit_amd/pipeline.py
--- a/gpt_image_edit_amd/pipeline.py
+++ b/gpt_image_edit_amd/pipeline.py
@@ -504,10 +504,16 @@
         return FluxPipelineOutput(images=image_out, latents=latents, crop_box=edit.box if edit is not None and edit.crop else None)
 
     def _denoise(self, L, callback_on_step_end=None, timesteps=None):
-        if hasattr(self.transformer, "prepare_conditioning"):
-            self.transformer.prepare_conditioning(L.t_model, L.guidance, L.pooled)
+        tr = self.transformer
+        sc, st = L.step_cache, None
+        plain = sc is None and getattr(tr, "supports_out_tokens", False)
+        rows_only = plain and getattr(tr, "weight_format", "bf16") == "bf16"
+        if hasattr(tr, "prepare_conditioning"):
+            if plain:
+                tr.prepare_conditioning(L.t_model, L.guidance, L.pooled, L.embeds)
+            else:
+                tr.prepare_conditioning(L.t_model, L.guidance, L.pooled)
         tokens, B = L.tokens, L.batch_size
-        sc, st = L.step_cache, None
         if sc is not None:
             st = self._step_cache_state(L)
             sc.begin(len(L.dsigma))
@@ -521,7 +527,9 @@
             fwd = dict(hidden_states=L.model_tokens, timestep=L.t_model[i], guidance=L.guidance,
                        pooled_projections=L.pooled, encoder_hidden_states=L.embeds,
                        txt_ids=L.text_ids, img_ids=L.latent_ids, joint_attention_kwargs=L.jak)
-            if sc is None:
+            if rows_only:
+                noise_pred = self.transformer(**fwd, return_dict=False, out_tokens=L.S_tgt)[0]
+            elif sc is None:
                 noise_pred = self.transformer(**fwd, return_dict=False)[0]
             else:
                 self.transformer.step_cache_begin(st, **fwd)
diff --git a/gpt_image_edit_amd/transformer.py b/gpt_image_edit_amd/transformer.py
--- a/gpt_image_edit_amd/transformer.py
+++ b/gpt_image_edit_amd/transformer.py
@@ -82,6 +82,7 @@
         self.set_weight_format(weight_format)
 
     WEIGHT_FORMATS = ("bf16", "mxfp8")
+    supports_out_tokens = True
 
     def set_weight_format(self, weight_format):
         if weight_format not in self.WEIGHT_FORMATS:
@@ -295,7 +296,7 @@
                 ops.gemm(act, P(n + ".weight"), P(n + ".bias"), out=mod[:, o:o + rows])
 
     @torch.no_grad()
-    def prepare_conditioning(self, timesteps, guidance, pooled_projections):
+    def prepare_conditioning(self, timesteps, guidance, pooled_projections, encoder_hidden_states=None):
         pk = self.packed()
         N, B = timesteps.shape
         D, dev = self.inner_dim, self.device
@@ -310,7 +311,21 @@
         sources = [n for n in self._names if n.startswith("time_text_embed.")] + list(pk.mod_sources)
         self._cond = SimpleNamespace(ts=ts, N=N, B=B, step_bytes=B * ts.element_size(), guidance=guidance,
                                      pooled=pooled_projections, mod=mod.view(N, B, pk.mod_total), sources=sources,
-                                     versions=self.param_versions(sources))
+                                     versions=self.param_versions(sources), enc=None, cx=None)
+        if encoder_hidden_states is not None and encoder_hidden_states.is_cuda and encoder_hidden_states.dim() == 3:
+            cd, names = self._cond, ["context_embedder.weight", "context_embedder.bias"]
+            cd.cx = ops.gemm(encoder_hidden_states.to(BF16).contiguous(), self.p(names[0]), self.p(names[1]))
+            cd.enc, cd.enc_version = encoder_hidden_states, encoder_hidden_states._version
+            cd.cx_sources, cd.cx_versions = names, self.param_versions(names)
+
+    def _cached_context(self, encoder_hidden_states):
+        cd = self._cond
+        if cd is None or cd.cx is None or encoder_hidden_states is not cd.enc or encoder_hidden_states._version != cd.enc_version:
+            return None
+        if cd.cx_versions != self.param_versions(cd.cx_sources):
+            cd.cx = cd.enc = None
+            return None
+        return cd.cx
 
     def _cached_modulation(self, timestep, guidance, pooled_in):
         cd = self._cond
@@ -328,9 +343,11 @@
 
     def forward(self, hidden_states, encoder_hidden_states=None, pooled_projections=None, timestep=None,
                 img_ids=None, txt_ids=None, guidance=None, joint_attention_kwargs=None, return_dict=True,
-                **unused):
+                out_tokens=None, **unused):
         if not hidden_states.is_cuda:
             raise RuntimeError("HipFluxTransformer2DModel needs GPU tensors: there is no CPU fallback")
+        if out_tokens is not None and not 0 < int(out_tokens) <= hidden_states.shape[1]:
+            raise ValueError(f"out_tokens = {out_tokens} outside (0, {hidden_states.shape[1]}]")
         key_mask = None
         if joint_attention_kwargs and joint_attention_kwargs.get("attention_mask") is not None:
             key_mask = self._joint_key_mask(joint_attention_kwargs["attention_mask"], hidden_states, encoder_hidden_states)
@@ -339,9 +356,11 @@
             if names or (encoder_hidden_states is not None and encoder_hidden_states.requires_grad):
                 sample = self._forward_train(names, hidden_states, encoder_hidden_states, pooled_projections, timestep,
                                              img_ids, txt_ids, guidance, key_mask)
+                if out_tokens is not None:
+                    sample = sample[:, :int(out_tokens)]
                 return SimpleNamespace(sample=sample) if return_dict else (sample,)
         return self._forward_infer(hidden_states, encoder_hidden_states, pooled_projections, timestep, img_ids, txt_ids,
-                                   guidance, return_dict, key_mask)
+                                   guidance, return_dict, key_mask, None if out_tokens is None else int(out_tokens))
 
     def _joint_key_mask(self, mask, hidden_states, encoder_hidden_states):
         B, S_img = hidden_states.shape[0], hidden_states.shape[1]
@@ -379,14 +398,23 @@
 
     @torch.no_grad()
     def _forward_infer(self, hidden_states, encoder_hidden_states, pooled_projections, timestep, img_ids, txt_ids,
-                       guidance, return_dict, key_mask=None):
+                       guidance, return_dict, key_mask=None, out_tokens=None):
+        if out_tokens is not None and self._pack_format() == "mxfp8":
+            raise ValueError('out_tokens is not available with weight_format="mxfp8": the MXFP8 blocks have no output-row window')
         f = self._infer_frame(hidden_states, encoder_hidden_states, pooled_projections, img_ids, txt_ids)
         P = self.p
         ops.gemm(f.hs, P("x_embedder.weight"), P("x_embedder.bias"), out=f.h)
-        ops.gemm(f.enc, P("context_embedder.weight"), P("context_embedder.bias"), out=f.cx)
+        cx = self._cached_context(encoder_hidden_states)
+        if cx is not None:
+            f.cx.copy_(cx)
+        else:
+            ops.gemm(f.enc, P("context_embedder.weight"), P("context_embedder.bias"), out=f.cx)
         mod = self._infer_modulation(f, timestep, guidance, pooled_projections)
-        self._infer_blocks(f, mod, key_mask)
-        sample = self._infer_head(f, mod)
+        self._infer_blocks(f, mod, key_mask, out_rows=None if out_tokens is None else (f.S_txt, out_tokens))
+        if out_tokens is not None and f.B * out_tokens < 192:
+            sample = self._infer_head(f, mod)[:, :out_tokens].contiguous()
+        else:
+            sample = self._infer_head(f, mod, out_tokens)
         if not return_dict:
             return (sample,)
         return SimpleNamespace(sample=sample)
@@ -424,14 +452,18 @@
             raise ValueError(f"block range {blocks} outside the model's {nd} + {ns} blocks")
         return range(min(lo, nd), min(hi, nd)), range(max(lo - nd, 0), max(hi - nd, 0))
 
-    def _infer_blocks(self, f, mod, key_mask=None, blocks=None):
+    def _infer_blocks(self, f, mod, key_mask=None, blocks=None, out_rows=None):
         D = self.inner_dim
         pk, ws, B, S_txt, S_img, cos, sin, cs = f.pk, f.ws, f.B, f.S_txt, f.S_img, f.cos, f.sin, f.cs
         s = ws.s
+        if out_rows is not None:
+            sr = self._block_ranges(pk, blocks)[1]
+            if not len(sr) or sr.stop != len(pk.single) or pk.format == "mxfp8" or out_rows[1] >= ws.S or B * out_rows[1] < 192:
+                out_rows = None
         block_api = BLOCK_API if (FUSE_QKV and not MLP_FIRST and not (OVERLAP_MLP and (OVERLAP_MLP != "auto" or self._overlap_pays(B, ws.S)))
                                   and S_txt > 0) else 0
         if key_mask is not None:
-            self._blocks_by_kernel_calls(ws, pk, mod, cos, sin, cs, B, S_txt, key_mask, blocks=blocks)
+            self._blocks_by_kernel_calls(ws, pk, mod, cos, sin, cs, B, S_txt, key_mask, blocks=blocks, out_rows=out_rows)
         elif pk.format == "mxfp8":
             if ws.mxq is None:
                 cols = 6 * D
@@ -446,12 +478,16 @@
             else:
                 self._blocks_by_kernel_calls_mx(ws, pk, mod, cs, S_txt, blocks=blocks)
         elif block_api:
-            self._blocks_by_c_entry(ws, pk, mod, cs, B, S_txt, S_img, block_api, blocks=blocks)
+            self._blocks_by_c_entry(ws, pk, mod, cs, B, S_txt, S_img, block_api, blocks=blocks, out_rows=out_rows)
         else:
-            self._blocks_by_kernel_calls(ws, pk, mod, cos, sin, cs, B, S_txt, blocks=blocks)
-
-    def _infer_head(self, f, mod):
+            self._blocks_by_kernel_calls(ws, pk, mod, cos, sin, cs, B, S_txt, blocks=blocks, out_rows=out_rows)
+
+    def _infer_head(self, f, mod, out_tokens=None):
         D, off = self.inner_dim, f.pk.mod_out
+        if out_tokens is not None:
+            h, n_img = f.h[:, :out_tokens], f.n_img[:, :out_tokens]
+            ops.ln_modulate(h, mod[:, off + D: off + 2 * D], mod[:, off: off + D], out=n_img)
+            return ops.gemm(n_img, self.p("proj_out.weight"), self.p("proj_out.bias"))
         ops.ln_modulate(f.h, mod[:, off + D: off + 2 * D], mod[:, off: off + D], out=f.n_img)
         return ops.gemm(f.n_img, self.p("proj_out.weight"), self.p("proj_out.bias"))
 
@@ -554,7 +590,7 @@
             ops.residual_apply(state.h0, state.r, out=f.h)
         return self._infer_head(f, mod)
 
-    def _blocks_by_kernel_calls(self, ws, pk, mod, cos, sin, cs, B, S_txt, key_mask=None, blocks=None):
+    def _blocks_by_kernel_calls(self, ws, pk, mod, cos, sin, cs, B, S_txt, key_mask=None, blocks=None, out_rows=None):
         P, D = self.p, self.inner_dim
         s, n = ws.s, ws.n
         h, cx = s[:, S_txt:], s[:, :S_txt]
@@ -605,16 +641,23 @@
             blk = pk.single[i]
             p = f"single_transformer_blocks.{i}."
             m0 = blk.mod
+            win = out_rows if out_rows is not None and i == len(pk.single) - 1 else None
+            n_w, cat_w, s_w, split_ws = n, ws.cat, s, None
+            if win is not None:
+                rw = slice(win[0], win[0] + win[1])
+                n_w, cat_w, s_w = n[:, rw], ws.cat[:, rw], s[:, rw]
+                cus = torch.cuda.get_device_properties(s.device).multi_processor_count
+                split_ws = None if 2 * ((B * ws.S + 255) // 256) * (D // 256) <= cus else False
             ops.ln_modulate(s, chunk(m0, 0), chunk(m0, 1), out=n)
             if side is not None:
                 ev_n.record(main)
                 side.wait_event(ev_n)
                 with torch.cuda.stream(side):
-                    ops.gemm(n, P(p + "proj_mlp.weight"), P(p + "proj_mlp.bias"), out=ws.cat[:, :, D:],
+                    ops.gemm(n_w, P(p + "proj_mlp.weight"), P(p + "proj_mlp.bias"), out=cat_w[:, :, D:],
                              epilogue=ops.FK_EPI_GELU_TANH)
                     ev_mlp.record(side)
             if side is None and MLP_FIRST:
-                ops.gemm(n, P(p + "proj_mlp.weight"), P(p + "proj_mlp.bias"), out=ws.cat[:, :, D:],
+                ops.gemm(n_w, P(p + "proj_mlp.weight"), P(p + "proj_mlp.bias"), out=cat_w[:, :, D:],
                          epilogue=ops.FK_EPI_GELU_TANH)
             if FUSE_QKV:
                 ops.gemm(n, blk.wqkv, blk.bqkv, out=ws.qkv, epilogue=ops.FK_EPI_QKV,
@@ -624,14 +667,17 @@
                 ops.gemm(n, blk.wqkv, blk.bqkv, out=ws.qkv)
                 ops.qkv_post(ws.qkv, ws.q, ws.k, P(p + "attn.norm_q.weight"), P(p + "attn.norm_k.weight"), None, None,
                              cos, sin, 0)
-            ops.attention(ws.q, ws.k, ws.qkv[:, :, 2 * D:], ws.cat[:, :, :D], key_mask=key_mask)
+            if win is not None:
+                ops.attention(ws.q, ws.k, ws.qkv[:, :, 2 * D:], ws.cat[:, :, :D], key_mask=key_mask, q_rows=win)
+            else:
+                ops.attention(ws.q, ws.k, ws.qkv[:, :, 2 * D:], ws.cat[:, :, :D], key_mask=key_mask)
             if side is not None:
                 main.wait_event(ev_mlp)
             elif not MLP_FIRST:
-                ops.gemm(n, P(p + "proj_mlp.weight"), P(p + "proj_mlp.bias"), out=ws.cat[:, :, D:],
+                ops.gemm(n_w, P(p + "proj_mlp.weight"), P(p + "proj_mlp.bias"), out=cat_w[:, :, D:],
                          epilogue=ops.FK_EPI_GELU_TANH)
-            ops.gemm(ws.cat, P(p + "proj_out.weight"), P(p + "proj_out.bias"), out=s,
-                     epilogue=ops.FK_EPI_GATE_RES, res=s, gate=chunk(m0, 2))
+            ops.gemm(cat_w, P(p + "proj_out.weight"), P(p + "proj_out.bias"), out=s_w,
+                     epilogue=ops.FK_EPI_GATE_RES, res=s_w, gate=chunk(m0, 2), splitk_ws=split_ws)
 
 
     def _blocks_by_kernel_calls_mx(self, ws, pk, mod, cs, S_txt, blocks=None):
@@ -801,7 +847,7 @@
             self.__dict__["_block_structs"] = st
         return st
 
-    def _blocks_by_c_entry(self, ws, pk, mod, cs, B, S_txt, S_img, api, blocks=None):
+    def _blocks_by_c_entry(self, ws, pk, mod, cs, B, S_txt, S_img, api, blocks=None, out_rows=None):
         import ctypes
         from . import libfk
         lib = libfk.load()
@@ -851,12 +897,20 @@
                                                        ctypes.byref(sx.sgl[i]), mp, mbs, stream), "fk_single_block_fwd_mx")
             return
         if api >= 2:
+            if out_rows is not None:
+                libfk.check(lib.fk_mmdit_blocks_fwd_rows(ctypes.byref(c), None, at(st.dbl, dr), len(dr), at(st.sgl, sr), len(sr), mp, mbs,
+                                                         out_rows[0], out_rows[1], stream), "fk_mmdit_blocks_fwd_rows")
+                return
             libfk.check(lib.fk_mmdit_blocks_fwd(ctypes.byref(c), at(st.dbl, dr), len(dr), at(st.sgl, sr), len(sr), mp, mbs, stream),
                         "fk_mmdit_blocks_fwd")
             return
         for i in dr:
             libfk.check(lib.fk_double_block_fwd(ctypes.byref(c), ctypes.byref(st.dbl[i]), mp, mbs, stream), "fk_double_block_fwd")
         for i in sr:
+            if out_rows is not None and i == len(pk.single) - 1:
+                libfk.check(lib.fk_single_block_fwd_rows(ctypes.byref(c), None, ctypes.byref(st.sgl[i]), mp, mbs, out_rows[0], out_rows[1],
+                                                         stream), "fk_single_block_fwd_rows")
+                continue
             libfk.check(lib.fk_single_block_fwd(ctypes.byref(c), ctypes.byref(st.sgl[i]), mp, mbs, stream), "fk_single_block_fwd")
 
     gradient_checkpointing = False
diff --git a/include/fk.h b/include/fk.h
--- a/include/fk.h
+++ b/include/fk.h
@@ -119,6 +119,10 @@
                              int32_t S, int64_t v_ld, int64_t v_batch_stride, int64_t o_ld, int64_t o_batch_stride,
                              float scale, void* ws, int64_t ws_bytes, int32_t grid, fk_stream_t stream);
 int64_t fk_attention_ws_bytes(void);
+int fk_attention_fwd_ws_rows_bf16(const void* q, const void* k, const void* v, void* o, float* lse, int32_t B, int32_t H,
+                                  int32_t S, int64_t v_ld, int64_t v_batch_stride, int64_t o_ld, int64_t o_batch_stride,
+                                  float scale, int32_t row0, int32_t rows, void* ws, int64_t ws_bytes, int32_t grid,
+                                  fk_stream_t stream);
 
 typedef struct fk_attn_mx_out {
   void* q; void* scales;
@@ -201,6 +205,12 @@
                            const fk_double_block_weights_mx* dblx, int32_t n_double, const fk_single_block_weights* sgl,
                            const fk_single_block_weights_mx* sglx, int32_t n_single, const void* mod, int64_t mod_batch_stride,
                            fk_stream_t stream);
+
+int fk_single_block_fwd_rows(const fk_block_ws* ws, const fk_mx_ws* mx, const fk_single_block_weights* w, const void* mod,
+                             int64_t mod_batch_stride, int32_t row0, int32_t rows, fk_stream_t stream);
+int fk_mmdit_blocks_fwd_rows(const fk_block_ws* ws, const fk_mx_ws* mx, const fk_double_block_weights* dbl, int32_t n_double,
+                             const fk_single_block_weights* sgl, int32_t n_single, const void* mod, int64_t mod_batch_stride,
+                             int32_t row0, int32_t rows, fk_stream_t stream);
 
 int fk_attention_fwd_lse_bf16(const void* q, const void* k, const void* v, void* o, float* lse, int32_t B, int32_t H,
                               int32_t S, int64_t v_ld, int64_t v_batch_stride, int64_t o_ld, int64_t o_batch_stride,
```

After: 1.128 images/s, median of 6. Within noise of the previous version (+0.5%).
